# hrz2000/CustomNeRF

Hardware: AMD Instinct MI355X
Metric: training rays/s (higher is better)
Workload: dtype f16

## Files before the change

customnerf_amd/_lib.py:

```python
import ctypes as C
import os

import torch

_HERE = os.path.dirname(os.path.abspath(__file__))
LIB_PATH = os.path.join(_HERE, "libcustomnerf_hip.so")
ABI_VERSION = 7

vp, u32, u64, f32, i32 = C.c_void_p, C.c_uint32, C.c_uint64, C.c_float, C.c_int

SIGNATURES = {
    "cnerf_abi_version": [],
    "cnerf_profile_stage_events": [vp, u32],
    "cnerf_near_far_from_aabb": [vp, vp, vp, u32, f32, vp, vp, vp],
    "cnerf_sph_from_ray": [vp, vp, f32, u32, vp, vp],
    "cnerf_morton3D": [vp, u32, vp, vp],
    "cnerf_morton3D_invert": [vp, u32, vp, vp],
    "cnerf_packbits": [vp, u32, f32, vp, vp],
    "cnerf_march_rays_train": [vp, vp, vp, f32, f32, u32, u32, u32, u32, u32, vp, vp, vp, vp, vp, vp, vp, vp, vp],
    "cnerf_march_rays_train_count": [vp, vp, vp, f32, f32, u32, u32, u32, u32, vp, vp, vp, vp, vp, vp],
    "cnerf_march_rays_train_write": [vp, vp, vp, f32, f32, u32, u32, u32, u32, u32, vp, vp, vp, vp, vp, vp, vp, vp],
    "cnerf_march_rays_train_count_hits": [vp, vp, vp, f32, f32, u32, u32, u32, u32, vp, vp, vp, vp, vp, vp, vp],
    "cnerf_march_rays_train_write_hits": [vp, vp, f32, f32, u32, u32, u32, u32, u32, vp, vp, vp, vp, vp, vp, vp, vp],
    "cnerf_composite_rays_train_forward": [vp, vp, vp, vp, u32, u32, f32, vp, vp, vp, u32, vp],
    "cnerf_composite_rays_train_backward": [vp, vp, vp, vp, vp, vp, vp, vp, u32, u32, f32, vp, vp, u32, vp],
    "cnerf_march_rays": [u32, u32, vp, vp, vp, vp, f32, f32, u32, u32, u32, vp, vp, vp, vp, vp, vp, vp, vp],
    "cnerf_composite_rays": [u32, u32, f32, vp, vp, vp, vp, vp, vp, vp, vp, u32, vp],
    "cnerf_compact_rays_alive": [vp, u32, vp, vp, vp],
    "cnerf_grid_encode_forward": [vp, vp, vp, vp, u32, u32, u32, u32, u32, f32, u32, vp, u32, i32, u32, i32, vp],
    "cnerf_grid_encode_forward_strided": [vp, vp, vp, vp, u32, u32, u32, u32, u32, f32, u32, vp, u32, i32, u32, i32, u32, vp],
    "cnerf_grid_encode_forward_ordered": [vp, vp, vp, vp, u32, u32, u32, u32, u32, f32, u32, vp, u32, i32, u32, i32, u32, u32, vp],
    "cnerf_grid_encode_backward": [vp, vp, vp, vp, u32, u32, u32, u32, u32, f32, u32, vp, vp, u32, i32, u32, i32, vp, u64, vp],
    "cnerf_grid_encode_backward_prepare": [vp, vp, u32, u32, u32, u32, u32, f32, u32, u32, i32, u32, i32, vp, u64, vp, vp],
    "cnerf_grid_encode_backward_prepared": [vp, vp, vp, vp, u32, u32, u32, u32, u32, f32, u32, u32, i32, u32, i32, vp, u64, vp],
    "cnerf_grid_encode_backward_workspace_bytes": [vp, u32, u32, u32, u32, u32, f32, u32, i32, vp],
    "cnerf_grid_encode_backward_needs_plan": [vp, u32, u32, u32, u32, u32, f32, u32, u32, i32, vp],
    "cnerf_grad_total_variation": [vp, vp, vp, vp, f32, u32, u32, u32, u32, f32, u32, u32, i32, vp],
    "cnerf_cast_f32_to_f16": [vp, vp, u64, vp],
    "cnerf_field_forward": [vp, vp, vp, u32, u32, u32, u32, u32, vp, vp, vp, vp, vp, i32, vp],
    "cnerf_field_forward_strided": [vp, vp, vp, u32, u32, u32, u32, u32, vp, vp, vp, vp, vp, i32, u32, vp],
    "cnerf_field_backward": [vp, vp, vp, u32, u32, u32, u32, u32, vp, vp, vp, vp, vp, vp, vp, vp, vp, vp, u64, i32, vp],
    "cnerf_field_backward_ex": [vp, vp, vp, u32, u32, u32, u32, u32, vp, vp, vp, vp, vp, vp, vp, vp, vp, vp, u64, i32, vp, vp],
    "cnerf_field_backward_workspace_bytes": [u32, u32, u32, u32, i32, vp],
    "cnerf_stream_capture_id": [vp, vp],
    "cnerf_field_weight_image_bytes": [u32, u32, u32, vp],
    "cnerf_field_pack_weights": [u32, u32, u32, vp, vp, vp, vp, u64, vp],
    "cnerf_field_forward_img": [vp, vp, vp, u32, u32, u32, u32, u32, vp, vp, vp, vp, vp, i32, u32, vp, vp],
    "cnerf_field_backward_img": [vp, vp, vp, u32, u32, u32, u32, u32, vp, vp, vp, vp, vp, vp, vp, vp, vp, vp, u64, i32, vp, vp, vp],
    "cnerf_mlp_forward": [vp, u32, vp, u32, u32, u32, u32, u32, i32, vp, u32, i32, vp],
    "cnerf_mlp_backward": [vp, u32, vp, vp, u32, u32, u32, u32, u32, u32, i32, vp, u32, vp, vp, u64, i32, vp],
    "cnerf_mlp_backward_workspace_bytes": [u32, u32, u32, u32, u32, i32, vp],
    "cnerf_generate_rays": [vp, u32, u32, u32, f32, f32, f32, f32, f32, i32, vp, vp, vp],
    "cnerf_generate_rays_fisheye": [vp, u32, u32, u32, f32, f32, f32, f32, f32, vp, vp, vp, vp],
    "cnerf_occupancy_points": [vp, u32, f32, f32, vp, vp],
    "cnerf_occupancy_update": [vp, u32, f32, vp, vp, vp],
    "cnerf_occupancy_finalize_pack": [vp, u32, f32, vp, u32, vp, vp, vp],
    "cnerf_sample_pdf": [vp, vp, vp, u32, u32, u32, vp, vp],
    "cnerf_sample_coarse": [vp, vp, vp, vp, vp, vp, u32, u32, vp, vp, vp],
    "cnerf_sample_fine_merge": [vp, vp, vp, vp, vp, vp, vp, vp, u32, u32, u32, vp, vp, vp],
    "cnerf_sample_fine_merge_split": [vp, vp, vp, vp, vp, vp, vp, vp, u32, u32, u32, vp, vp, vp, vp, vp],
    "cnerf_sample_coarse_unit": [vp, vp, vp, vp, vp, vp, u32, u32, vp, vp, vp, f32, vp],
    "cnerf_sample_fine_merge_split_unit": [vp, vp, vp, vp, vp, vp, vp, vp, u32, u32, u32, vp, vp, vp, vp, f32, vp],
    "cnerf_composite_run": [vp, vp, vp, vp, vp, u32, u32, u32, i32, f32, vp, vp, vp],
    "cnerf_composite_run_backward": [vp, vp, vp, vp, vp, vp, u32, u32, u32, i32, f32, i32, i32, vp, vp, vp],
    "cnerf_recon_loss": [vp, vp, vp, u32, f32, f32, vp, vp, vp],
    "cnerf_recon_loss_scaled": [vp, vp, vp, u32, f32, f32, vp, vp, vp, vp],
    "cnerf_sample_coarse_unit_aabb": [vp, vp, vp, f32, vp, u32, u32, vp, vp, vp, vp, vp, f32, vp],
    "cnerf_composite_run_indexed": [vp, vp, vp, vp, vp, u32, u32, u32, i32, f32, vp, vp, vp, vp, vp, vp],
    "cnerf_composite_run_indexed_variants": [vp, vp, vp, vp, vp, u32, u32, u32, i32, f32, vp, vp, vp, vp, vp, u32, vp],
    "cnerf_composite_run_backward_indexed": [vp, vp, vp, vp, vp, vp, u32, u32, u32, i32, f32, i32, i32, vp, vp, vp, vp],
    "cnerf_composite_run_backward_indexed_flush": [vp, vp, vp, vp, vp, vp, u32, u32, u32, i32, f32, i32, i32, vp, vp, vp, i32, vp, vp],
    "cnerf_adam_step": [vp, vp, vp, vp, vp, u64, f32, f32, f32, f32, u32, f32, i32, vp],
    "cnerf_scaler_check": [vp, u64, vp, vp],
    "cnerf_scaler_watch": [vp],
    "cnerf_grid_backward_adam": [vp],
    "cnerf_grid_backward_adam_consumed": [vp],
    "cnerf_adam_step_scaled": [vp, vp, vp, vp, vp, u64, f32, f32, f32, f32, vp, f32, i32, vp],
    "cnerf_dp_pack": [vp, vp, u64, f32, vp],
    "cnerf_dp_reduce": [vp, u32, u64, vp, vp, vp],
    "cnerf_scaler_update": [vp, f32, f32, u32, vp],
    "cnerf_adam_step_scaled_multi": [vp, f32, f32, f32, vp, f32, i32, i32, f32, f32, u32, vp],
    "cnerf_marching_cubes_workspace_bytes": [u32, u32, u32, vp],
    "cnerf_marching_cubes_count": [vp, u32, u32, u32, f32, vp, u64, vp, vp],
    "cnerf_marching_cubes_emit": [vp, u32, u32, u32, f32, vp, vp, vp, u64, vp, vp, vp, u32, u32, vp],
    "cnerf_mesh_components_workspace_bytes": [u32, u32, vp],
    "cnerf_mesh_components_count": [vp, u32, u32, u32, i32, vp, u64, vp, vp],
    "cnerf_mesh_components_emit": [vp, vp, u32, vp, u32, u32, i32, vp, u64, vp, vp, vp, vp, u32, u32, vp],
    "cnerf_mesh_cluster_workspace_bytes": [u32, u32, vp, vp],
    "cnerf_mesh_cluster_count": [vp, u32, vp, u32, vp, vp, vp, vp, u64, vp, vp],
    "cnerf_mesh_cluster_emit": [vp, vp, u32, vp, u32, vp, vp, vp, vp, u64, vp, vp, vp, u32, u32, vp],
    "cnerf_mesh_decimate_workspace_bytes": [u32, u32, vp],
    "cnerf_mesh_decimate_init": [vp, u32, vp, u32, vp, u64, vp, vp],
    "cnerf_mesh_decimate_round": [u32, u32, u32, vp, u64, vp, vp],
    "cnerf_mesh_decimate_emit": [vp, u32, u32, vp, u64, vp, vp, vp, vp, u32, u32, vp],
    "cnerf_mesh_smooth_workspace_bytes": [u32, u32, vp],
    "cnerf_mesh_smooth_init": [vp, u32, u32, vp, u64, vp, vp],
    "cnerf_mesh_smooth_steps": [vp, u32, u32, u32, f32, f32, i32, vp, u64, vp, vp],
    "cnerf_mesh_smooth_normals": [vp, vp, u32, vp, u32, vp, u64, vp, vp],
    "cnerf_mesh_atlas_layout": [u32, u32, vp, vp],
    "cnerf_mesh_atlas_uvs": [vp, u32, u32, u32, vp, u32, vp, vp],
    "cnerf_mesh_atlas_points": [vp, vp, u32, vp, u32, u32, u32, u32, vp, vp, vp, u32, vp],
    "cnerf_mesh_atlas_store": [u32, u32, u32, u32, vp, u32, vp, vp, vp, vp],
    "cnerf_mesh_atlas_fill": [u32, u32, vp, vp, vp],
    "cnerf_mesh_raster_workspace_bytes": [u32, u32, u32, u32, vp],
    "cnerf_mesh_raster_visibility": [vp, u32, vp, u32, vp, f32, f32, f32, f32, u32, u32, i32, f32, i32, vp, u64, vp, vp, vp, vp, vp],
    "cnerf_mesh_raster_shade": [vp, vp, vp, u32, u32, vp, u32, u32, i32, vp, vp, vp, u32, vp, vp, f32, f32, vp, vp, vp, vp],
    "cnerf_mesh_bvh_workspace_bytes": [u32, u32, vp],
    "cnerf_mesh_bvh_build": [vp, u32, vp, u32, vp, u64, vp, vp],
    "cnerf_mesh_bvh_closest": [vp, u64, u32, u32, vp, u32, vp, vp, vp, vp, vp, vp],
    "cnerf_mesh_sample_workspace_bytes": [u32, vp],
    "cnerf_mesh_sample_count": [vp, u32, vp, u32, f32, vp, u64, vp, vp],
    "cnerf_mesh_sample_emit": [vp, u32, vp, u32, f32, vp, u64, vp, vp, vp, vp, u64, vp],
    "cnerf_sd_gemm": [vp, vp, u64, vp],
    "cnerf_sd_gemm_workspace_bytes": [vp, vp],
    "cnerf_sd_gemm_serves_ln": [vp, vp],
    "cnerf_sd_groupnorm_forward": [vp, vp, vp, u32, u32, u32, u32, f32, i32, vp, i32, vp, vp],
    "cnerf_sd_groupnorm_backward": [vp, vp, vp, vp, u32, u32, u32, u32, f32, i32, vp, vp, vp, vp],
    "cnerf_sd_groupnorm_backward_ex": [vp, vp, vp, vp, u32, u32, u32, u32, f32, i32, vp, vp, i32, vp, vp, vp],
    "cnerf_sd_layernorm_forward": [vp, vp, vp, u32, u32, f32, vp, vp],
    "cnerf_sd_softmax_forward": [vp, u64, u32, u32, vp],
    "cnerf_sd_softmax_backward": [vp, vp, u64, u32, u32, vp],
    "cnerf_sd_attention": [vp, vp, vp, vp, u32, u32, u32, u32, u32, u32, u64, u32, u64, u32, u64, u32, u64, i32, vp],
    "cnerf_sd_attention_v": [vp, vp, vp, vp, u32, u32, u32, u32, u32, u32, u64, u32, u64, u32, u64, u32, u64, i32, vp],
    "cnerf_sd_geglu": [vp, u64, u32, vp, vp],
    "cnerf_sd_transpose": [vp, vp, u32, u32, u32, u32, u32, u64, u64, vp],
    "cnerf_sd_image_to_vae_input": [vp, u32, u32, u32, u32, u32, vp, vp],
    "cnerf_sd_image_to_vae_input_backward": [vp, u32, u32, u32, u32, u32, vp, vp],
    "cnerf_sd_clip_preprocess": [vp, u32, u32, u32, u32, vp, vp, vp, vp],
    "cnerf_sd_patchify": [vp, u32, u32, u32, vp, vp],
    "cnerf_sd_timestep_embedding": [vp, u32, u32, vp, vp],
    "cnerf_sd_add_noise": [vp, vp, f32, u32, vp, vp],
    "cnerf_sd_sds_grad": [vp, u32, vp, f32, f32, f32, u32, vp, vp],
    "cnerf_edit_ray_images": [vp, u32, u32, vp, vp, vp, vp],
    "cnerf_edit_ray_images_backward": [vp, vp, vp, u32, u32, vp, vp],
    "cnerf_edit_l1_loss": [vp, vp, u32, f32, vp, vp, vp],
    "cnerf_edit_sds_loss": [vp, vp, u32, vp, vp, vp],
    "cnerf_edit_scale_by_scalar": [vp, vp, f32, u32, vp, vp],
    "cnerf_sd_sample_latents": [vp, vp, u32, u32, f32, vp, vp],
    "cnerf_sd_sample_latents_backward": [vp, vp, vp, u32, u32, f32, vp, vp],
    "cnerf_set_floats": [vp, vp, u32, vp],
    "cnerf_sd_add": [vp, vp, u64, vp, vp],
    "cnerf_sd_silu": [vp, u64, vp, vp],
    "cnerf_sd_concat": [vp, vp, u64, u32, u32, vp, vp],
    "cnerf_sd_concat_gn": [vp, vp, u64, u32, u32, vp, vp, u32, u32, vp],
}


class SdGemmDesc(C.Structure):
    _fields_ = [("A", vp), ("B", vp), ("C", vp), ("C32", vp), ("bias", vp), ("bias_rows", vp), ("residual", vp),
                ("M", u32), ("N", u32), ("K", u32), ("lda", u32), ("ldb", u32), ("ldc", u32), ("ldr", u32),
                ("rows_per_bias_row", u32), ("ld_bias_rows", u32), ("alpha", f32), ("act", C.c_int32), ("batch_outer", u32), ("batch_inner", u32),
                ("sa_o", u64), ("sa_i", u64), ("sb_o", u64), ("sb_i", u64), ("sc_o", u64), ("sc_i", u64),
                ("mode", C.c_int32), ("Cin", u32), ("H_in", u32), ("W_in", u32), ("H_out", u32), ("W_out", u32),
                ("KH", u32), ("KW", u32), ("stride", u32), ("pad_t", u32), ("pad_l", u32), ("ups", u32), ("tstride", u32),
                ("gn_sums", vp), ("gn_groups", u32), ("gn_rows", u32),
                ("ln_out", vp), ("ln_gamma", vp), ("ln_beta", vp), ("ln_eps", f32)]

ADAM_MAX_JOBS = 8


class AdamJobs(C.Structure):
    _fields_ = [("p", vp * ADAM_MAX_JOBS), ("g", vp * ADAM_MAX_JOBS), ("m", vp * ADAM_MAX_JOBS), ("v", vp * ADAM_MAX_JOBS), ("p_half", vp * ADAM_MAX_JOBS),
                ("n", u64 * ADAM_MAX_JOBS), ("lr", f32 * ADAM_MAX_JOBS), ("n_jobs", u32)]


class GridAdam(C.Structure):
    _fields_ = [("p", vp), ("g", vp), ("m", vp), ("v", vp), ("p_half", vp), ("n", u64), ("lr", f32), ("beta1", f32), ("beta2", f32), ("eps", f32),
                ("scaler_state", vp), ("extra_inv", f32), ("zero_grad", C.c_int)]


F32, F16 = 0, 1


def _load():
    if not os.path.exists(LIB_PATH):
        raise ImportError(
            f"{LIB_PATH} not found: the HIP extension is the product and has no fallback. "
            "Build it with `python -c 'import __graft_entry__ as g; g.build()'` or `make -C customnerf_amd/csrc`.")
    lib = C.CDLL(LIB_PATH)
    for name, argtypes in SIGNATURES.items():
        fn = getattr(lib, name)
        fn.argtypes = argtypes
        fn.restype = C.c_int
    lib.cnerf_target_arch.restype = C.c_char_p
    if lib.cnerf_abi_version() != ABI_VERSION:
        raise ImportError(f"ABI mismatch: library {lib.cnerf_abi_version()} vs binding {ABI_VERSION}")
    return lib


lib = _load()


def check(rc, what=""):
    if rc == 0:
        return
    if rc < 0:
        raise ValueError(f"customnerf_hip: {what} rejected its arguments (code {rc})")
    raise RuntimeError(f"customnerf_hip: {what} failed with hipError {rc}")


def ptr(t):
    return None if t is None else t.data_ptr()


def stream():
    return torch.cuda.current_stream().cuda_stream


def require_cuda(*tensors):
    for t in tensors:
        if t is not None and not t.is_cuda:
            raise RuntimeError("customnerf_amd: tensors must live on the GPU (HIP device memory); there is no CPU path")


def dtype_id(t):
    if t.dtype == torch.float32:
        return F32
    if t.dtype == torch.float16:
        return F16
    raise ValueError(f"unsupported dtype {t.dtype}")


def scratch_key(device):
    import torch
    return (device, torch.cuda.current_stream(device).cuda_stream)


_SCRATCH_GENERATION = [0]


def scratch_reallocated():
    _SCRATCH_GENERATION[0] += 1


def scratch_generation():
    return _SCRATCH_GENERATION[0]


_GRAD_CHAIN = {}


def grad_chain_wait(device):
    import torch
    cur = torch.cuda.current_stream(device)
    last = _GRAD_CHAIN.get(device)
    if last is not None and last.cuda_stream != cur.cuda_stream:
        cur.wait_stream(last)


def grad_chain_record(device):
    import torch
    _GRAD_CHAIN[device] = torch.cuda.current_stream(device)
```

customnerf_amd/csrc/gridencoder_binned.hip:

```cpp
#include "grid_common.h"
#include <vector>
#include <algorithm>
#include <cstdio>

#define BN_CHUNK_LOG2 12
#define BN_CHUNK (1u << BN_CHUNK_LOG2)
#define BN_THREADS 256
#define BN_PPT 4
#define BN_PTS (BN_THREADS * BN_PPT)
#define BN_MAX_CHUNKS 512
#define BN_SEG (1u << 18)

struct BinPlan {
    uint32_t bin_first[GE_MAX_LEVELS + 1];
    uint32_t nb;
    uint32_t total_bins;
};

struct BinWs {
    uint32_t *hist;
    uint32_t *bin_base;
    uint32_t *seg_first;
    void *records;
};
// ... 611 lines not shown
                    res_a = (uint32_t)old & 0x7FFFFFFFu;
                    res_b = (uint32_t)(old >> 32) & 0x7FFFFFFFu;
                }
            } else {
                if (sa) res_a = atomicAdd(&cursor[bin0 + 2 * lane], sa) & 0x7FFFFFFFu;
                if (sb) res_b = atomicAdd(&cursor[bin0 + 2 * lane + 1], sb) & 0x7FFFFFFFu;
            }
        }
    }
    asm volatile("s_waitcnt lgkmcnt(0)" ::: "memory");
    __builtin_amdgcn_s_barrier();
    asm volatile("" ::: "memory");
    uint2 *__restrict__ region = dslab + ((size_t)slot * nb + pb) * B3_REGION;
#pragma unroll
    for (int i = 0; i < PPT; i++) {
        if (!ok[i] || (abl & 4)) continue;
        const uint32_t fxq = min((uint32_t)(fx[i] * 65536.0f), 65535u);
        union { __half2 h; uint32_t u; } v;
        auto put = [&](uint32_t c, uint32_t ticket, uint32_t word, uint32_t val) {
            const uint32_t sl = start[c] + ticket;
            if (sl < B3_CAP) { s_rec[sl] = make_uint2(word, val); if (!wide) s_bin[sl] = (uint8_t)c; }
            else region[sl] = make_uint2(word, val);
        };
#pragma unroll
        for (int q = 0; q < 4; q++) {
            const uint32_t a0 = i0[i][q], a1 = i1[i][q];
            const uint32_t c0 = bin_of(a0);
            if (paired(a0, a1)) {
                const uint32_t t = 31u - (uint32_t)__clz((int)(a0 ^ a1));
                v.h = __floats2half2_rn(wyz[i][q] * g0[i], wyz[i][q] * g1[i]);
                put(c0, tk[i][q], local_of(a0) | (t << 12) | (fxq << 16), v.u);
            } else {
                const float w0 = (1 - fx[i]) * wyz[i][q], w1 = fx[i] * wyz[i][q];
                v.h = __floats2half2_rn(w0 * g0[i], w0 * g1[i]);
                put(c0, tk[i][q] & 0xFFFFu, local_of(a0) | (B3_SINGLE << 12), v.u);
                v.h = __floats2half2_rn(w1 * g0[i], w1 * g1[i]);
                put(bin_of(a1), tk[i][q] >> 16, local_of(a1) | (B3_SINGLE << 12), v.u);
            }
        }
    }
    if (!dense_lvl && wide) {
        if (threadIdx.x <= NBN / 2) {
            const uint32_t capb = plan.capb, b_lo = ((bin0 >> 1) + threadIdx.x) * 2u;
#pragma unroll
            for (int h = 0; h < 2; h++) {
                const uint32_t c = b_lo + h - bin0;
                if (c >= nch) continue;
                const uint32_t n = cnt[c], st0 = start[c], res = h ? res_b : res_a;
                const uint32_t staged = st0 >= B3_CAP ? 0u : min(n, (uint32_t)B3_CAP - st0);
                const uint32_t room = res >= capb ? 0u : capb - res;
                const uint32_t fit = min(min(n, room), staged);
                gdst[c] = res - st0;
                cnt[c] = fit;
                if (!(abl & 8)) runs[(size_t)(bin0 + c) * nb + pb] = (n - fit) | ((st0 + fit) << 16);
                if (n > fit) atomicOr(&cursor[bin0 + c], 0x80000000u);
            }
        }
    } else if (!dense_lvl && threadIdx.x < 64) {
        const uint32_t capb = plan.capb;
#pragma unroll
        for (int h = 0; h < 2; h++) {
            const uint32_t c = 2 * threadIdx.x + h;
            const uint32_t n = cnt[c], st0 = start[c], res = h ? res_b : res_a;
            const uint32_t staged = st0 >= B3_CAP ? 0u : min(n, (uint32_t)B3_CAP - st0);
            const uint32_t room = res >= capb ? 0u : capb - res;
            const uint32_t fit = min(min(n, room), staged);
            gdst[c] = res - st0;
            cnt[c] = fit;
            if (c < nch && !(abl & 8)) runs[(size_t)(bin0 + c) * nb + pb] = (n - fit) | ((st0 + fit) << 16);
            if (c < nch && n > fit) atomicOr(&cursor[bin0 + c], 0x80000000u);
        }
    }
    __syncthreads();
    const uint32_t total = (abl & 2) ? 0u : min(*s_total, (uint32_t)B3_CAP);
    if (dense_lvl) {
        for (uint32_t sl = threadIdx.x; sl < total; sl += B3_THREADS) region[sl] = s_rec[sl];
    } else if (wide) {
        const uint32_t capb = plan.capb, l16 = threadIdx.x & 15, grp = threadIdx.x >> 4;
        for (uint32_t c = grp; c < nch; c += B3_THREADS / 16) {
            const uint32_t st0 = start[c], en = min(c + 1 < NBN ? start[c + 1] : *s_total, total), fit = cnt[c], gd = gdst[c];
            for (uint32_t sl = st0 + l16; sl < en; sl += 16) {
                if (sl - st0 < fit) hslab[(size_t)(bin0 + c) * capb + (gd + sl)] = s_rec[sl];
                else region[sl] = s_rec[sl];
            }
        }
    } else {
        const uint32_t capb = plan.capb;
        for (uint32_t sl = threadIdx.x; sl < total; sl += B3_THREADS) {
            const uint32_t c = s_bin[sl];
            const uint32_t pos = gdst[c] + sl;
            if (sl - start[c] < cnt[c]) hslab[(size_t)(bin0 + c) * capb + pos] = s_rec[sl];
            else region[sl] = s_rec[sl];
        }
    }
}

__global__ void __launch_bounds__(BN_SCAN_THREADS) k_bin3_totals(const uint32_t *__restrict__ runs, uint32_t *__restrict__ pre, const uint32_t *__restrict__ cursor,
                                                                 uint32_t *__restrict__ bin_total, const Bin3Plan plan, uint32_t n_slots) {
    constexpr uint32_t NW = BN_SCAN_THREADS / 64;
    __shared__ uint32_t wave_tot[NW];
    __shared__ uint32_t carry;
    const uint32_t bin = blockIdx.x, nb = plan.p.nb;
    uint32_t slot = 0;
    while (slot + 1 < n_slots && plan.p.bin_first[slot + 1] <= bin) slot++;
    const bool hashed = plan.dense_slot[slot] == 0xFFFFFFFFu;
    if (hashed) {
        const uint32_t cw = cursor[bin], c = cw & 0x7FFFFFFFu;
        if (!(cw >> 31)) {
            if (threadIdx.x == 0) bin_total[bin] = min(c, plan.capb);
            return;
        }
    }
    const uint32_t *h = runs + (size_t)bin * nb;
    uint32_t *o = pre + (size_t)bin * nb;
    const uint32_t tid = threadIdx.x, lane = tid & 63, wave = tid >> 6;
    if (tid == 0) carry = 0;
    __syncthreads();
    for (uint32_t s0 = 0; s0 < nb; s0 += BN_SCAN_THREADS * 4) {
        const uint32_t i = s0 + tid * 4;
        uint32_t v[4];
#pragma unroll
        for (int k = 0; k < 4; k++) v[k] = i + k < nb ? (h[i + k] & 0xFFFFu) : 0;
        const uint32_t mine = v[0] + v[1] + v[2] + v[3];
        const uint32_t incl = cn_wave_incl_scan(mine);
        if (lane == 63) wave_tot[wave] = incl;
        __syncthreads();
        uint32_t wbase = 0, tot = 0;
#pragma unroll
        for (uint32_t w = 0; w < NW; w++) {
            const uint32_t t = wave_tot[w];
            if (w < wave) wbase += t;
            tot += t;
        }
        const uint32_t base = carry;
        uint32_t run = base + wbase + incl - mine;
#pragma unroll
        for (int k = 0; k < 4; k++) {
            if (i + k < nb) o[i + k] = run;
            run += v[k];
        }
        __syncthreads();
        if (tid == 0) carry = base + tot;
        __syncthreads();
    }
    if (tid == 0) bin_total[bin] = hashed ? min(cursor[bin] & 0x7FFFFFFFu, plan.capb) + carry : carry;
}

struct B3Adam {
    float *p, *m, *v;
    __half *ph;
    const float *state;
    float lr, beta1, beta2, eps, extra_inv;
    int zero_grad, on;
    const float *cst;
};
struct B3AdamConst { float gscale, step_size, rsqrt_bc2; int skip; };
__device__ __forceinline__ B3AdamConst b3_adam_const(const B3Adam &ad) {
    B3AdamConst c;
    c.gscale = ad.cst[0]; c.step_size = ad.cst[1]; c.rsqrt_bc2 = ad.cst[2]; c.skip = ad.cst[3] != 0.0f;
    return c;
}
__device__ __forceinline__ void b3_adam_update(const B3Adam &ad, const B3AdamConst &c, size_t idx, float4 gg, float4 pp, float4 mm, float4 vv, float4 *d4) {
    float *pa = &pp.x, *ga = &gg.x, *ma = &mm.x, *va = &vv.x;
#pragma unroll
    for (int k = 0; k < 4; k++) {
        const float gk = ga[k] * c.gscale;
        ma[k] = ad.beta1 * ma[k] + (1.0f - ad.beta1) * gk;
        va[k] = ad.beta2 * va[k] + (1.0f - ad.beta2) * gk * gk;
        pa[k] -= c.step_size * ma[k] / (sqrtf(va[k]) * c.rsqrt_bc2 + ad.eps);
    }
    *reinterpret_cast<float4 *>(ad.p + idx) = pp;
    *reinterpret_cast<float4 *>(ad.m + idx) = mm;
    *reinterpret_cast<float4 *>(ad.v + idx) = vv;
    *d4 = ad.zero_grad ? make_float4(0, 0, 0, 0) : gg;
    if (ad.ph) {
        union { __half2 h[2]; uint2 u; } o;
        o.h[0] = __floats2half2_rn(pp.x, pp.y);
        o.h[1] = __floats2half2_rn(pp.z, pp.w);
        *reinterpret_cast<uint2 *>(ad.ph + idx) = o.u;
    }
}
__device__ __forceinline__ void b3_adam_apply(const B3Adam &ad, const B3AdamConst &c, size_t idx, float4 gg, float4 *d4) {
    if (c.skip) {
        *d4 = ad.zero_grad ? make_float4(0, 0, 0, 0) : gg;
        return;
    }
    b3_adam_update(ad, c, idx, gg, *reinterpret_cast<const float4 *>(ad.p + idx), *reinterpret_cast<const float4 *>(ad.m + idx),
                   *reinterpret_cast<const float4 *>(ad.v + idx), d4);
}

__device__ __forceinline__ void b3_flush(const long long *acc, const GridLevels &lv, const Bin3Slots &plan, uint32_t slot, uint32_t bin, uint32_t nseg, uint32_t gseg,
                                         float *__restrict__ grad_grid, long long *__restrict__ partial, uint32_t hbits, const B3Adam &ad,
                                         const B3AdamConst &adc) {
    const uint32_t level = lv.order[slot];
    const uint32_t cb = bin - plan.bin_first[slot];
    const uint32_t e0 = hbits == 0xFFu ? cb << BN_CHUNK_LOG2 : 0u;
    const uint32_t n_entries = hbits == 0xFFu ? min(BN_CHUNK, lv.size[level] - e0) : min(BN_CHUNK, lv.size[level] >> hbits);
    float *__restrict__ dst = grad_grid + (size_t)lv.offset[level] * 2;
    if (nseg == 1 && ad.on && !adc.skip) {
        constexpr int NIT = BN_CHUNK / 2 / 1024;
        float4 gg[NIT], pp[NIT], mm[NIT], vv[NIT];
        auto index_of = [&](uint32_t j) {
            const uint32_t e = hbits == 0xFFu ? e0 + 2 * j : b3_entry_of(2 * j, cb, hbits);
            return ((size_t)lv.offset[level] + e) * 2;
        };
#pragma unroll
        for (int it = 0; it < NIT; it++) {
            const uint32_t j = it * 1024 + threadIdx.x;
            if (j < n_entries / 2) {
                const size_t idx = index_of(j);
                gg[it] = *reinterpret_cast<const float4 *>(grad_grid + idx);
                pp[it] = *reinterpret_cast<const float4 *>(ad.p + idx);
                mm[it] = *reinterpret_cast<const float4 *>(ad.m + idx);
                vv[it] = *reinterpret_cast<const float4 *>(ad.v + idx);
            }
        }
#pragma unroll
        for (int it = 0; it < NIT; it++) {
            const uint32_t j = it * 1024 + threadIdx.x;
            if (j >= n_entries / 2) continue;
            const size_t idx = index_of(j);
            float4 g = gg[it];
            g.x += bn_acc_to_float<__half>(acc[j * 2]); g.y += bn_acc_to_float<__half>(acc[BN_CHUNK + j * 2]);
            g.z += bn_acc_to_float<__half>(acc[j * 2 + 1]); g.w += bn_acc_to_float<__half>(acc[BN_CHUNK + j * 2 + 1]);
            b3_adam_update(ad, adc, idx, g, pp[it], mm[it], vv[it], reinterpret_cast<float4 *>(grad_grid + idx));
        }
    } else if (nseg == 1) {
        for (uint32_t j = threadIdx.x; j < n_entries / 2; j += 1024) {
            const uint32_t e = hbits == 0xFFu ? e0 + 2 * j : b3_entry_of(2 * j, cb, hbits);
            float4 *d4 = reinterpret_cast<float4 *>(dst + (size_t)e * 2);
            float4 g = *d4;
            g.x += bn_acc_to_float<__half>(acc[j * 2]); g.y += bn_acc_to_float<__half>(acc[BN_CHUNK + j * 2]);
            g.z += bn_acc_to_float<__half>(acc[j * 2 + 1]); g.w += bn_acc_to_float<__half>(acc[BN_CHUNK + j * 2 + 1]);
            if (ad.on) b3_adam_apply(ad, adc, ((size_t)lv.offset[level] + e) * 2, g, d4);
            else *d4 = g;
        }
    } else {
        long long *__restrict__ img = partial + (size_t)gseg * (BN_CHUNK * 2);
        for (uint32_t j = threadIdx.x; j < n_entries * 2; j += 1024) img[j] = acc[(j & 1) * BN_CHUNK + (j >> 1)];
    }
}

#define B3_RS_GROUPS 64
#ifndef B3_RS_BINS
#define B3_RS_BINS 256
#endif
__global__ void __launch_bounds__(256) k_bin3_reduce_split(const long long *__restrict__ partial, const uint32_t *__restrict__ seg_first,
                                                           const GridLevels lv, const Bin3Plan plan, float *__restrict__ grad_grid, uint32_t n_slots,
                                                           const uint32_t *__restrict__ split_list, const B3Adam ad) {
    __shared__ long long s_sum[3][B3_RS_GROUPS][4];
    const uint32_t n_split = split_list ? split_list[0] : gridDim.x;
    if (blockIdx.x >= n_split) return;
    B3AdamConst adc = {0.0f, 0.0f, 0.0f, 0};
    if (ad.on) adc = b3_adam_const(ad);
    for (uint32_t b = blockIdx.x; b < n_split; b += gridDim.x) {
    const uint32_t bin = split_list ? split_list[1 + b] : b;
    const uint32_t s0 = seg_first[bin], nseg = seg_first[bin + 1] - s0;
    if (nseg <= 1) continue;
    uint32_t slot = 0;
    while (slot + 1 < n_slots && plan.p.bin_first[slot + 1] <= bin) slot++;
    const uint32_t level = lv.order[slot];
    const bool dense_lvl = plan.dense_slot[slot] != 0xFFFFFFFFu;
    const uint32_t hb = plan.hbits[slot], cb = bin - plan.p.bin_first[slot];
    const uint32_t e0 = dense_lvl ? cb << BN_CHUNK_LOG2 : 0u;
    const uint32_t n_entries = dense_lvl ? min(BN_CHUNK, lv.size[level] - e0) : min(BN_CHUNK, lv.size[level] >> hb);
    if (blockIdx.y * B3_RS_GROUPS >= n_entries / 2) continue;
    const uint32_t lane = threadIdx.x & 63, sl = threadIdx.x >> 6;
    const uint32_t j = blockIdx.y * B3_RS_GROUPS + lane;
    const bool ok = j < n_entries / 2;
    long long sum[4] = {0, 0, 0, 0};
    const uint32_t e_dst = dense_lvl ? e0 + 2 * j : b3_entry_of(2 * j, cb, hb);
    const size_t idx = ((size_t)lv.offset[level] + e_dst) * 2;
    const bool fin = !sl && ok, upd = fin && ad.on && !adc.skip;
    float4 g_old = make_float4(0, 0, 0, 0), pp = g_old, mm = g_old, vv = g_old;
    if (fin) g_old = *reinterpret_cast<const float4 *>(grad_grid + idx);
    if (upd) {
        pp = *reinterpret_cast<const float4 *>(ad.p + idx);
        mm = *reinterpret_cast<const float4 *>(ad.m + idx);
        vv = *reinterpret_cast<const float4 *>(ad.v + idx);
    }
    if (ok) {
        const long long *__restrict__ src = partial + (size_t)s0 * (BN_CHUNK * 2) + (size_t)j * 4;
#pragma unroll 8
        for (uint32_t s = sl; s < nseg; s += 4) {
            const longlong2 v0 = reinterpret_cast<const longlong2 *>(src + (size_t)s * (BN_CHUNK * 2))[0];
            const longlong2 v1 = reinterpret_cast<const longlong2 *>(src + (size_t)s * (BN_CHUNK * 2))[1];
            sum[0] += v0.x; sum[1] += v0.y; sum[2] += v1.x; sum[3] += v1.y;
        }
    }
    if (sl) {
#pragma unroll
        for (int k = 0; k < 4; k++) s_sum[sl - 1][lane][k] = sum[k];
    }
    __syncthreads();
    if (!sl && ok) {
#pragma unroll
        for (int w = 0; w < 3; w++)
#pragma unroll
            for (int k = 0; k < 4; k++) sum[k] += s_sum[w][lane][k];
        float4 *dst = reinterpret_cast<float4 *>(grad_grid + idx);
        float4 g = g_old;
        g.x += bn_acc_to_float<__half>(sum[0]); g.y += bn_acc_to_float<__half>(sum[1]);
        g.z += bn_acc_to_float<__half>(sum[2]); g.w += bn_acc_to_float<__half>(sum[3]);
        if (upd) b3_adam_update(ad, adc, idx, g, pp, mm, vv, dst);
        else if (ad.on) *dst = ad.zero_grad ? make_float4(0, 0, 0, 0) : g;
        else *dst = g;
    }
    __syncthreads();
    }
}

template <int W>
__device__ __forceinline__ void b3_walk_runs(long long *acc, uint32_t *s_c, uint32_t *tiles, const uint32_t *__restrict__ rt, const uint32_t *__restrict__ pt,
                                             const uint2 *__restrict__ lvl_slab, uint32_t nb, uint32_t pb_first, uint32_t begin, uint32_t end) {
    const uint32_t lane = threadIdx.x & 63;
    constexpr uint32_t CB = B3_WALK_BLOCKS, KPL = CB / 64;
    uint32_t *s_pre = tiles, *s_base = tiles + CB + 1;
    for (uint32_t pb0 = pb_first; pb0 < nb; pb0 += CB) {
        if (threadIdx.x < 64) {
            uint32_t len[KPL], base[KPL], loc = 0, p_last = 0xFFFFFFFFu;
#pragma unroll
            for (uint32_t k = 0; k < KPL; k++) {
                const uint32_t pbl = pb0 + lane * KPL + k;
                uint32_t p_j = 0xFFFFFFFFu, r_j = 0;
                if (pbl < nb) { p_j = pt[pbl]; r_j = rt[pbl]; }
                uint32_t lo = 0, hi = 0;
                if (p_j < end) {
                    const uint32_t c_j = r_j & 0xFFFFu;
                    lo = max(p_j, begin) - p_j;
                    hi = max(min(p_j + c_j, end), p_j) - p_j;
                    if (hi < lo) hi = lo;
                }
                len[k] = hi - lo;
                base[k] = pbl * B3_REGION + (r_j >> 16) + lo;
                loc += len[k];
                p_last = p_j;
            }
            const uint32_t incl = cn_wave_incl_scan(loc);
            uint32_t run = incl - loc;
#pragma unroll
            for (uint32_t k = 0; k < KPL; k++) {
                s_pre[lane * KPL + k] = run;
                s_base[lane * KPL + k] = base[k];
                run += len[k];
            }
            if (lane == 63) { s_pre[CB] = incl; s_c[1] = p_last >= end ? 1u : 0u; }
        }
        __syncthreads();
        const uint32_t total = s_pre[CB], last = s_c[1];
        for (uint32_t f0 = threadIdx.x * W; f0 < total; f0 += 1024 * W) {
            uint32_t j = 0;
#pragma unroll
            for (uint32_t step = CB / 2; step; step >>= 1)
                if (s_pre[j + step] <= f0) j += step;
            uint32_t idx[W];
            bool ok4[W];
#pragma unroll
            for (int u = 0; u < W; u++) {
                const uint32_t f = f0 + u;
                ok4[u] = f < total;
                while (ok4[u] && f >= s_pre[j + 1]) j++;
                idx[u] = ok4[u] ? s_base[j] + (f - s_pre[j]) : s_base[0];
            }
            uint2 v[W];
#pragma unroll
            for (int u = 0; u < W; u++) v[u] = lvl_slab[idx[u]];
            B3Pending c;
            c.key = 0xFFFFFFFFu;
#pragma unroll
            for (int u = 0; u < W; u++)
                if (ok4[u]) b3_push_record(acc, c, v[u]);
            b3_flush_pending(acc, c);
        }
        __syncthreads();
        if (last) break;
    }
}

__global__ void __launch_bounds__(1024, 8) k_bin3_accum(const uint2 *__restrict__ hslab, const uint2 *__restrict__ dslab, const uint32_t *__restrict__ runs,
                                                     const uint32_t *__restrict__ pre, const uint32_t *__restrict__ cursor, const uint32_t *__restrict__ bin_base,
                                                     const uint32_t *__restrict__ seg_first, const GridLevels lv, const Bin3Plan plan,
                                                     float *__restrict__ grad_grid, long long *__restrict__ partial, const uint32_t *__restrict__ seg_bin,
                                                     uint32_t n_slots, uint32_t seg_records, uint32_t only, const B3Adam ad) {
    extern __shared__ __attribute__((aligned(16))) unsigned char bn_lds[];
    long long *acc = reinterpret_cast<long long *>(bn_lds);
    uint32_t *s_w = reinterpret_cast<uint32_t *>(bn_lds + sizeof(long long) * BN_CHUNK * 2);
    const uint32_t gseg = blockIdx.x;
    if (gseg >= seg_first[plan.p.total_bins]) return;
#ifdef CNERF_TUNING
    if (only) {
        uint32_t sl_ = 0;
        const uint32_t b_ = seg_bin[gseg];
        while (sl_ + 1 < n_slots && plan.p.bin_first[sl_ + 1] <= b_) sl_++;
        if ((plan.dense_slot[sl_] == 0xFFFFFFFFu) != (only == 1)) return;
    }
#else
    (void)only;
#endif
    const uint32_t nb = plan.p.nb;
    if (threadIdx.x == 0) {
        const uint32_t bin = seg_bin[gseg];
        uint32_t slot = 0;
        while (slot + 1 < n_slots && plan.p.bin_first[slot + 1] <= bin) slot++;
        uint32_t lo = 0;
        const bool hashed = plan.dense_slot[slot] == 0xFFFFFFFFu;
        const uint32_t cw = hashed ? cursor[bin] : 0u;
        const uint32_t treg = hashed ? min(cw & 0x7FFFFFFFu, plan.capb) : 0u;
        uint32_t begin = (gseg - seg_first[bin]) * seg_records;
        if (!hashed || ((cw >> 31) && begin > treg)) {
            begin -= treg;
            const uint32_t *p = pre + (size_t)bin * nb;
            uint32_t hi = nb;
            while (hi - lo > 1) {
                const uint32_t mid = (lo + hi) >> 1;
                if (p[mid] <= begin) lo = mid; else hi = mid;
            }
        }
        s_w[0] = bin; s_w[1] = lo; s_w[2] = slot; s_w[3] = treg;
    }
    for (uint32_t i = threadIdx.x; i < sizeof(long long) * BN_CHUNK * 2 / 16; i += 1024) reinterpret_cast<uint4 *>(bn_lds)[i] = make_uint4(0, 0, 0, 0);
    __syncthreads();
    const uint32_t bin = s_w[0], pb_first = s_w[1], slot = s_w[2], treg = s_w[3];
    const uint32_t seg = gseg - seg_first[bin], nseg = seg_first[bin + 1] - seg_first[bin];
    const uint32_t total = bin_base[bin + 1] - bin_base[bin];
    const uint32_t begin = seg * seg_records, end = min(begin + seg_records, total);
    uint32_t *s_c = s_w + 4, *tiles = s_w + 8;
    const uint32_t *__restrict__ rt = runs + (size_t)bin * nb, *__restrict__ pt = pre + (size_t)bin * nb;
    const uint2 *__restrict__ lvl_slab = dslab + (size_t)slot * nb * B3_REGION;
// ... 48 lines not shown
    plan.total_bins = acc;
}

static uint64_t bn_layout(const BinPlan &plan, uint32_t B, uint32_t nl, int dtype, BinWs *ws, void *base) {
    const uint64_t rec = dtype == CNERF_F16 ? 8 : 12;
    uint64_t off = 0;
    const uint64_t o_hist = off; off = bn_align(off + (uint64_t)plan.total_bins * plan.nb * 4);
    const uint64_t o_base = off; off = bn_align(off + (uint64_t)(plan.total_bins + 1) * 4);
    const uint64_t o_seg = off; off = bn_align(off + (uint64_t)(plan.total_bins + 1) * 4);
    const uint64_t o_rec = off; off = bn_align(off + (uint64_t)B * nl * 8 * rec);
    if (ws) {
        char *p = (char *)base;
        ws->hist = (uint32_t *)(p + o_hist);
        ws->bin_base = (uint32_t *)(p + o_base);
        ws->seg_first = (uint32_t *)(p + o_seg);
        ws->records = p + o_rec;
    }
    return off;
}

#define B3_SEG_MIN ((1u << 16) + (1u << 13))
static uint32_t b3_seg(uint32_t B, uint32_t max_chunks) {
    const uint64_t hashed_bin = (uint64_t)B * 4 / (max_chunks ? max_chunks : 1);
    const uint64_t s = hashed_bin + hashed_bin / 8;
    static const uint64_t cap = (uint64_t)cn_tune_env("CNERF_B3_SEG_CAP", 1 << 18);
    if (s < B3_SEG_MIN) return B3_SEG_MIN;
    const uint64_t k = (s + cap - 1) / cap;
    return (uint32_t)((s + k - 1) / k);
}

static uint32_t b3_max_bins(const Bin3Slots &plan, uint32_t nl) {
    uint32_t m = 1;
    for (uint32_t s = 0; s < nl; s++) m = m > plan.bin_first[s + 1] - plan.bin_first[s] ? m : plan.bin_first[s + 1] - plan.bin_first[s];
    return m;
}

struct Bin3Ws {
    uint32_t *runs, *pre, *cursor, *bin_base, *seg_first, *seg_bin, *split_list;
    float *adam_const;
    uint2 *hslab, *dslab;
    long long *partial;
    uint64_t max_seg, cursor_bytes;
};

static bool b3_is_dense(const GridLevels &lv, uint32_t level, int ac) {
    const uint64_t r1 = (uint64_t)lv.resolution[level] + (ac ? 0 : 1);
    return r1 * r1 * r1 <= lv.size[level];
}

static bool b3_plan(const GridLevels &lv, uint32_t nl, uint32_t B, Bin3Plan &plan, uint32_t &n_dense, int ac) {
    Bin3Slots &ps = plan.p;
    ps.nb = cn_div_up(B, B3_PTS);
    uint32_t acc = 0;
    for (uint32_t s = 0; s < nl; s++) {
        ps.bin_first[s] = acc;
        acc += cn_div_up(lv.size[lv.order[s]], BN_CHUNK);
    }
    for (uint32_t s = nl; s <= GE_MAX_LEVELS; s++) ps.bin_first[s] = acc;
    ps.total_bins = acc;
    n_dense = 0;
    uint64_t cap = 0;
    bool ok = true;
    for (uint32_t s = 0; s < GE_MAX_LEVELS; s++) { plan.dense_slot[s] = 0xFFFFFFFFu; plan.hbits[s] = 0; }
    for (uint32_t s = 0; s < nl; s++) {
        const uint32_t level = lv.order[s], size = lv.size[level];
        if (b3_is_dense(lv, level, ac)) { plan.dense_slot[s] = n_dense++; continue; }
        const uint32_t nch = ps.bin_first[s + 1] - ps.bin_first[s];
        if ((size & (size - 1)) != 0 || (nch & (nch - 1)) != 0 || !(size == nch * BN_CHUNK || (nch == 1 && size >= 32))) ok = false;
        uint32_t hb = 0;
        while ((1u << hb) < nch) hb++;
        plan.hbits[s] = (uint8_t)hb;
        const uint64_t mean = (uint64_t)B * 17 / 4 / nch;
        const uint64_t c = mean + mean / 2 + 8192;
        cap = cap > c ? cap : c;
    }
    plan.capb = (uint32_t)((cap + 1) & ~(uint64_t)1);
    return ok;
}

static bool b3_enabled(const GridLevels &lv, uint32_t nl, uint32_t B, int dtype, uint32_t gridtype, int ac) {
    static const int on = cn_tune_env("CNERF_B3", 1);
    static const int wide_on = cn_tune_env("CNERF_B3_WIDE", 1);
    (void)gridtype;
    if (!on || dtype != CNERF_F16) return false;
    Bin3Plan plan;
    uint32_t nd;
    if (!b3_plan(lv, nl, B, plan, nd, ac)) return false;
    const uint32_t mc = b3_max_bins(plan.p, nl);
    if (mc > (wide_on ? (uint32_t)B3_WIDE_CHUNKS : (uint32_t)B3_NARROW_CHUNKS)) return false;
    if ((uint64_t)plan.p.total_bins * plan.capb >= 0xF0000000ull) return false;
    return (uint64_t)nl * plan.p.nb * B3_REGION < 0xF0000000ull && (uint64_t)B * 8 < 0x7FFFFFFFull;
}

static uint64_t b3_layout(const Bin3Plan &plan, uint32_t n_dense, uint32_t B, uint32_t nl, Bin3Ws *ws, void *base) {
    const Bin3Slots &ps = plan.p;
    uint64_t off = 0;
    const uint64_t o_runs = off; off = bn_align(off + (uint64_t)ps.total_bins * ps.nb * 4);
    const uint64_t o_pre = off; off = bn_align(off + (uint64_t)ps.total_bins * ps.nb * 4);
    const uint64_t o_cur = off; off = bn_align(off + ((uint64_t)ps.total_bins + 2) * 4);
    const uint64_t o_base = off; off = bn_align(off + (uint64_t)(ps.total_bins + 1) * 4);
    const uint64_t o_seg = off; off = bn_align(off + (uint64_t)(ps.total_bins + 1) * 4);
    const uint64_t o_split = off; off = bn_align(off + (uint64_t)(ps.total_bins + 1) * 4);
    const uint64_t o_adamc = off; off = bn_align(off + 16);
    const uint64_t h_records = (uint64_t)ps.total_bins * plan.capb;
    const uint64_t d_records = (uint64_t)nl * ps.nb * B3_REGION;
    (void)n_dense;
    const uint64_t o_h = off; off = bn_align(off + h_records * 8);
    const uint64_t o_d = off; off = bn_align(off + d_records * 8);
    const uint64_t max_seg = (uint64_t)ps.total_bins + cn_div_up64((uint64_t)B * nl * 8, b3_seg(B, b3_max_bins(ps, nl)));
    const uint64_t o_segbin = off; off = bn_align(off + max_seg * 4);
    const uint64_t o_part = off; off = bn_align(off + max_seg * BN_CHUNK * 2 * 8);
    if (ws) {
        char *p = (char *)base;
        ws->runs = (uint32_t *)(p + o_runs);
        ws->pre = (uint32_t *)(p + o_pre);
        ws->cursor = (uint32_t *)(p + o_cur);
        ws->cursor_bytes = (uint64_t)ps.total_bins * 4;
        ws->bin_base = (uint32_t *)(p + o_base);
        ws->seg_first = (uint32_t *)(p + o_seg);
        ws->split_list = (uint32_t *)(p + o_split);
        ws->adam_const = (float *)(p + o_adamc);
        ws->hslab = (uint2 *)(p + o_h);
        ws->dslab = (uint2 *)(p + o_d);
        ws->seg_bin = (uint32_t *)(p + o_segbin);
        ws->partial = (long long *)(p + o_part);
        ws->max_seg = max_seg;
    }
    return off;
}

__global__ void __launch_bounds__(256) k_bin3_zero(uint32_t *__restrict__ p, uint32_t n) {
    const uint32_t i = blockIdx.x * 256 + threadIdx.x;
    if (i < n) p[i] = 0;
}

static CnerfGridAdam g_grid_adam;
static bool g_grid_adam_armed = false;
static int g_grid_adam_consumed = 0;
void bn_grid_adam_arm(const CnerfGridAdam *cfg) {
    g_grid_adam_armed = cfg != nullptr;
    if (cfg) { g_grid_adam = *cfg; g_grid_adam_consumed = 0; }
}
int bn_grid_adam_consumed() { const int c = g_grid_adam_consumed; g_grid_adam_consumed = 0; return c; }
static B3Adam b3_take_adam(float *gemb, const GridLevels &lv, uint32_t nl, bool third_form) {
    B3Adam ad = {};
    if (!g_grid_adam_armed || g_grid_adam.g != gemb) return ad;
    g_grid_adam_armed = false;
    const uint64_t covered = ((uint64_t)lv.offset[nl - 1] + lv.size[nl - 1]) * 2;
    if (!third_form || covered != g_grid_adam.n) return ad;
    ad.p = g_grid_adam.p; ad.m = g_grid_adam.m; ad.v = g_grid_adam.v; ad.ph = reinterpret_cast<__half *>(g_grid_adam.p_half);
    ad.state = g_grid_adam.scaler_state;
    ad.lr = g_grid_adam.lr; ad.beta1 = g_grid_adam.beta1; ad.beta2 = g_grid_adam.beta2; ad.eps = g_grid_adam.eps; ad.extra_inv = g_grid_adam.extra_inv;
    ad.zero_grad = g_grid_adam.zero_grad; ad.on = 1;
    g_grid_adam_consumed = 1;
    return ad;
}

static int b3_backward(const __half *grad, const float *inputs, const GridLevels &lv, float *gemb, uint32_t B, uint32_t nl, uint32_t gridtype, int ac,
                       uint32_t interp, void *workspace, hipStream_t st) {
    if (nl == 0) return CNERF_OK;
    Bin3Plan plan;
    uint32_t n_dense;
    if (!b3_plan(lv, nl, B, plan, n_dense, ac)) return CNERF_EINVAL;
    Bin3Ws ws;
    b3_layout(plan, n_dense, B, nl, &ws, workspace);
    static const int emit_pad = cn_tune_env("CNERF_B3_EMIT_LDS_PAD", 0);
    const uint32_t lds_n = B3_CAP * 9 + B3_NARROW_CHUNKS * 12 + 16, lds_w = B3_CAP * 8 + B3_WIDE_CHUNKS * 12 + 16;
    const uint32_t emit_lds = (lds_n > lds_w ? lds_n : lds_w) + (uint32_t)emit_pad, acc_lds = BN_CHUNK * 2 * sizeof(long long) + 32 + B3_MAXT * 8;
    static bool attr_set = false;
    if (!attr_set) {
        (void)hipFuncSetAttribute(reinterpret_cast<const void *>(&k_bin3_emit), hipFuncAttributeMaxDynamicSharedMemorySize, emit_lds);
        (void)hipFuncSetAttribute(reinterpret_cast<const void *>(&k_bin3_accum), hipFuncAttributeMaxDynamicSharedMemorySize, acc_lds);
        attr_set = true;
    }
    const Bin3Slots &ps = plan.p;
    const uint32_t seg = b3_seg(B, b3_max_bins(ps, nl));
    B3Adam ad = b3_take_adam(gemb, lv, nl, true);
    ad.cst = ws.adam_const;
    hipLaunchKernelGGL(k_bin3_zero, dim3(cn_div_up(ps.total_bins, 256)), dim3(256), 0, st, ws.cursor, ps.total_bins);
    cn_stage(0, st);
    hipLaunchKernelGGL(k_bin3_emit, dim3(ps.nb * nl), dim3(B3_THREADS), emit_lds, st, grad, inputs, lv, plan, ws.runs, ws.cursor, ws.hslab, ws.dslab, B, gridtype, ac,
                       interp, gemb, nl, (uint32_t)cn_tune_env("CNERF_B3_EMIT_ABL", 0), g_cn_found_inf);
    cn_stage(1, st);
    hipLaunchKernelGGL(k_bin3_totals, dim3(ps.total_bins), dim3(BN_SCAN_THREADS), 0, st, (const uint32_t *)ws.runs, ws.pre, (const uint32_t *)ws.cursor, ws.bin_base,
                       plan, nl);
    static const uint32_t rs_bins = (uint32_t)cn_tune_env("CNERF_B3_RS_BINS", B3_RS_BINS);
    static const int rs_list = cn_tune_env("CNERF_B3_RSLIST", 1);
    hipLaunchKernelGGL(k_bin_scan_bins, dim3(1), dim3(1024), 0, st, ws.bin_base, ws.bin_base, ws.seg_first, ps.total_bins, seg, ws.seg_bin, ws.split_list, ad.on,
                       ad.state, ad.lr, ad.beta1, ad.beta2, ad.extra_inv, ad.on ? ws.adam_const : (float *)nullptr);
    hipLaunchKernelGGL(k_bin3_accum, dim3((uint32_t)ws.max_seg), dim3(1024), acc_lds, st, (const uint2 *)ws.hslab, (const uint2 *)ws.dslab, (const uint32_t *)ws.runs,
                       (const uint32_t *)ws.pre, (const uint32_t *)ws.cursor, (const uint32_t *)ws.bin_base, (const uint32_t *)ws.seg_first, lv, plan, gemb, ws.partial,
                       (const uint32_t *)ws.seg_bin, nl, seg, (uint32_t)cn_tune_env("CNERF_B3_ONLY", 0), ad);
    cn_stage(2, st);
    hipLaunchKernelGGL(k_bin3_reduce_split, dim3(!rs_list || ps.total_bins < rs_bins ? ps.total_bins : rs_bins, BN_CHUNK * 2 / 4 / B3_RS_GROUPS), dim3(256), 0, st,
                       (const long long *)ws.partial, ws.seg_first, lv, plan, gemb, nl, rs_list ? (const uint32_t *)ws.split_list : (const uint32_t *)nullptr, ad);
    cn_stage(3, st);
#ifdef CNERF_TUNING
    static const int dbg = cn_tune_env("CNERF_B3_DEBUG", 0);
    static int dbg_calls = 0;
    if (dbg && (++dbg_calls % dbg) == 0) {
        uint32_t n_split = 0, n_seg = 0;
        (void)hipStreamSynchronize(st);
        (void)hipMemcpy(&n_split, ws.split_list, 4, hipMemcpyDeviceToHost);
        (void)hipMemcpy(&n_seg, ws.seg_first + ps.total_bins, 4, hipMemcpyDeviceToHost);
        std::vector<uint32_t> sf(ps.total_bins + 1), bb(ps.total_bins + 1);
        (void)hipMemcpy(sf.data(), ws.seg_first, sf.size() * 4, hipMemcpyDeviceToHost);
        (void)hipMemcpy(bb.data(), ws.bin_base, bb.size() * 4, hipMemcpyDeviceToHost);
        fprintf(stderr, "[b3] call %d: bins %u segments %u split bins %u seg %u | per slot (bins, segments, records, max bin):", dbg_calls, ps.total_bins, n_seg, n_split, seg);
        for (uint32_t sl = 0; sl < nl; sl++) {
            uint32_t mx = 0;
            for (uint32_t b_ = ps.bin_first[sl]; b_ < ps.bin_first[sl + 1]; b_++) mx = std::max(mx, bb[b_ + 1] - bb[b_]);
            fprintf(stderr, " L%u(%u,%u,%u,%u)", lv.order[sl], ps.bin_first[sl + 1] - ps.bin_first[sl], sf[ps.bin_first[sl + 1]] - sf[ps.bin_first[sl]],
                    bb[ps.bin_first[sl + 1]] - bb[ps.bin_first[sl]], mx);
        }
        fprintf(stderr, "\n");
    }
#endif
    return cn_launch_status();
}

bool bn_needs_plan(uint32_t B, uint32_t nl, const GridLevels &lv, int dtype, uint32_t gridtype) {
    return !(b3_enabled(lv, nl, B, dtype, gridtype, 0) && b3_enabled(lv, nl, B, dtype, gridtype, 1));
}

bool bn_eligible(uint32_t B, uint32_t D, uint32_t C, uint32_t nl, const GridLevels &lv) {
    if (D != 3 || C != 2 || nl == 0) return false;
    for (uint32_t l = 0; l < nl; l++)
        if (cn_div_up(lv.size[l], BN_CHUNK) > BN_MAX_CHUNKS || (lv.size[l] & 7)) return false;
    return (uint64_t)B * nl * 8 < 0xF0000000ull;
}

uint64_t bn_workspace_bytes(uint32_t B, uint32_t nl, const GridLevels &lv, int dtype) {
    uint64_t b3 = 0;
    for (int ac = 0; ac < 2; ac++) {
        if (!b3_enabled(lv, nl, B, dtype, 0u, ac)) continue;
        Bin3Plan p3;
        uint32_t nd;
        b3_plan(lv, nl, B, p3, nd, ac);
        const uint64_t b = b3_layout(p3, nd, B, nl, nullptr, nullptr);
        b3 = b > b3 ? b : b3;
    }
    BinPlan plan;
    bn_plan(lv, nl, B, plan);
    const uint64_t b1 = bn_layout(plan, B, nl, dtype, nullptr, nullptr);
    return b1 > b3 ? b1 : b3;
}

int bn_prepare(const float *inputs, const GridLevels &lv, uint32_t B, uint32_t nl, uint32_t gridtype, int ac, uint32_t interp, int dtype,
               void *workspace, hipStream_t st) {
    BinPlan plan;
    bn_plan(lv, nl, B, plan);
    BinWs ws;
    bn_layout(plan, B, nl, dtype, &ws, workspace);
    const dim3 grid1(plan.nb * nl);
    hipLaunchKernelGGL(k_bin_hist, grid1, dim3(BN_THREADS), 0, st, inputs, lv, plan, ws.hist, B, gridtype, ac, interp);
    hipLaunchKernelGGL(k_bin_scan_blocks, dim3(plan.total_bins), dim3(BN_SCAN_THREADS), 0, st, ws.hist, ws.bin_base, plan.nb);
    hipLaunchKernelGGL(k_bin_scan_bins, dim3(1), dim3(1024), 0, st, ws.bin_base, ws.bin_base, ws.seg_first, plan.total_bins, BN_SEG, (uint32_t *)nullptr);
    return cn_launch_status();
}

template <typename T>
static int bn_phase2(const T *grad, const float *inputs, const GridLevels &lv, float *gemb, uint32_t B, uint32_t nl, uint32_t gridtype, int ac,
                     uint32_t interp, int dtype, void *workspace, hipStream_t st) {
    BinPlan plan;
    bn_plan(lv, nl, B, plan);
    BinWs ws;
    bn_layout(plan, B, nl, dtype, &ws, workspace);
    const dim3 grid1(plan.nb * nl);
    hipLaunchKernelGGL((k_bin_emit<T>), grid1, dim3(BN_THREADS), 0, st, grad, inputs, lv, plan, ws.hist, ws.bin_base, (BinRec<T> *)ws.records, B,
                       gridtype, ac, interp, gemb, g_cn_found_inf);
    const uint64_t max_seg = (uint64_t)plan.total_bins + cn_div_up64((uint64_t)B * nl * 8, BN_SEG);
    const uint32_t lds_bytes = BN_CHUNK * 2 * sizeof(typename BinAcc<T>::type) + 16;
    static bool attr_set = false;
    if (!attr_set) {
        (void)hipFuncSetAttribute(reinterpret_cast<const void *>(&k_bin_accum<T>), hipFuncAttributeMaxDynamicSharedMemorySize, lds_bytes);
        attr_set = true;
    }
    hipLaunchKernelGGL((k_bin_accum<T>), dim3((uint32_t)max_seg), dim3(1024), lds_bytes, st, (const BinRec<T> *)ws.records,
                       ws.bin_base, ws.seg_first, lv, plan, gemb);
    return cn_launch_status();
}

int bn_backward(const void *grad, const float *inputs, const GridLevels &lv, float *gemb, uint32_t B, uint32_t nl, uint32_t gridtype, int ac,
                uint32_t interp, int dtype, void *workspace, hipStream_t st, bool prepared) {
    if (b3_enabled(lv, nl, B, dtype, gridtype, ac)) return b3_backward((const __half *)grad, inputs, lv, gemb, B, nl, gridtype, ac, interp, workspace, st);
    if (nl) (void)b3_take_adam(gemb, lv, nl, false);
    if (!prepared) {
        const int rc = bn_prepare(inputs, lv, B, nl, gridtype, ac, interp, dtype, workspace, st);
        if (rc) return rc;
    }
    if (dtype == CNERF_F16) return bn_phase2<__half>((const __half *)grad, inputs, lv, gemb, B, nl, gridtype, ac, interp, dtype, workspace, st);
    return bn_phase2<float>((const float *)grad, inputs, lv, gemb, B, nl, gridtype, ac, interp, dtype, workspace, st);
}
```

customnerf_amd/csrc/render.hip:

```cpp
#include "common.h"
#include <float.h>

#define RN_WAVES 4
#define RN_THREADS (RN_WAVES * 64)
#define RN_MAXS 128

__device__ __forceinline__ float rn_linspace01(uint32_t i, uint32_t n) {
    const float step = 1.0f / (float)(n - 1);
    return (i < n / 2) ? step * (float)i : 1.0f - step * (float)(n - 1 - i);
}

__device__ __forceinline__ float rn_norm_depth(float z, float near, float far) {
    const float x = (z - near) / (far - near);
    return (x != x) ? x : fminf(fmaxf(x, 0.0f), 1.0f);
}

__device__ __forceinline__ void rn_point(const float *o, const float *d, float z, const float *aabb, float *out) {
#pragma unroll
    for (int c = 0; c < 3; c++) out[c] = fminf(fmaxf(o[c] + d[c] * z, aabb[c]), aabb[3 + c]);
}

__global__ void __launch_bounds__(256) k_sample_coarse(const float *__restrict__ rays_o, const float *__restrict__ rays_d, const float *__restrict__ nears,
                                                       const float *__restrict__ fars, const float *__restrict__ aabb, const float *__restrict__ noise,
                                                       uint32_t N, uint32_t T, float *__restrict__ z_vals, float *__restrict__ xyzs,
// ... 338 lines not shown
        for (int k = 0; k < 6; k++) go[v][k] = g_out[((size_t)v * N + n) * 6 + k];
    bool use[3];
#pragma unroll
    for (int v = 0; v < 3; v++) {
        bool any = false;
#pragma unroll
        for (int k = 0; k < 6; k++) any = any || !(go[v][k] == 0.0f);
        use[v] = __builtin_amdgcn_readfirstlane(any ? 1 : 0) != 0;
    }

    float z_[NCH], delta_[NCH], sigma_[NCH], alpha_[3][NCH], tr_[3][NCH];
    float4 c_[NCH];
    uint32_t row_[NCH];
    float tot[3] = {0, 0, 0};
    {
        float carry[3] = {1.0f, 1.0f, 1.0f};
#pragma unroll
        for (int ch = 0; ch < NCH; ch++) {
            const uint32_t i = ch * 64 + lane;
            const bool ok = i < S;
            float z = 0, delta = 0, sigma = 0;
            float4 c = make_float4(0, 0, 0, 0);
            uint32_t row = 0;
            if (ok) {
                z = zr[i]; delta = (i + 1 < S) ? zr[i + 1] - z : sd;
                row = src_index ? src_index[(size_t)n * S + i] : n * S + i;
                sigma = sigmas[row]; c = c4[row];
            }
            z_[ch] = z; delta_[ch] = delta; sigma_[ch] = sigma; c_[ch] = c; row_[ch] = row;
            const float zn = rn_norm_depth(z, near, far);
            const float e = rn_edit(c.w, soft, thr);
#pragma unroll
            for (int v = 0; v < 3; v++) {
                if (!use[v]) continue;
                const float alpha = ok ? 1.0f - expf(-delta * (sigma * rn_variant_scale(v, e))) : 0.0f;
                const float tr = rn_excl_prod_scan(ok ? (1.0f - alpha + 1e-15f) : 1.0f, carry[v], lane);
                alpha_[v][ch] = alpha; tr_[v][ch] = tr;
                const float G = go[v][0] * c.x + go[v][1] * c.y + go[v][2] * c.z + go[v][3] * zn + go[v][4] + (detach_mask ? 0.0f : go[v][5] * c.w);
                if (ok) tot[v] += G * alpha * tr;
            }
        }
#pragma unroll
        for (int v = 0; v < 3; v++)
            if (use[v]) tot[v] = rn_wave_sum(tot[v]);
    }
    float pref[3] = {0, 0, 0};
#pragma unroll
    for (int ch = 0; ch < NCH; ch++) {
        const uint32_t i = ch * 64 + lane;
        const bool ok = i < S;
        const float z = z_[ch], delta = delta_[ch], sigma = sigma_[ch];
        const float4 c = c_[ch];
        const uint32_t row = row_[ch];
        const float zn = rn_norm_depth(z, near, far);
        const float e = rn_edit(c.w, soft, thr);
        float gs = 0.0f, ge = 0.0f;
        float4 gc = make_float4(0, 0, 0, 0);
#pragma unroll
        for (int v = 0; v < 3; v++) {
            if (!use[v]) continue;
            const float m = rn_variant_scale(v, e);
            const float alpha = alpha_[v][ch];
            const float q = 1.0f - alpha + 1e-15f;
            const float tr = tr_[v][ch];
            const float w = alpha * tr;
            const float G = go[v][0] * c.x + go[v][1] * c.y + go[v][2] * c.z + go[v][3] * zn + go[v][4] + (detach_mask ? 0.0f : go[v][5] * c.w);
            const float incl = rn_incl_sum_scan(ok ? G * w : 0.0f, pref[v], lane);
            const float suffix = tot[v] - incl;
            const float dalpha = G * tr - suffix / q;
            const float dsv = dalpha * delta * (1.0f - alpha);
            const bool detached = (v == 0) && detach_bg && !(c.w >= 0.5f);
            if (!detached) {
                gs += dsv * m;
                gc.x += go[v][0] * w; gc.y += go[v][1] * w; gc.z += go[v][2] * w;
            }
            gc.w += go[v][5] * w;
            if (v == 1) ge += dsv * sigma;
            if (v == 2) ge -= dsv * sigma;
        }
        if (soft) gc.w += ge * 100.0f * e * (1.0f - e);
        if (flush_thr > 0.0f) {
            const float sc = fminf(fmaxf(sigma, e_lo), e_hi);
            const bool dead = fabsf(gs) * sc < flush_thr && fabsf(gc.x) * (c.x * (1.0f - c.x)) < flush_thr && fabsf(gc.y) * (c.y * (1.0f - c.y)) < flush_thr &&
                              fabsf(gc.z) * (c.z * (1.0f - c.z)) < flush_thr && fabsf(gc.w) * (c.w * (1.0f - c.w)) < flush_thr;
            if (dead) { gs = 0.0f; gc = make_float4(0, 0, 0, 0); }
            else if (ok && tile_live) {
                const uint32_t Pc = N * T_coarse, t_f = S - T_coarse;
                const uint32_t lt = row < Pc ? (row - n * T_coarse) >> 5 : (T_coarse >> 5) + ((row - Pc - n * t_f) >> 5);
                live_bits |= 1u << lt;
            }
        }
        if (ok) {
            g_sigma[row] = gs;
            reinterpret_cast<float4 *>(g_rgbc)[row] = gc;
        }
    }
    if (tile_live) {
        const uint32_t Pc = N * T_coarse, t_f = S - T_coarse, ntc = T_coarse >> 5, ntf = t_f >> 5;
        for (uint32_t k = 0; k < ntc + ntf; k++) {
            const bool any = __ballot((live_bits >> k) & 1u) != 0;
            if (lane == 0) tile_live[k < ntc ? (n * T_coarse >> 5) + k : ((Pc + n * t_f) >> 5) + (k - ntc)] = any ? 1 : 0;
        }
    }
}

#define RL_BLOCKS 64
__device__ unsigned int g_recon_loss_ticket = 0;
__global__ void __launch_bounds__(256) k_recon_loss(const float *__restrict__ out_ray, const float *__restrict__ rgb_gt, const float *__restrict__ mask_gt,
                                                    uint32_t N, float k_rgb, float k_m, float *__restrict__ partial, float *__restrict__ g_out,
                                                    const float *__restrict__ grad_scale, float *__restrict__ loss) {
    __shared__ float red[2][4];
    __shared__ unsigned int s_last;
    float s_rgb = 0.0f, s_m = 0.0f;
    const float gsc = grad_scale ? grad_scale[0] : 1.0f;
    for (uint32_t n = blockIdx.x * 256 + threadIdx.x; n < N; n += gridDim.x * 256) {
        const float *r = out_ray + (size_t)n * 6;
        float g[6] = {0, 0, 0, 0, 0, 0};
#pragma unroll
        for (int c = 0; c < 3; c++) {
            const float d = r[c] - rgb_gt[(size_t)n * 3 + c];
            s_rgb += d * d;
            g[c] = (2.0f * k_rgb * d) * gsc;
        }
        if (mask_gt) {
            const float d = r[5] - mask_gt[n];
            s_m += d * d;
            g[5] = (2.0f * k_m * d) * gsc;
        }
#pragma unroll
        for (int c = 0; c < 6; c++) {
            g_out[(size_t)n * 6 + c] = g[c];
            g_out[((size_t)N + n) * 6 + c] = 0.0f;
            g_out[((size_t)2 * N + n) * 6 + c] = 0.0f;
        }
    }
    s_rgb = rn_wave_sum(s_rgb);
    s_m = rn_wave_sum(s_m);
    const uint32_t lane = threadIdx.x & 63, wave = threadIdx.x >> 6;
    if (lane == 0) { red[0][wave] = s_rgb; red[1][wave] = s_m; }
    __syncthreads();
    if (threadIdx.x == 0) {
        partial[blockIdx.x] = k_rgb * (red[0][0] + red[0][1] + red[0][2] + red[0][3]) + k_m * (red[1][0] + red[1][1] + red[1][2] + red[1][3]);
        __threadfence();
        s_last = atomicAdd(&g_recon_loss_ticket, 1u) == gridDim.x - 1 ? 1u : 0u;
    }
    __syncthreads();
    if (s_last && threadIdx.x < 64) {
        __threadfence();
        const float v = rn_wave_sum(threadIdx.x < gridDim.x ? __builtin_nontemporal_load(partial + threadIdx.x) : 0.0f);
        if (threadIdx.x == 0) { loss[0] = v; g_recon_loss_ticket = 0; }
    }
}


extern "C" {

int cnerf_sample_coarse(const float *rays_o, const float *rays_d, const float *nears, const float *fars, const float *aabb, const float *noise,
                        uint32_t N, uint32_t T, float *z_vals, float *xyzs, void *stream) {
    if (T < 2 || T > RN_MAXS) return CNERF_EINVAL;
    if (N == 0) return CNERF_OK;
    if (!rays_o || !rays_d || !nears || !fars || !aabb || !z_vals || !xyzs) return CNERF_ENULL;
    hipLaunchKernelGGL(k_sample_coarse, dim3(cn_div_up(N * T, 256)), dim3(256), 0, CN_STREAM(stream), rays_o, rays_d, nears, fars, aabb, noise, N, T,
                       z_vals, xyzs, (float *)nullptr, 0.0f, (float *)nullptr, (float *)nullptr, 0.0f);
    return cn_launch_status();
}

int cnerf_sample_coarse_unit(const float *rays_o, const float *rays_d, const float *nears, const float *fars, const float *aabb, const float *noise,
                             uint32_t N, uint32_t T, float *z_vals, float *xyzs, float *unit, float bound, void *stream) {
    if (T < 2 || T > RN_MAXS || !(bound > 0.0f)) return CNERF_EINVAL;
    if (N == 0) return CNERF_OK;
    if (!rays_o || !rays_d || !nears || !fars || !aabb || !z_vals || !xyzs || !unit) return CNERF_ENULL;
    hipLaunchKernelGGL(k_sample_coarse, dim3(cn_div_up(N * T, 256)), dim3(256), 0, CN_STREAM(stream), rays_o, rays_d, nears, fars, aabb, noise, N, T,
                       z_vals, xyzs, unit, bound, (float *)nullptr, (float *)nullptr, 0.0f);
    return cn_launch_status();
}

int cnerf_sample_coarse_unit_aabb(const float *rays_o, const float *rays_d, const float *aabb, float min_near, const float *noise, uint32_t N, uint32_t T,
                                  float *nears, float *fars, float *z_vals, float *xyzs, float *unit, float bound, void *stream) {
    if (T < 2 || T > RN_MAXS || !(bound > 0.0f)) return CNERF_EINVAL;
    if (N == 0) return CNERF_OK;
    if (!rays_o || !rays_d || !nears || !fars || !aabb || !z_vals || !xyzs || !unit) return CNERF_ENULL;
    hipLaunchKernelGGL(k_sample_coarse, dim3(cn_div_up(N * T, 256)), dim3(256), 0, CN_STREAM(stream), rays_o, rays_d, (const float *)nullptr,
                       (const float *)nullptr, aabb, noise, N, T, z_vals, xyzs, unit, bound, nears, fars, min_near);
    return cn_launch_status();
}

int cnerf_sample_fine_merge_split(const float *rays_o, const float *rays_d, const float *nears, const float *fars, const float *aabb, const float *z_vals,
                                  const float *sigmas, const float *u, uint32_t N, uint32_t T, uint32_t t, float *z_all, float *xyz_all, float *xyz_fine,
                                  uint32_t *src_index, void *stream) {
    if (T < 3 || T > RN_MAXS || t < 2 || t > RN_MAXS) return CNERF_EINVAL;
    if ((uint64_t)N * (T + t) >= 0xFFFFFFFFull) return CNERF_EINVAL;
    if (N == 0) return CNERF_OK;
    if (!rays_o || !rays_d || !nears || !fars || !aabb || !z_vals || !sigmas || !z_all) return CNERF_ENULL;
    if (!xyz_all && !(xyz_fine && src_index)) return CNERF_ENULL;
    hipLaunchKernelGGL(k_sample_fine_merge, dim3(cn_div_up(N, RN_WAVES)), dim3(RN_THREADS), 0, CN_STREAM(stream), rays_o, rays_d, nears, fars, aabb,
                       z_vals, sigmas, u, N, T, t, z_all, xyz_all, xyz_fine, src_index, (float *)nullptr, 0.0f);
    return cn_launch_status();
}

int cnerf_sample_fine_merge_split_unit(const float *rays_o, const float *rays_d, const float *nears, const float *fars, const float *aabb,
                                       const float *z_vals, const float *sigmas, const float *u, uint32_t N, uint32_t T, uint32_t t, float *z_all,
                                       float *xyz_fine, uint32_t *src_index, float *unit_fine, float bound, void *stream) {
    if (T < 3 || T > RN_MAXS || t < 2 || t > RN_MAXS || !(bound > 0.0f)) return CNERF_EINVAL;
    if ((uint64_t)N * (T + t) >= 0xFFFFFFFFull) return CNERF_EINVAL;
    if (N == 0) return CNERF_OK;
    if (!rays_o || !rays_d || !nears || !fars || !aabb || !z_vals || !sigmas || !z_all || !xyz_fine || !src_index || !unit_fine) return CNERF_ENULL;
    hipLaunchKernelGGL(k_sample_fine_merge, dim3(cn_div_up(N, RN_WAVES)), dim3(RN_THREADS), 0, CN_STREAM(stream), rays_o, rays_d, nears, fars, aabb,
                       z_vals, sigmas, u, N, T, t, z_all, (float *)nullptr, xyz_fine, src_index, unit_fine, bound);
    return cn_launch_status();
}

int cnerf_sample_fine_merge(const float *rays_o, const float *rays_d, const float *nears, const float *fars, const float *aabb, const float *z_vals,
                            const float *sigmas, const float *u, uint32_t N, uint32_t T, uint32_t t, float *z_all, float *xyz_all, void *stream) {
    if (!xyz_all) return CNERF_ENULL;
    return cnerf_sample_fine_merge_split(rays_o, rays_d, nears, fars, aabb, z_vals, sigmas, u, N, T, t, z_all, xyz_all, nullptr, nullptr, stream);
}

int cnerf_composite_run_indexed(const float *sigmas, const float *rgbc, const float *z_vals, const float *nears, const float *fars, uint32_t N, uint32_t S,
                                uint32_t num_steps, int soft_mask, float conf_thr, const uint32_t *src_index, float *out_ray, float *out_weights,
                                float *sigma_sorted, float *rgbc_sorted, void *stream) {
    return cnerf_composite_run_indexed_variants(sigmas, rgbc, z_vals, nears, fars, N, S, num_steps, soft_mask, conf_thr, src_index, out_ray, out_weights,
                                                sigma_sorted, rgbc_sorted, 7u, stream);
}

int cnerf_composite_run_indexed_variants(const float *sigmas, const float *rgbc, const float *z_vals, const float *nears, const float *fars, uint32_t N,
                                         uint32_t S, uint32_t num_steps, int soft_mask, float conf_thr, const uint32_t *src_index, float *out_ray,
                                         float *out_weights, float *sigma_sorted, float *rgbc_sorted, uint32_t variant_mask, void *stream) {
    if (S == 0 || S > 64 * RN_MAXCH || num_steps == 0 || variant_mask == 0 || variant_mask > 7u) return CNERF_EINVAL;
    if (N == 0) return CNERF_OK;
    if (!sigmas || !rgbc || !z_vals || !nears || !fars || !out_ray) return CNERF_ENULL;
    if ((((uintptr_t)rgbc) | ((uintptr_t)rgbc_sorted)) & 15) return CNERF_EINVAL;
    hipLaunchKernelGGL(k_composite_run_fwd, dim3(cn_div_up(N, RN_WAVES)), dim3(RN_THREADS), 0, CN_STREAM(stream), sigmas, rgbc, z_vals, nears, fars, N, S,
                       num_steps, soft_mask, conf_thr, out_ray, out_weights, src_index, sigma_sorted, rgbc_sorted, variant_mask);
    return cn_launch_status();
}

int cnerf_composite_run(const float *sigmas, const float *rgbc, const float *z_vals, const float *nears, const float *fars, uint32_t N, uint32_t S,
                        uint32_t num_steps, int soft_mask, float conf_thr, float *out_ray, float *out_weights, void *stream) {
    return cnerf_composite_run_indexed(sigmas, rgbc, z_vals, nears, fars, N, S, num_steps, soft_mask, conf_thr, nullptr, out_ray, out_weights, nullptr,
                                       nullptr, stream);
}

int cnerf_composite_run_backward_indexed_flush(const float *grad_out_ray, const float *sigmas, const float *rgbc, const float *z_vals, const float *nears,
                                               const float *fars, uint32_t N, uint32_t S, uint32_t num_steps, int soft_mask, float conf_thr, int detach_bg,
                                               int detach_mask_from_field, const uint32_t *src_index, float *grad_sigmas, float *grad_rgbc, int flush_half_zero,
                                               uint8_t *tile_live, void *stream) {
    if (S == 0 || S > 64 * RN_MAXCH || num_steps == 0) return CNERF_EINVAL;
    if (N == 0) return CNERF_OK;
    if (!grad_out_ray || !sigmas || !rgbc || !z_vals || !nears || !fars || !grad_sigmas || !grad_rgbc) return CNERF_ENULL;
    if ((((uintptr_t)rgbc) | ((uintptr_t)grad_rgbc)) & 15) return CNERF_EINVAL;
    if (tile_live && (!flush_half_zero || !src_index || num_steps >= S || (num_steps & 31u) || ((S - num_steps) & 31u) || S > 256)) return CNERF_EINVAL;
    if ((uint64_t)N * S > 0xFFFFFFFFull) return CNERF_EINVAL;
#define RN_CBWD(NCH)                                                                                                                                  \
    hipLaunchKernelGGL(k_composite_run_bwd<NCH>, dim3(cn_div_up(N, RN_WAVES)), dim3(RN_THREADS), 0, CN_STREAM(stream), grad_out_ray, sigmas, rgbc, z_vals, \
                       nears, fars, N, S, num_steps, soft_mask, conf_thr, detach_bg, detach_mask_from_field, grad_sigmas, grad_rgbc, src_index,     \
                       flush_half_zero ? 1.4901161193847656e-08f  : 0.0f, tile_live, num_steps)
    switch (cn_div_up(S, 64)) {
        case 1: RN_CBWD(1); break;
        case 2: RN_CBWD(2); break;
        case 3: RN_CBWD(3); break;
        default: RN_CBWD(4); break;
    }
#undef RN_CBWD
    return cn_launch_status();
}

int cnerf_composite_run_backward_indexed(const float *grad_out_ray, const float *sigmas, const float *rgbc, const float *z_vals, const float *nears,
                                         const float *fars, uint32_t N, uint32_t S, uint32_t num_steps, int soft_mask, float conf_thr, int detach_bg,
                                         int detach_mask_from_field, const uint32_t *src_index, float *grad_sigmas, float *grad_rgbc, void *stream) {
    return cnerf_composite_run_backward_indexed_flush(grad_out_ray, sigmas, rgbc, z_vals, nears, fars, N, S, num_steps, soft_mask, conf_thr, detach_bg,
                                                      detach_mask_from_field, src_index, grad_sigmas, grad_rgbc, 0, nullptr, stream);
}

int cnerf_composite_run_backward(const float *grad_out_ray, const float *sigmas, const float *rgbc, const float *z_vals, const float *nears,
                                 const float *fars, uint32_t N, uint32_t S, uint32_t num_steps, int soft_mask, float conf_thr, int detach_bg,
                                 int detach_mask_from_field, float *grad_sigmas, float *grad_rgbc, void *stream) {
    return cnerf_composite_run_backward_indexed(grad_out_ray, sigmas, rgbc, z_vals, nears, fars, N, S, num_steps, soft_mask, conf_thr, detach_bg,
                                                detach_mask_from_field, nullptr, grad_sigmas, grad_rgbc, stream);
}

int cnerf_recon_loss_scaled(const float *out_ray, const float *rgb_gt, const float *mask_gt, uint32_t N, float w_rgb, float w_conf,
                            const float *grad_scale, float *loss, float *grad_out_ray, void *stream) {
    if (N == 0) return CNERF_EINVAL;
    if (!out_ray || !rgb_gt || !loss || !grad_out_ray) return CNERF_ENULL;
    const uint32_t blocks = cn_div_up(N, 256) < RL_BLOCKS ? cn_div_up(N, 256) : RL_BLOCKS;
    hipLaunchKernelGGL(k_recon_loss, dim3(blocks), dim3(256), 0, CN_STREAM(stream), out_ray, rgb_gt, mask_gt, N, w_rgb / (3.0f * (float)N),
                       mask_gt ? w_conf / (float)N : 0.0f, loss + 1, grad_out_ray, grad_scale, loss);
    return cn_launch_status();
}

int cnerf_recon_loss(const float *out_ray, const float *rgb_gt, const float *mask_gt, uint32_t N, float w_rgb, float w_conf, float *loss,
                     float *grad_out_ray, void *stream) {
    return cnerf_recon_loss_scaled(out_ray, rgb_gt, mask_gt, N, w_rgb, w_conf, nullptr, loss, grad_out_ray, stream);
}

int cnerf_sample_pdf(const float *bins, const float *weights, const float *u, uint32_t B, uint32_t n_bins, uint32_t n_samples, float *samples, void *stream) {
    if (n_bins < 2 || n_bins > RN_PDF_MAXB) return CNERF_EINVAL;
    if (B == 0 || n_samples == 0) return CNERF_OK;
    if (!bins || !weights || !samples) return CNERF_ENULL;
    hipLaunchKernelGGL(k_sample_pdf, dim3(cn_div_up(B, RN_WAVES)), dim3(RN_THREADS), 0, CN_STREAM(stream), bins, weights, u, B, n_bins, n_samples, samples);
    return cn_launch_status();
}


}
```

customnerf_amd/gridencoder/grid.py:

```python
import os
import weakref

import numpy as np
import torch
import torch.nn as nn
from torch.autograd import Function

from .._lib import lib, check, ptr, stream, dtype_id, require_cuda, scratch_key, grad_chain_wait, grad_chain_record, scratch_reallocated

_PROFILE = None


def set_profile(sink):
    global _PROFILE
    _PROFILE = sink


def forward_kernel_name(half):
    return "k_grid_fwd_fast" if half else "k_grid_fwd"


LEVEL_MAJOR, SAMPLE_MAJOR = 0, 1


# ... 85 lines not shown
        C = table.shape[1]
        S = float(np.log2(per_level_scale))
        H = int(base_resolution)
        max_level = L if max_level is None else min(max_level, L)
        outputs = torch.empty(L, B, C, device=inputs.device, dtype=table.dtype)
        if max_level < L:
            outputs.zero_()
        if calc_grad_inputs:
            dy_dx = torch.empty(B, L * D * C, device=inputs.device, dtype=table.dtype)
            if max_level < L:
                dy_dx.zero_()
        else:
            dy_dx = None
        prof = _PROFILE
        if prof is not None:
            e0, e1 = torch.cuda.Event(enable_timing=True), torch.cuda.Event(enable_timing=True)
            e0.record()
        check(lib.cnerf_grid_encode_forward(ptr(inputs), ptr(table), offsets_host.ctypes.data, ptr(outputs), B, D, C, L, max_level, S, H,
                                            ptr(dy_dx), gridtype, int(align_corners), interpolation, dtype_id(table), stream()),
              "grid_encode_forward")
        if prof is not None:
            e1.record()
            prof.append((e0, e1, B, max_level, table.element_size()))
        ctx.save_for_backward(inputs, dy_dx)
        ctx.cfg = (offsets_host, B, D, C, L, S, H, gridtype, interpolation, max_level, align_corners, tuple(embeddings.shape))
        return outputs

    @staticmethod
    def backward(ctx, grad):
        inputs, dy_dx = ctx.saved_tensors
        offsets_host, B, D, C, L, S, H, gridtype, interpolation, max_level, align_corners, eshape = ctx.cfg
        grad = grad.contiguous()
        if dy_dx is not None and grad.dtype != dy_dx.dtype:
            grad = grad.to(dy_dx.dtype)
        grad_embeddings = torch.zeros(eshape, device=grad.device, dtype=torch.float32)
        grad_inputs = torch.empty(B, D, device=grad.device, dtype=torch.float32) if dy_dx is not None else None
        ws, ws_bytes = (None, 0) if dy_dx is not None else _bwd_workspace(offsets_host, B, D, C, L, max_level, S, H, dtype_id(grad), grad.device)
        check(lib.cnerf_grid_encode_backward(ptr(grad), ptr(inputs), offsets_host.ctypes.data, ptr(grad_embeddings), B, D, C, L, max_level,
                                             S, H, ptr(dy_dx), ptr(grad_inputs), gridtype, int(align_corners), interpolation,
                                             dtype_id(grad), ptr(ws), ws_bytes, stream()), "grid_encode_backward")
        return grad_inputs, grad_embeddings, None, None, None, None, None, None, None, None, None


_PRE_SCATTER_HOOK = None


def set_pre_scatter_hook(fn):
    global _PRE_SCATTER_HOOK
    _PRE_SCATTER_HOOK = fn


_SIDE = {}


class _Plan:
    __slots__ = ('ws', 'event', 'inputs_ptr', 'rows', '__weakref__')

    def __init__(self, ws, event, inputs_ptr, rows):
        self.ws, self.event, self.inputs_ptr, self.rows = ws, event, inputs_ptr, rows


def _side(device):
    key = scratch_key(device)
    st = _SIDE.get(key)
    if st is None:
        st = _SIDE[key] = {'stream': torch.cuda.Stream(device=device), 'ws': None, 'owner': None}
    return st


def _side_busy(side):
    return side['owner'] is not None and side['owner']() is not None


_NEEDS_PLAN = {}


def _needs_plan(offsets_host, B, D, C, L, S, H, dt, gridtype):
    import ctypes
    key = (offsets_host.ctypes.data, B, D, C, L, S, H, dt, gridtype)
    v = _NEEDS_PLAN.get(key)
    if v is None:
        n = ctypes.c_int(0)
        check(lib.cnerf_grid_encode_backward_needs_plan(offsets_host.ctypes.data, B, D, C, L, L, S, H, gridtype, dt, ctypes.addressof(n)),
              "grid_encode_backward_needs_plan")
        if len(_NEEDS_PLAN) > 256:
            _NEEDS_PLAN.clear()
        v = _NEEDS_PLAN[key] = (bool(n.value), offsets_host)
    return v[0]


def _prepare_plan(inputs, offsets_host, B, D, C, L, S, H, gridtype, align_corners, interpolation, dt, device):
    import ctypes
    if not _needs_plan(offsets_host, B, D, C, L, S, H, dt, gridtype):
        return None
    side = _side(device)
    if _side_busy(side):
        return None
    need = ctypes.c_uint64(0)
    check(lib.cnerf_grid_encode_backward_workspace_bytes(offsets_host.ctypes.data, B, D, C, L, L, S, H, dt, ctypes.addressof(need)),
          "grid_encode_backward_workspace_bytes")
    if not need.value:
        return None
    if side['ws'] is None or side['ws'].numel() < need.value:
        side['ws'] = torch.empty(int(need.value * 1.25) + 256, dtype=torch.uint8, device=device)
        scratch_reallocated()
    ws = side['ws']
    cur = torch.cuda.current_stream()
    side['stream'].wait_stream(cur)
    ok = ctypes.c_int(0)
    check(lib.cnerf_grid_encode_backward_prepare(ptr(inputs), offsets_host.ctypes.data, B, D, C, L, L, S, H, gridtype, int(align_corners),
                                                 interpolation, dt, ptr(ws), ws.numel(), ctypes.addressof(ok), side['stream'].cuda_stream),
          "grid_encode_backward_prepare")
    if not ok.value:
        return None
    ev = torch.cuda.Event()
    ev.record(side['stream'])
    plan = _Plan(ws, ev, inputs.data_ptr(), B)
    side['owner'] = weakref.ref(plan)
    return plan


class _grid_attach(Function):

    @staticmethod
    def forward(ctx, enc, inputs, embeddings, offsets_host, per_level_scale, base_resolution, gridtype, align_corners, interpolation, overlap,
                grad_in_place=False, plan=None):
        ctx.param = embeddings if grad_in_place else None
        L, B, C = enc.shape
        D = inputs.shape[1]
        S, H = float(np.log2(per_level_scale)), int(base_resolution)
        dt = dtype_id(enc)
        ctx.save_for_backward(inputs)
        ctx.cfg = (offsets_host, B, D, C, L, S, H, gridtype, interpolation, align_corners, tuple(embeddings.shape))
        if plan is not None and (plan.inputs_ptr != inputs.data_ptr() or plan.rows != B):
            plan = None
        if plan is None and overlap:
            plan = _prepare_plan(inputs, offsets_host, B, D, C, L, S, H, gridtype, align_corners, interpolation, dt, enc.device)
        ctx.plan = plan
        return enc.detach()

    @staticmethod
    def backward(ctx, grad):
        inputs, = ctx.saved_tensors
        offsets_host, B, D, C, L, S, H, gridtype, interpolation, align_corners, eshape = ctx.cfg
        grad = grad.contiguous()
        if _PRE_SCATTER_HOOK is not None:
            _PRE_SCATTER_HOOK()
        tgt = ctx.param.grad if ctx.param is not None else None
        in_place = (tgt is not None and tgt.dtype == torch.float32 and tgt.is_contiguous() and tuple(tgt.shape) == tuple(eshape)
                    and tgt.device == grad.device)
        grad_embeddings = tgt if in_place else torch.zeros(eshape, device=grad.device, dtype=torch.float32)
        if in_place:
            grad_chain_wait(grad.device)
        if ctx.plan is not None:
            ws, ev = ctx.plan.ws, ctx.plan.event
            torch.cuda.current_stream().wait_event(ev)
            try:
                check(lib.cnerf_grid_encode_backward_prepared(ptr(grad), ptr(inputs), offsets_host.ctypes.data, ptr(grad_embeddings), B, D, C, L, L, S, H,
                                                              gridtype, int(align_corners), interpolation, dtype_id(grad), ptr(ws), ws.numel(), stream()),
                      "grid_encode_backward_prepared")
            finally:
                ctx.plan = None
        else:
            ws, ws_bytes = _bwd_workspace(offsets_host, B, D, C, L, L, S, H, dtype_id(grad), grad.device)
            check(lib.cnerf_grid_encode_backward(ptr(grad), ptr(inputs), offsets_host.ctypes.data, ptr(grad_embeddings), B, D, C, L, L, S, H, None, None,
                                                 gridtype, int(align_corners), interpolation, dtype_id(grad), ptr(ws), ws_bytes, stream()), "grid_encode_backward")
        if in_place:
            grad_chain_record(grad.device)
        return None, None, (None if in_place else grad_embeddings), None, None, None, None, None, None, None, None, None


def grid_encode(inputs, embeddings, offsets, per_level_scale, base_resolution, calc_grad_inputs=False, gridtype=0,
                align_corners=False, interpolation=0, max_level=None):
    table = embeddings
    if torch.is_autocast_enabled() and embeddings.shape[1] % 2 == 0:
        table = embeddings.detach().to(torch.half)
    out = _grid_encode.apply(inputs, embeddings, table.detach(), _offsets_host(offsets), per_level_scale, base_resolution,
                             calc_grad_inputs, gridtype, align_corners, interpolation, max_level)
    L, B, C = out.shape
    return out.permute(1, 0, 2).reshape(B, L * C)


class GridEncoder(nn.Module):

    def __init__(self, input_dim=3, num_levels=16, level_dim=2, per_level_scale=2, base_resolution=16, log2_hashmap_size=19,
                 desired_resolution=None, gridtype='hash', align_corners=False, interpolation='linear'):
        super().__init__()
        if desired_resolution is not None:
            per_level_scale = np.exp2(np.log2(desired_resolution / base_resolution) / (num_levels - 1))
        if level_dim not in (1, 2, 4, 8):
            raise ValueError("GridEncoding: C must be 1, 2, 4, or 8.")
        if input_dim not in (2, 3, 4, 5):
            raise ValueError("GridEncoding: D must be 2, 3, 4, or 5.")
        self.input_dim = input_dim
        self.num_levels = num_levels
        self.level_dim = level_dim
        self.per_level_scale = per_level_scale
        self.log2_hashmap_size = log2_hashmap_size
        self.base_resolution = base_resolution
        self.output_dim = num_levels * level_dim
        self.gridtype = gridtype
        self.gridtype_id = _gridtype_to_id[gridtype]
        self.interpolation = interpolation
        self.interp_id = _interp_to_id[interpolation]
        self.align_corners = align_corners

        offsets, offset = [], 0
        self.max_params = 2 ** log2_hashmap_size
        for i in range(num_levels):
            resolution = int(np.ceil(base_resolution * per_level_scale ** i))
            params_in_level = min(self.max_params, (resolution if align_corners else resolution + 1) ** input_dim)
            params_in_level = int(np.ceil(params_in_level / 8) * 8)
            offsets.append(offset)
            offset += params_in_level
        offsets.append(offset)
        self._offsets_host = np.array(offsets, dtype=np.int32)
        self.register_buffer('offsets', torch.from_numpy(self._offsets_host.copy()))
        self.n_params = offsets[-1] * level_dim
        self.embeddings = nn.Parameter(torch.empty(offset, level_dim))
        self._half_table = None
        self._half_version = None
        self.reset_parameters()

    def reset_parameters(self):
        std = 1e-4
        self.embeddings.data.uniform_(-std, std)
        self.invalidate_half_table()

    def __repr__(self):
        return (f"GridEncoder: input_dim={self.input_dim} num_levels={self.num_levels} level_dim={self.level_dim} "
                f"resolution={self.base_resolution} -> {int(round(self.base_resolution * self.per_level_scale ** (self.num_levels - 1)))} "
                f"per_level_scale={self.per_level_scale:.4f} params={tuple(self.embeddings.shape)} gridtype={self.gridtype} "
                f"align_corners={self.align_corners} interpolation={self.interpolation}")

    def half_table(self):
        emb = self.embeddings
        key = (emb._version, emb.data_ptr(), getattr(emb, '_cnerf_epoch', 0))
        if self._half_table is None or self._half_version != key or self._half_table.device != emb.device:
            if self._half_table is None or self._half_table.shape != emb.shape or self._half_table.device != emb.device:
                self._half_table = torch.empty(emb.shape, dtype=torch.half, device=emb.device)
            check(lib.cnerf_cast_f32_to_f16(ptr(emb), ptr(self._half_table), emb.numel(), stream()), "cast_f32_to_f16")
            self._half_version = key
        return self._half_table

    def invalidate_half_table(self):
        self._half_version = None

    def set_half_table(self, table, version_key=None):
        self._half_table = table
        emb = self.embeddings
        self._half_version = version_key if version_key is not None else (emb._version, emb.data_ptr(), getattr(emb, '_cnerf_epoch', 0))

    def encode(self, inputs, bound=1, max_level=None, half=None):
        inputs = (inputs + bound) / (2 * bound)
        inputs = inputs.reshape(-1, self.input_dim)
        if half is None:
            half = torch.is_autocast_enabled() and self.level_dim % 2 == 0
        table = self.half_table() if half else self.embeddings.detach()
        return _grid_encode.apply(inputs, self.embeddings, table, self._offsets_host, self.per_level_scale, self.base_resolution,
                                  inputs.requires_grad, self.gridtype_id, self.align_corners, self.interp_id, max_level)

    @torch.no_grad()
    def encode_into(self, inputs_unit, out, row0, half=None, traversal=LEVEL_MAJOR):
        if half is None:
            half = torch.is_autocast_enabled() and self.level_dim % 2 == 0
        table = self.half_table() if half else self.embeddings.detach()
        require_cuda(inputs_unit, out, table)
        inputs_unit = inputs_unit.contiguous().float()
        B, D = inputs_unit.shape
        L, P, C = out.shape
        assert out.is_contiguous() and out.dtype == table.dtype and C == table.shape[1] and row0 + B <= P and L == self._offsets_host.shape[0] - 1
        prof = _PROFILE
        dst = out.data_ptr() + row0 * C * out.element_size()
        tuner = traversal if isinstance(traversal, TraversalTuner) else None
        todo = tuner.plan() if tuner is not None else [int(traversal)]
        for k, trav in enumerate(todo):
            timed = prof is not None or len(todo) > 1
            if timed:
                e0, e1 = torch.cuda.Event(enable_timing=True), torch.cuda.Event(enable_timing=True)
                e0.record()
            check(lib.cnerf_grid_encode_forward_ordered(ptr(inputs_unit), ptr(table), self._offsets_host.ctypes.data, dst, B, D, C, L, L,
                                                        float(np.log2(self.per_level_scale)), int(self.base_resolution), None, self.gridtype_id,
                                                        int(self.align_corners), self.interp_id, dtype_id(table), P, trav, stream()), "grid_encode_forward_ordered")
            if timed:
                e1.record()
                if len(todo) > 1:
                    tuner.record(trav, e0, e1)
                if prof is not None and k == len(todo) - 1:
                    prof.append((e0, e1, B, L, table.element_size()))

    def prepare_backward(self, inputs_unit, half):
        assert inputs_unit.is_contiguous() and inputs_unit.dtype == torch.float32
        P, D = inputs_unit.shape
        dt = dtype_id(torch.empty(0, dtype=torch.float16 if half else torch.float32))
        return _prepare_plan(inputs_unit, self._offsets_host, P, D, self.level_dim, self.num_levels, float(np.log2(self.per_level_scale)),
                             int(self.base_resolution), self.gridtype_id, self.align_corners, self.interp_id, dt, inputs_unit.device)

    def attach_backward(self, enc, inputs_unit, overlap=True, plan=None):
        return _grid_attach.apply(enc, inputs_unit.contiguous().float(), self.embeddings, self._offsets_host, self.per_level_scale, self.base_resolution,
                                  self.gridtype_id, self.align_corners, self.interp_id, bool(overlap), bool(getattr(self, 'grad_in_place', False)), plan)

    def forward(self, inputs, bound=1, max_level=None, return_kernel_layout=False):
        prefix_shape = list(inputs.shape[:-1])
        out = self.encode(inputs, bound, max_level)
        if return_kernel_layout:
            return out
        L, B, C = out.shape
        return out.permute(1, 0, 2).reshape(prefix_shape + [self.output_dim])

    @torch.no_grad()
    def grad_total_variation(self, weight=1e-7, inputs=None, bound=1, B=1000000):
        D, C = self.input_dim, self.embeddings.shape[1]
        L = self._offsets_host.shape[0] - 1
        S = float(np.log2(self.per_level_scale))
        H = self.base_resolution
        if inputs is None:
            inputs = torch.rand(B, self.input_dim, device=self.embeddings.device)
        else:
            inputs = ((inputs + bound) / (2 * bound)).view(-1, self.input_dim)
            B = inputs.shape[0]
        if self.embeddings.grad is None:
            raise ValueError('grad is None, should be called after loss.backward() and before optimizer.step()!')
        inputs = inputs.contiguous().float()
        require_cuda(inputs, self.embeddings)
        check(lib.cnerf_grad_total_variation(ptr(inputs), ptr(self.embeddings), ptr(self.embeddings.grad), self._offsets_host.ctypes.data,
                                             float(weight), B, D, C, L, S, H, self.gridtype_id, int(self.align_corners), stream()),
              "grad_total_variation")
```

customnerf_amd/nerf/render_ops.py:

```python
import torch
from torch.autograd import Function

from .._lib import lib, check, ptr, stream, require_cuda


def sample_coarse(rays_o, rays_d, nears, fars, aabb, T, noise=None, xyz_out=None, unit_out=None, bound=None):
    require_cuda(rays_o, rays_d, nears, fars, aabb, noise, xyz_out, unit_out)
    N = rays_o.shape[0]
    z = torch.empty(N, T, dtype=torch.float32, device=rays_o.device)
    xyz = xyz_out if xyz_out is not None else torch.empty(N, T, 3, dtype=torch.float32, device=rays_o.device)
    assert xyz.is_contiguous() and xyz.dtype == torch.float32 and xyz.numel() == N * T * 3
    if unit_out is not None:
        assert unit_out.is_contiguous() and unit_out.dtype == torch.float32 and unit_out.numel() == N * T * 3 and bound is not None
        check(lib.cnerf_sample_coarse_unit(ptr(rays_o), ptr(rays_d), ptr(nears), ptr(fars), ptr(aabb), ptr(noise), N, int(T), ptr(z), ptr(xyz),
                                           ptr(unit_out), float(bound), stream()), "sample_coarse_unit")
        return z, xyz
    check(lib.cnerf_sample_coarse(ptr(rays_o), ptr(rays_d), ptr(nears), ptr(fars), ptr(aabb), ptr(noise), N, int(T), ptr(z), ptr(xyz), stream()),
          "sample_coarse")
    return z, xyz


def sample_coarse_aabb(rays_o, rays_d, aabb, min_near, T, noise, xyz_out, unit_out, bound):
    require_cuda(rays_o, rays_d, aabb, noise, xyz_out, unit_out)
    N = rays_o.shape[0]
# ... 13 lines not shown
    z_all = torch.empty(N, T + t, dtype=torch.float32, device=z_vals.device)
    xyz_all = torch.empty(N, T + t, 3, dtype=torch.float32, device=z_vals.device)
    check(lib.cnerf_sample_fine_merge(ptr(rays_o), ptr(rays_d), ptr(nears), ptr(fars), ptr(aabb), ptr(z_vals), ptr(sigmas), ptr(u), N, int(T), int(t),
                                      ptr(z_all), ptr(xyz_all), stream()), "sample_fine_merge")
    return z_all, xyz_all


def sample_fine_merge_split(rays_o, rays_d, nears, fars, aabb, z_vals, sigmas, t, u=None, xyz_fine_out=None, unit_fine_out=None, bound=None):
    require_cuda(z_vals, sigmas, u, xyz_fine_out)
    N, T = z_vals.shape
    z_all = torch.empty(N, T + t, dtype=torch.float32, device=z_vals.device)
    xyz_fine = xyz_fine_out if xyz_fine_out is not None else torch.empty(N, t, 3, dtype=torch.float32, device=z_vals.device)
    assert xyz_fine.is_contiguous() and xyz_fine.dtype == torch.float32 and xyz_fine.numel() == N * t * 3
    src = torch.empty(N, T + t, dtype=torch.int32, device=z_vals.device)
    if unit_fine_out is not None:
        require_cuda(unit_fine_out)
        assert unit_fine_out.is_contiguous() and unit_fine_out.dtype == torch.float32 and unit_fine_out.numel() == N * t * 3 and bound is not None
        check(lib.cnerf_sample_fine_merge_split_unit(ptr(rays_o), ptr(rays_d), ptr(nears), ptr(fars), ptr(aabb), ptr(z_vals), ptr(sigmas), ptr(u), N, int(T),
                                                     int(t), ptr(z_all), ptr(xyz_fine), ptr(src), ptr(unit_fine_out), float(bound), stream()),
              "sample_fine_merge_split_unit")
        return z_all, xyz_fine, src
    check(lib.cnerf_sample_fine_merge_split(ptr(rays_o), ptr(rays_d), ptr(nears), ptr(fars), ptr(aabb), ptr(z_vals), ptr(sigmas), ptr(u), N, int(T), int(t),
                                            ptr(z_all), None, ptr(xyz_fine), ptr(src), stream()), "sample_fine_merge_split")
    return z_all, xyz_fine, src


class _CompositeRunIndexed(Function):

    @staticmethod
    def forward(ctx, sigmas, rgbc, z_vals, src_index, nears, fars, num_steps, soft_mask, conf_thr, detach_bg, detach_mask, flush_half_zero=False, variants=7):
        sigmas = sigmas.contiguous().float()
        rgbc = rgbc.contiguous().float()
        N, S = z_vals.shape
        ctx.flush = bool(flush_half_zero)
        out_ray = torch.empty(3, N, 6, dtype=torch.float32, device=z_vals.device)
        check(lib.cnerf_composite_run_indexed_variants(ptr(sigmas), ptr(rgbc), ptr(z_vals), ptr(nears), ptr(fars), N, S, int(num_steps), int(soft_mask),
                                                       float(conf_thr), ptr(src_index), ptr(out_ray), None, None, None, int(variants), stream()),
              "composite_run_indexed")
        ctx.save_for_backward(sigmas, rgbc, z_vals, src_index, nears, fars)
        ctx.cfg = (int(num_steps), int(soft_mask), float(conf_thr), int(detach_bg), int(detach_mask))
        return out_ray

    @staticmethod
    def backward(ctx, g_ray):
        if g_ray is None:
            return (None,) * 13
        sigmas, rgbc, z_vals, src_index, nears, fars = ctx.saved_tensors
        num_steps, soft, thr, dbg, dmask = ctx.cfg
        N, S = z_vals.shape
        g_ray = g_ray.contiguous().float()
        g_sigma = torch.empty_like(sigmas)
        g_rgbc = torch.empty_like(rgbc)
        if ctx.flush:
            tiles = (num_steps % 32 == 0 and (S - num_steps) % 32 == 0 and 0 < num_steps < S and S <= 256 and g_sigma.numel() == N * S)
            tile_live = torch.empty(N * S // 32, dtype=torch.uint8, device=g_sigma.device) if tiles else None
            check(lib.cnerf_composite_run_backward_indexed_flush(ptr(g_ray), ptr(sigmas), ptr(rgbc), ptr(z_vals), ptr(nears), ptr(fars), N, S, num_steps, soft,
                                                                 thr, dbg, dmask, ptr(src_index), ptr(g_sigma), ptr(g_rgbc), 1, ptr(tile_live), stream()),
                  "composite_run_backward_indexed_flush")
            if tile_live is not None:
                g_sigma._cnerf_tile_live = (tile_live, g_sigma.data_ptr(), g_sigma._version, g_rgbc.data_ptr(), g_rgbc._version)
        else:
            check(lib.cnerf_composite_run_backward_indexed(ptr(g_ray), ptr(sigmas), ptr(rgbc), ptr(z_vals), ptr(nears), ptr(fars), N, S, num_steps, soft, thr,
                                                           dbg, dmask, ptr(src_index), ptr(g_sigma), ptr(g_rgbc), stream()), "composite_run_backward_indexed")
        return g_sigma, g_rgbc, None, None, None, None, None, None, None, None, None, None, None


def composite_run_indexed(sigmas, rgbc, z_vals, src_index, nears, fars, num_steps, soft_mask, conf_thr, detach_bg=False, detach_mask=False,
                          flush_half_zero=False, variants=7):
    return _CompositeRunIndexed.apply(sigmas, rgbc, z_vals, src_index, nears, fars, num_steps, soft_mask, conf_thr, detach_bg, detach_mask, flush_half_zero,
                                      variants)


@torch.no_grad()
def composite_run_indexed_aux(sigmas, rgbc, z_vals, src_index, nears, fars, num_steps, soft_mask, conf_thr):
    sigmas = sigmas.detach().contiguous().float()
    rgbc = rgbc.detach().contiguous().float()
    N, S = z_vals.shape
    dev = z_vals.device
    out_ray = torch.empty(3, N, 6, dtype=torch.float32, device=dev)
    out_w = torch.empty(3, N, S, dtype=torch.float32, device=dev)
    sig_s = torch.empty(N, S, dtype=torch.float32, device=dev)
    rgbc_s = torch.empty(N, S, 4, dtype=torch.float32, device=dev)
    check(lib.cnerf_composite_run_indexed(ptr(sigmas), ptr(rgbc), ptr(z_vals), ptr(nears), ptr(fars), N, S, int(num_steps), int(soft_mask), float(conf_thr),
                                          ptr(src_index), ptr(out_ray), ptr(out_w), ptr(sig_s), ptr(rgbc_s), stream()), "composite_run_indexed")
    return out_w, sig_s, rgbc_s


class _CompositeRun(Function):

    @staticmethod
    def forward(ctx, sigmas, rgbc, z_vals, nears, fars, num_steps, soft_mask, conf_thr, detach_bg, detach_mask):
        sigmas = sigmas.contiguous().float()
        rgbc = rgbc.contiguous().float()
        N, S = z_vals.shape
        out_ray = torch.empty(3, N, 6, dtype=torch.float32, device=z_vals.device)
        out_w = torch.empty(3, N, S, dtype=torch.float32, device=z_vals.device)
        check(lib.cnerf_composite_run(ptr(sigmas), ptr(rgbc), ptr(z_vals), ptr(nears), ptr(fars), N, S, int(num_steps), int(soft_mask), float(conf_thr),
                                      ptr(out_ray), ptr(out_w), stream()), "composite_run")
        ctx.save_for_backward(sigmas, rgbc, z_vals, nears, fars)
        ctx.cfg = (int(num_steps), int(soft_mask), float(conf_thr), int(detach_bg), int(detach_mask))
        ctx.mark_non_differentiable(out_w)
        ctx.set_materialize_grads(False)
        return out_ray, out_w

    @staticmethod
    def backward(ctx, g_ray, g_w):
        if g_ray is None:
            return (None,) * 10
        sigmas, rgbc, z_vals, nears, fars = ctx.saved_tensors
        num_steps, soft, thr, dbg, dmask = ctx.cfg
        N, S = z_vals.shape
        g_ray = g_ray.contiguous().float()
        g_sigma = torch.empty_like(sigmas)
        g_rgbc = torch.empty_like(rgbc)
        check(lib.cnerf_composite_run_backward(ptr(g_ray), ptr(sigmas), ptr(rgbc), ptr(z_vals), ptr(nears), ptr(fars), N, S, num_steps, soft, thr, dbg,
                                               dmask, ptr(g_sigma), ptr(g_rgbc), stream()), "composite_run_backward")
        return g_sigma, g_rgbc, None, None, None, None, None, None, None, None


def composite_run(sigmas, rgbc, z_vals, nears, fars, num_steps, soft_mask, conf_thr, detach_bg=False, detach_mask=False):
    return _CompositeRun.apply(sigmas, rgbc, z_vals, nears, fars, num_steps, soft_mask, conf_thr, detach_bg, detach_mask)


class _ReconLoss(Function):

    @staticmethod
    def forward(ctx, out_ray, rgb_gt, mask_gt, w_rgb, w_conf, grad_scale=None):
        require_cuda(out_ray, rgb_gt, mask_gt, grad_scale)
        out_ray = out_ray.contiguous().float()
        N = out_ray.shape[1]
        rgb_gt = rgb_gt.reshape(N, 3).contiguous().float()
        mask_gt = mask_gt.reshape(N).contiguous().float() if mask_gt is not None else None
        loss = torch.empty(65, dtype=torch.float32, device=out_ray.device)
        g = torch.empty_like(out_ray)
        check(lib.cnerf_recon_loss_scaled(ptr(out_ray), ptr(rgb_gt), ptr(mask_gt), N, float(w_rgb), float(w_conf), ptr(grad_scale), ptr(loss), ptr(g),
                                          stream()), "recon_loss")
        ctx.save_for_backward(g)
        ctx.scale = grad_scale
        return loss[0]

    @staticmethod
    def backward(ctx, g_loss):
        g, = ctx.saved_tensors
        sc = ctx.scale
        if sc is None:
            return g * g_loss, None, None, None, None, None
        if g_loss.data_ptr() == sc.data_ptr() and g_loss.dtype == sc.dtype:
            return g, None, None, None, None, None
        return g * (g_loss / sc.reshape(())), None, None, None, None, None


def recon_loss(out_ray, rgb_gt, mask_gt, w_rgb, w_conf, grad_scale=None):
    return _ReconLoss.apply(out_ray, rgb_gt, mask_gt, w_rgb, w_conf, grad_scale)
```

customnerf_amd/nerf/renderer.py:

```python
import math

import numpy as np
import torch
import torch.nn as nn

from .. import raymarching, mesh as _mesh
from .._lib import lib, check, ptr, stream, require_cuda
from . import render_ops


def sample_pdf(bins, weights, n_samples, det=False, u=None):
    require_cuda(bins, weights, u)
    bins, weights = bins.contiguous().float(), weights.contiguous().float()
    B, T = bins.shape
    if weights.shape != (B, T - 1):
        raise ValueError(f"sample_pdf: weights must be [B, {T - 1}] for bins [B, {T}]")
    if not det and u is None:
        u = torch.rand(B, n_samples, device=bins.device)
    out = torch.empty(B, n_samples, dtype=torch.float32, device=bins.device)
    check(lib.cnerf_sample_pdf(ptr(bins), ptr(weights), None if det else ptr(u.contiguous().float()), B, T, int(n_samples), ptr(out), stream()), "sample_pdf")
    return out


def convert_sigma_samples_to_ply(input_3d_sigma_array, voxel_grid_origin, volume_size, ply_filename_out, level=5.0, offset=None, scale=None):
    vol = input_3d_sigma_array
    vol = (vol if torch.is_tensor(vol) else torch.from_numpy(np.ascontiguousarray(vol))).float()
    if not vol.is_cuda:
        vol = vol.cuda()
    verts, faces, normals = _mesh.marching_cubes(vol, level, spacing=tuple(volume_size), origin=(0.0, 0.0, 0.0))
    verts, faces, normals = verts.cpu().numpy(), faces.cpu().numpy(), normals.cpu().numpy()
    mesh_points = verts + np.asarray(voxel_grid_origin, dtype=np.float32)
    if scale is not None:
        mesh_points = mesh_points / scale
    if offset is not None:
        mesh_points = mesh_points - offset
    _mesh.write_ply(ply_filename_out, mesh_points, faces)
    return verts, faces, normals


class _Lazy:
    __slots__ = ('fn', 'value', 'done')

    def __init__(self, fn):
        self.fn, self.value, self.done = fn, None, False

    def get(self):
        if not self.done:
            self.value, self.done, self.fn = self.fn(), True, None
        return self.value


class _LazyResults(dict):

    def __getitem__(self, k):
        v = dict.__getitem__(self, k)
        if isinstance(v, _Lazy):
            v = v.get()
            dict.__setitem__(self, k, v)
        return v

    def get(self, k, default=None):
        return self[k] if k in self else default

    def items(self):
        return [(k, self[k]) for k in dict.keys(self)]

    def values(self):
        return [self[k] for k in dict.keys(self)]


class NeRFRenderer(nn.Module):
    def __init__(self, opt):
        super().__init__()
        self.opt = opt
        self.bound = opt.bound
        self.cascade = 1 + math.ceil(math.log2(opt.bound))
        self.grid_size = 128
        self.cuda_ray = opt.cuda_ray
        self.min_near = opt.min_near
        self.density_thresh = opt.density_thresh

        aabb_train = torch.FloatTensor([-opt.bound, -opt.bound, -opt.bound, opt.bound, opt.bound, opt.bound])
        self.register_buffer('aabb_train', aabb_train)
        self.register_buffer('aabb_infer', aabb_train.clone())
        self.register_buffer('aabb_train_bg', 2 * aabb_train.clone())
        self.register_buffer('aabb_infer_bg', 2 * aabb_train.clone())

        if self.cuda_ray:
            self.register_buffer('density_grid', torch.zeros([self.cascade, self.grid_size ** 3]))
            self.register_buffer('density_bitfield', torch.zeros(self.cascade * self.grid_size ** 3 // 8, dtype=torch.uint8))
            self.mean_density = 0
            self.iter_density = 0
            self.register_buffer('step_counter', torch.zeros(16, 2, dtype=torch.int32))
            self.mean_count = 0
            self.local_step = 0

    def forward(self, x, d):
        raise NotImplementedError()

    def density(self, x):
        raise NotImplementedError()

    def reset_extra_state(self):
        if not self.cuda_ray:
            return
        self.density_grid.zero_()
        self.mean_density = 0
        self.iter_density = 0
        self.step_counter.zero_()
        self.mean_count = 0
        self.local_step = 0

    def run(self, rays_o, rays_d, num_steps=128, upsample_steps=128, light_d=None, ambient_ratio=1.0, shading='albedo',
            bg_color=None, perturb=False, _draws=None, **kwargs):
        require_cuda(rays_o, rays_d)
        if not getattr(self.opt, 'train_conf', 0):
            return {}
        if not (3 <= num_steps <= 128 and 2 <= upsample_steps <= 128):
            raise ValueError(f"run(): the sampling kernels take 3..128 coarse and 2..128 importance samples per ray (got {num_steps} + {upsample_steps}; "
                             "the reference's recipe is 64 + 64)")
        return self._run_fused(rays_o, rays_d, num_steps, upsample_steps, perturb, _draws, fg_bg=bool(kwargs.get('fg_bg', True)))

    def _dirs_twice(self, rays_d):
        if torch.cuda.is_current_stream_capturing():
            return torch.cat([rays_d, rays_d], 0)
        cache = self.__dict__.setdefault('_dirs2_cache', {})
        key = (rays_d.data_ptr(), rays_d._version, tuple(rays_d.shape))
        ent = cache.get(key)
        if ent is None:
            if len(cache) >= 64:
                cache.pop(next(iter(cache)))
            ent = (rays_d, torch.cat([rays_d, rays_d], 0))
            cache[key] = ent
        return ent[1]

    def _field_all(self, xyz, rays_d, S):
        if getattr(self, 'supports_dir_group', False):
            sigmas, rgbc, _ = self(xyz, rays_d, dir_group=S)
        else:
            sigmas, rgbc, _ = self(xyz, rays_d.repeat_interleave(S, dim=0))
        if rgbc.shape[-1] != 4:
            raise ValueError("run() with opt.train_conf needs forward() to return rgb + 1 confidence channel (network_grid.py:126-129)")
        return sigmas.reshape(-1), rgbc.reshape(-1, 4)

    def _run_fused(self, rays_o, rays_d, num_steps, upsample_steps, perturb, _draws=None, fg_bg=True):
        prefix = rays_o.shape[:-1]
        rays_o = rays_o.contiguous().view(-1, 3).float()
        rays_d = rays_d.contiguous().view(-1, 3).float()
        N = rays_o.shape[0]
        device = rays_o.device
        draws = _draws or {}
        aabb = self.aabb_train if self.training else self.aabb_infer
        S = num_steps + upsample_steps
        soft, thr = bool(getattr(self.opt, 'soft_mask', False)), float(getattr(self.opt, 'conf_thr', 0.5))
        dbg, dmask = bool(getattr(self.opt, 'detach_bg', False)), bool(getattr(self.opt, 'detach_mask_from_field', False))
        split = (num_steps == upsample_steps and getattr(self.opt, 'split_eval', True) and getattr(self, 'supports_split_eval', False)
                 and not getattr(self.opt, 'eval_fine_density', False))
        grad_on = torch.is_grad_enabled()
        plan = None
        if not split:
            nears, fars = raymarching.near_far_from_aabb(rays_o, rays_d, aabb, self.min_near)
        with torch.no_grad():
            noise = None
            both = None
            blockwise = False
            if perturb and self.training and 'z' not in draws and 'u' not in draws:
                both = torch.rand(N * (num_steps + upsample_steps), device=device)
            if perturb:
                noise = (draws['z'].to(device).contiguous() if 'z' in draws else
                         (both[:N * num_steps].view(N, num_steps) if both is not None else torch.rand(N, num_steps, device=device)))
            if self.training:
                u_draw = lambda: (draws['u'].to(device).contiguous() if 'u' in draws else
                                  (both[N * num_steps:].view(N, upsample_steps) if both is not None else torch.rand(N, upsample_steps, device=device)))
            else:
                u_draw = lambda: None
            if split:
                Pc, P = N * num_steps, N * S
                xyz_list = torch.empty(P, 3, dtype=torch.float32, device=device)
                enc, unit = self.split_buffers(P, device)
                bnd = float(self.opt.bound)
                nears, fars, z_vals, xyz_c = render_ops.sample_coarse_aabb(rays_o, rays_d, aabb.contiguous().float(), self.min_near, num_steps, noise,
                                                                           xyz_list[:Pc].view(N, num_steps, 3), unit[:Pc].view(N, num_steps, 3), bnd)
                self.split_encode(enc, unit, xyz_list[:Pc], 0, unit_ready=True)
                blockwise = bool(getattr(self.opt, 'blockwise_field', True)) and self._fused_cfg()[2] == 4
                if blockwise:
                    sig_all, rgbc_all = self.split_outputs(P, device)
                    self.split_forward_rows(enc, 0, xyz_list[:Pc], rays_d, num_steps, sig_all, rgbc_all)
                    sig_c = sig_all[:Pc]
                else:
                    sig_c = self.split_density(enc, xyz_list[:Pc])
                z_all, xyz_f, src = render_ops.sample_fine_merge_split(rays_o, rays_d, nears, fars, aabb, z_vals, sig_c, upsample_steps, u_draw(),
                                                                        xyz_fine_out=xyz_list[Pc:].view(N, upsample_steps, 3),
                                                                        unit_fine_out=unit[Pc:].view(N, upsample_steps, 3), bound=bnd)
                plan = self.split_prepare(unit, grad_on)
                self.split_encode(enc, unit, xyz_list[Pc:], Pc, unit_ready=True, importance=True)
                if blockwise:
                    self.split_forward_rows(enc, Pc, xyz_list[Pc:], rays_d, upsample_steps, sig_all, rgbc_all)
            else:
                z_vals, xyzs = render_ops.sample_coarse(rays_o, rays_d, nears, fars, aabb, num_steps, noise)
                sig_c = self.density(xyzs.view(-1, 3))['sigma'].float().contiguous()
                z_all, xyz_all = render_ops.sample_fine_merge(rays_o, rays_d, nears, fars, aabb, z_vals, sig_c, upsample_steps, u_draw())
                if getattr(self.opt, 'eval_fine_density', False):
                    self.density(xyz_all.view(-1, 3))
        if split:
            dirs2 = self._dirs_twice(rays_d)
            if blockwise:
                sig_l, rgbc_l = self.split_attach(enc, unit, xyz_list, dirs2, num_steps, sig_all, rgbc_all, plan=plan)
            else:
                sig_l, rgbc_l = self.split_forward(enc, unit, xyz_list, dirs2, num_steps, plan=plan)
            flush = bool(grad_on and getattr(self.opt, 'early_termination', True) and self._fused_cfg() and self._half())
            out_ray = render_ops.composite_run_indexed(sig_l, rgbc_l, z_all, src, nears, fars, num_steps, soft, thr, dbg, dmask, flush_half_zero=flush,
                                                       variants=7 if fg_bg else 1)
            aux = _Lazy(lambda: render_ops.composite_run_indexed_aux(sig_l, rgbc_l, z_all, src, nears, fars, num_steps, soft, thr))
            weights_of = lambda v: _Lazy(lambda: aux.get()[0][v])
            sigma_e = _Lazy(lambda: aux.get()[1].view(N, S, 1))
            rgbs_e = _Lazy(lambda: aux.get()[2].view(N, S, 4)[..., :3])
            conf_of = lambda: aux.get()[2].view(N, S, 4)[..., 3:4]
        else:
            sigmas, rgbc = self._field_all(xyz_all.view(-1, 3), rays_d, S)
            out_ray, out_w = render_ops.composite_run(sigmas.view(N, S), rgbc.view(N, S, 4), z_all, nears, fars, num_steps, soft, thr, dbg, dmask)
            weights_of = lambda v: out_w[v]
            sigma_e, rgbs_e = sigmas.view(N, S, 1), rgbc.view(N, S, 4)[..., :3]
            conf_of = lambda: rgbc.view(N, S, 4)[..., 3:4]
        mask = _Lazy(lambda: (nears < fars).reshape(*prefix))

        def pack(v):
            r = out_ray[v]
            return _LazyResults({'image': r[:, 0:3].reshape(*prefix, 3), 'depth': r[:, 3].reshape(*prefix), 'weights_sum': r[:, 4],
                                 'render_mask': r[:, 5].reshape(*prefix, 1), 'weights': weights_of(v), 'mask': mask})
        results = pack(0)
        results['sigma'] = sigma_e
        results['rgbs'] = rgbs_e
        if getattr(self.opt, 'soft_mask', False):
            thr_ = self.opt.conf_thr
            results['edit_mask'] = _Lazy(lambda: torch.sigmoid((conf_of().detach() - thr_) * 100))
        else:
            results['edit_mask'] = _Lazy(lambda: conf_of().detach() > 0.5)
        results['z_vals'] = z_all
        results['_out_ray'] = out_ray
        if fg_bg or not split:
            results['fg'] = pack(1)
            results['bg'] = pack(2)
        return results

    def weights_sum_i(self, sample_dist, sigmas, normals, dirs, weights, z_vals, nears, fars, rgbs, prefix, masks=None,
                      bg_color=None, if_fg=False, is_all=False, num_steps=None):
        N, S = z_vals.shape
        nears, fars = nears.reshape(N).contiguous().float(), fars.reshape(N).contiguous().float()
        if num_steps is None:
            sd_ = sample_dist.reshape(-1).float().expand(N) if sample_dist.numel() in (1, N) else sample_dist.reshape(-1).float()[:N]
            ratio = torch.where((fars > nears) & (sd_ > 0), (fars - nears) / sd_.clamp_min(1e-30), torch.full_like(nears, -1.0))
            num_steps = int(torch.round(ratio.max()).item())
            if num_steps <= 0:
                raise ValueError("weights_sum_i: no ray intersects the box (near >= far everywhere); pass num_steps")
        conf = masks.reshape(N, S, 1).float() if masks is not None else torch.zeros(N, S, 1, device=z_vals.device)
        rgbc = torch.cat([rgbs.reshape(N, S, 3).float(), conf], dim=-1)
        detach_bg = bool(is_all and getattr(self.opt, 'detach_bg', False))
        out_ray, out_w = render_ops.composite_run(sigmas.reshape(N, S).float(), rgbc, z_vals.contiguous().float(), nears, fars, num_steps,
                                                  True, float(getattr(self.opt, 'conf_thr', 0.5)), detach_bg,
                                                  bool(getattr(self.opt, 'detach_mask_from_field', False)))
        r = out_ray[0]
        results = {}
        image = r[:, 0:3].reshape(*prefix, 3)
        if if_fg and bg_color is not None:
            results['black_image'] = image
            image = image + (1 - r[:, 4]).unsqueeze(-1).reshape(*prefix, 1) * bg_color
        results['image'] = image
        if getattr(self.opt, 'train_conf', 0) and masks is not None:
            results['render_mask'] = r[:, 5].reshape(*prefix, 1)
        results['depth'] = r[:, 3].reshape(*prefix)
        results['weights_sum'] = r[:, 4]
        results['weights'] = out_w[0]
        results['mask'] = (nears < fars).reshape(*prefix)
        return results

    def run_cuda(self, rays_o, rays_d, dt_gamma=0, light_d=None, ambient_ratio=1.0, shading='albedo', bg_color=None,
                 perturb=False, force_all_rays=False, max_steps=1024, T_thresh=1e-4, _noises=None, **kwargs):
        prefix = rays_o.shape[:-1]
        rays_o = rays_o.cuda().contiguous().view(-1, 3)
        rays_d = rays_d.cuda().contiguous().view(-1, 3)
        aabb = self.aabb_train if self.training else self.aabb_infer
        nears, fars = raymarching.near_far_from_aabb(rays_o, rays_d, aabb)
        results = {}
        if self.training:
            weights_sum, depth, image = self._march_train(rays_o, rays_d, nears, fars, dt_gamma, perturb, force_all_rays, max_steps, T_thresh, _noises, results)
        else:
            weights_sum, depth, image = self._march_infer(rays_o, rays_d, nears, fars, dt_gamma, perturb, max_steps, T_thresh, light_d, ambient_ratio, shading)
        bg = getattr(self.opt, 'bg_color', None)
        if bg:
            bg = torch.as_tensor(np.asarray(bg, dtype=np.float32), device=image.device).reshape(1, -1)
            image = image + (1 - weights_sum).unsqueeze(-1) * bg
        results.update(image=image.view(*prefix, 3), depth=depth.view(*prefix), weights_sum=weights_sum.reshape(*prefix),
                       mask=(nears < fars).reshape(*prefix))
        return results

    def _march_train(self, rays_o, rays_d, nears, fars, dt_gamma, perturb, force_all_rays, max_steps, T_thresh, noises, results):
        counter = self.step_counter[self.local_step % 16]
        counter.zero_()
        self.local_step += 1
        xyzs, dirs, deltas, rays = raymarching.march_rays_train(rays_o, rays_d, self.bound, self.density_bitfield, self.cascade, self.grid_size,
                                                                nears, fars, counter, self.mean_count, perturb, 128, force_all_rays, dt_gamma,
                                                                max_steps, noises=noises)
        sigmas, rgbs, _ = self(xyzs, dirs)
        results['rays'] = rays
        results['num_points'] = xyzs.shape[0]
        return raymarching.composite_rays_train(sigmas, rgbs.float(), deltas, rays, T_thresh)

    def _march_infer(self, rays_o, rays_d, nears, fars, dt_gamma, perturb, max_steps, T_thresh, light_d, ambient_ratio, shading):
        N, device = rays_o.shape[0], rays_o.device
        acc = torch.zeros(5 * N, dtype=torch.float32, device=device)
        weights_sum, depth, image = acc[:N], acc[N:2 * N], acc[2 * N:].view(N, 3)
        alive = torch.arange(N, dtype=torch.int32, device=device)
        alive_next = torch.empty_like(alive)
        count = torch.zeros(1, dtype=torch.int32, device=device)
        rays_t = nears.clone()
        n_alive, done = N, 0
        while done < max_steps and n_alive > 0:
            n_step = max(min(N // n_alive, 8), 1)
            xyzs, dirs, deltas = raymarching.march_rays(n_alive, n_step, alive, rays_t, rays_o, rays_d, self.bound, self.density_bitfield,
                                                        self.cascade, self.grid_size, nears, fars, 128, perturb and done == 0, dt_gamma, max_steps)
            sigmas, rgbs, _ = self(xyzs, dirs, light_d, ratio=ambient_ratio, shading=shading)
            raymarching.composite_rays(n_alive, n_step, alive, rays_t, sigmas, rgbs, deltas, weights_sum, depth, image, T_thresh)
            raymarching.compact_rays_alive(alive, n_alive, alive_next, count)
            alive, alive_next = alive_next, alive
            n_alive = int(count.item())
            done += n_step
        return weights_sum, depth, image

    @property
    def mean_density(self):
        md = self.__dict__.get('_mean_density', 0)
        return float(md[0]) if torch.is_tensor(md) else md

    @mean_density.setter
    def mean_density(self, v):
        self.__dict__['_mean_density'] = v

    @torch.no_grad()
    def update_extra_state(self, decay=0.95, S=128, _rand=None):
        if not self.cuda_ray:
            return
        H, dev = self.grid_size, self.density_bitfield.device
        n = H ** 3
        nblk = (n + 255) // 256
        partials = torch.empty(self.cascade * nblk, 2, dtype=torch.float64, device=dev)
        xyzs = torch.empty(n, 3, dtype=torch.float32, device=dev)
        for cas in range(self.cascade):
            bound = min(2 ** cas, self.bound)
            half = bound / H
            rnd = (_rand[cas].to(dev) if _rand is not None else torch.rand(n, 3, device=dev)).contiguous().float()
            check(lib.cnerf_occupancy_points(ptr(rnd), H, float(bound), float(half), ptr(xyzs), stream()), "occupancy_points")
            sigmas = self.density(xyzs)['sigma'].reshape(-1).float().contiguous()
            check(lib.cnerf_occupancy_update(ptr(sigmas), H, float(decay), ptr(self.density_grid[cas]), ptr(partials[cas * nblk:]), stream()), "occupancy_update")
        state = torch.empty(2, dtype=torch.float32, device=dev)
        check(lib.cnerf_occupancy_finalize_pack(ptr(partials), self.cascade * nblk, float(self.density_thresh), ptr(self.density_grid),
                                                self.density_bitfield.numel(), ptr(state), ptr(self.density_bitfield), stream()), "occupancy_finalize_pack")
        self.mean_density = state
        self.iter_density += 1
        total_step = min(16, self.local_step)
        if total_step > 0:
            self.mean_count = self._mean_sample_count(total_step)
        self.local_step = 0

    def _mean_sample_count(self, total_step):
        tot = self.step_counter[:total_step, 0].sum().float()
        import torch.distributed as dist
        if getattr(self.opt, 'sync_mean_count', True) and dist.is_available() and dist.is_initialized() and dist.get_world_size() > 1:
            from .. import _coll
            _coll.all_reduce(tot)
            tot = tot / dist.get_world_size()
        return int(tot.item() / total_step)

    def _mesh_lattice(self, resolution, aabb):
        aabb = (self.aabb_infer if aabb is None else torch.as_tensor(aabb, dtype=torch.float32)).detach().float().cpu().reshape(6)
        lo, hi = aabb[:3], aabb[3:]
        if resolution < 2 or not bool((hi > lo).all()):
            raise ValueError(f"extract_mesh: need resolution >= 2 and a non-empty box, got {resolution} and {aabb.tolist()}")
        return lo, (hi - lo) / (resolution - 1)

    @torch.no_grad()
    def density_volume(self, resolution=256, aabb=None, chunk=2 ** 21, part='all', view_dir=(0.0, 0.0, -1.0)):
        if part not in ('all', 'fg', 'bg'):
            raise ValueError(f"extract_mesh: part must be 'all', 'fg' or 'bg', got {part!r}")
        R = int(resolution)
        lo, step = self._mesh_lattice(R, aabb)
        dev = self.aabb_infer.device
        lo, step = lo.to(dev), step.to(dev)
        n = R ** 3
        vol = torch.empty(n, dtype=torch.float32, device=dev)
        d = torch.tensor(view_dir, dtype=torch.float32, device=dev).reshape(1, 3)
        soft, thr = bool(getattr(self.opt, 'soft_mask', False)), float(getattr(self.opt, 'conf_thr', 0.5))
        for s in range(0, n, chunk):
# ... 94 lines not shown
```

customnerf_amd/optim.py:

```python
import torch

import ctypes

from ._lib import lib, check, ptr, stream, require_cuda, AdamJobs, ADAM_MAX_JOBS, GridAdam

SMALL_PARAM_MAX = 1 << 16


def adam_step(p, g, m, v, lr, betas=(0.9, 0.99), eps=1e-15, step=1, grad_scale_inv=1.0, zero_grad=True, p_half=None):
    require_cuda(p, g, m, v, p_half)
    check(lib.cnerf_adam_step(ptr(p), ptr(g), ptr(m), ptr(v), ptr(p_half), p.numel(), float(lr), float(betas[0]), float(betas[1]),
                              float(eps), int(step), float(grad_scale_inv), int(zero_grad), stream()), "adam_step")


class DynamicLossScaler:

    def __init__(self, device, init_scale=65536.0, growth_factor=2.0, backoff_factor=0.5, growth_interval=2000):
        self.state = torch.tensor([init_scale, 0.0, 0.0, 0.0], dtype=torch.float32, device=device)
        self.growth_factor, self.backoff_factor, self.growth_interval = growth_factor, backoff_factor, growth_interval
        self._update_consumed = False

    def scale(self, loss):
        return loss * self.state[0]

    def backward(self, loss):
        loss.backward(gradient=self.state[0].to(loss.dtype).reshape(loss.shape))

    def check(self, flat_grads):
        require_cuda(flat_grads)
        check(lib.cnerf_scaler_check(ptr(flat_grads), flat_grads.numel(), ptr(self.state), stream()), "scaler_check")

    def watch(self, on=True):
        check(lib.cnerf_scaler_watch(ptr(self.state) if on else None), "scaler_watch")

    def update(self):
        if self._update_consumed:
            self._update_consumed = False
            return
        check(lib.cnerf_scaler_update(ptr(self.state), float(self.growth_factor), float(self.backoff_factor), int(self.growth_interval), stream()), "scaler_update")

    def get_scale(self):
        return float(self.state[0])

    def good_steps(self):
        return int(self.state[3])

    def state_dict(self):
        st = self.state.detach().cpu().tolist()
        return {"scale": st[0], "growth_factor": self.growth_factor, "backoff_factor": self.backoff_factor, "growth_interval": self.growth_interval,
                "_growth_tracker": int(st[1]), "_good_steps": int(st[3])}

    def load_state_dict(self, sd):
        good = sd.get("_good_steps", int(self.state[3]))
        self.state.copy_(torch.tensor([float(sd["scale"]), float(sd.get("_growth_tracker", 0)), 0.0, float(good)]))
        self.growth_factor, self.backoff_factor, self.growth_interval = sd["growth_factor"], sd["backoff_factor"], sd["growth_interval"]


class FusedAdam(torch.optim.Optimizer):

    def __init__(self, params, lr=5e-4, betas=(0.9, 0.99), eps=1e-15, zero_grad_in_step=True):
        super().__init__(params, dict(lr=lr, betas=betas, eps=eps))
        self.zero_grad_in_step = zero_grad_in_step
        self.half_shadows = {}
        self.grad_scale_inv = 1.0
        self.scaler = None
        self.skip_params = set()
        self.updates_scaler = False

    def arm_in_backward(self, p):
        self.disarm_in_backward()
        if self.scaler is None or p.grad is None or not (p.is_cuda and p.is_contiguous() and p.grad.is_contiguous() and p.dtype == torch.float32
                                                           and p.grad.dtype == torch.float32 and p.numel() % 4 == 0):
            return False
        group = next((g for g in self.param_groups if any(q is p for q in g['params'])), None)
        if group is None or id(p) in self.skip_params:
            return False
        st = self.state[p]
        if not st:
            st['step'] = 0
            st['exp_avg'] = torch.zeros_like(p)
            st['exp_avg_sq'] = torch.zeros_like(p)
        sh = self.half_shadows.get(p)
        require_cuda(p.data, p.grad, st['exp_avg'], st['exp_avg_sq'], sh, self.scaler.state)
        cfg = GridAdam()
        cfg.p, cfg.g, cfg.m, cfg.v = p.data.data_ptr(), p.grad.data_ptr(), st['exp_avg'].data_ptr(), st['exp_avg_sq'].data_ptr()
        cfg.p_half = sh.data_ptr() if sh is not None else None
        cfg.n = p.numel()
        cfg.lr, cfg.beta1, cfg.beta2, cfg.eps = float(group['lr']), float(group['betas'][0]), float(group['betas'][1]), float(group['eps'])
        cfg.scaler_state = self.scaler.state.data_ptr()
        cfg.extra_inv = float(self.grad_scale_inv)
        cfg.zero_grad = int(self.zero_grad_in_step)
        check(lib.cnerf_grid_backward_adam(ctypes.addressof(cfg)), "grid_backward_adam")
        self._armed = p
        return True

    def disarm_in_backward(self):
        p, self._armed = getattr(self, '_armed', None), None
        if p is None:
            return None
        done = ctypes.c_int(0)
        check(lib.cnerf_grid_backward_adam_consumed(ctypes.addressof(done)), "grid_backward_adam_consumed")
        check(lib.cnerf_grid_backward_adam(None), "grid_backward_adam")
        return p if done.value else None

    @torch.no_grad()
    def step(self, closure=None):
        self.updates_scaler = False
        if self.scaler is not None:
            self.scaler._update_consumed = False
        stepped = self.disarm_in_backward()
        if stepped is not None:
            self.state[stepped]['step'] += 1
            stepped._cnerf_epoch = getattr(stepped, '_cnerf_epoch', 0) + 1
        small = []
        betas0, eps0 = self.param_groups[0]['betas'], self.param_groups[0]['eps']
        for group in self.param_groups:
            for p in group['params']:
                if p.grad is None or id(p) in self.skip_params or p is stepped:
                    continue
                st = self.state[p]
                if not st:
                    st['step'] = 0
                    st['exp_avg'] = torch.zeros_like(p)
                    st['exp_avg_sq'] = torch.zeros_like(p)
                st['step'] += 1
                if (self.scaler is not None and p.numel() <= SMALL_PARAM_MAX and len(small) < ADAM_MAX_JOBS and group['betas'] == betas0
                        and group['eps'] == eps0 and p.grad.is_contiguous() and p.is_contiguous()):
                    small.append((p, st, group))
                    continue
                if self.scaler is not None:
                    require_cuda(p.data, p.grad, st['exp_avg'], st['exp_avg_sq'], self.half_shadows.get(p))
                    check(lib.cnerf_adam_step_scaled(ptr(p.data), ptr(p.grad), ptr(st['exp_avg']), ptr(st['exp_avg_sq']), ptr(self.half_shadows.get(p)),
                                                     p.numel(), float(group['lr']), float(group['betas'][0]), float(group['betas'][1]), float(group['eps']),
                                                     ptr(self.scaler.state), float(self.grad_scale_inv), int(self.zero_grad_in_step), stream()), "adam_step_scaled")
                else:
                    adam_step(p.data, p.grad, st['exp_avg'], st['exp_avg_sq'], group['lr'], group['betas'], group['eps'], st['step'],
                              self.grad_scale_inv, self.zero_grad_in_step, self.half_shadows.get(p))
                p._cnerf_epoch = getattr(p, '_cnerf_epoch', 0) + 1
        if small:
            jobs = AdamJobs()
            for j, (p, st, group) in enumerate(small):
                sh = self.half_shadows.get(p)
                require_cuda(p.data, p.grad, st['exp_avg'], st['exp_avg_sq'], sh)
                jobs.p[j], jobs.g[j], jobs.m[j], jobs.v[j] = p.data.data_ptr(), p.grad.data_ptr(), st['exp_avg'].data_ptr(), st['exp_avg_sq'].data_ptr()
                jobs.p_half[j] = sh.data_ptr() if sh is not None else None
                jobs.n[j], jobs.lr[j] = p.numel(), float(group['lr'])
                p._cnerf_epoch = getattr(p, '_cnerf_epoch', 0) + 1
            jobs.n_jobs = len(small)
            sc = self.scaler
            check(lib.cnerf_adam_step_scaled_multi(ctypes.addressof(jobs), float(betas0[0]), float(betas0[1]), float(eps0), ptr(sc.state),
                                                   float(self.grad_scale_inv), int(self.zero_grad_in_step), 1, float(sc.growth_factor),
                                                   float(sc.backoff_factor), int(sc.growth_interval), stream()), "adam_step_scaled_multi")
            self.updates_scaler = True
            sc._update_consumed = True

    def zero_grad(self, set_to_none=False):
        if self.zero_grad_in_step and not set_to_none:
            return
        super().zero_grad(set_to_none=set_to_none)
```

customnerf_amd/trainer.py:

```python
import torch
import torch.distributed as dist
import torch.nn.functional as F

from . import _coll
from .optim import DynamicLossScaler, FusedAdam


def flat_grad_buffer(parameters):
    ps = [p for p in parameters if p.requires_grad]
    if not ps:
        return None
    flat = torch.zeros(sum(_slot(p.numel()) for p in ps), dtype=torch.float32, device=ps[0].device)
    off = 0
    for p in ps:
        p.grad = flat[off:off + p.numel()].view_as(p)
        off += _slot(p.numel())
    return flat


def enable_grad_in_place(model):
    enc = getattr(model, 'pos_en', None)
    if enc is not None and hasattr(enc, 'attach_backward'):
        enc.grad_in_place = True
    model.grad_in_place = True


def _slot(n):
    return (n + 3) // 4 * 4


def _grads_alias_flat(grads, flat):
    off = flat.data_ptr()
    for g in grads:
        if g.dtype != flat.dtype or not g.is_contiguous() or g.data_ptr() != off:
            return False
        off += _slot(g.numel()) * flat.element_size()
    return off == flat.data_ptr() + flat.numel() * flat.element_size()


def allreduce_grads_flat(parameters, flat, world_size):
    if world_size <= 1:
        return flat
    grads = [p.grad for p in parameters if p.grad is not None]
    if flat is not None and _grads_alias_flat(grads, flat):
        _coll.all_reduce(flat, op=dist.ReduceOp.SUM)
        return flat
    n = sum(g.numel() for g in grads)
    if flat is None or flat.numel() != n:
        flat = torch.empty(n, dtype=torch.float32, device=grads[0].device)
    torch._foreach_copy_(list(flat.split([g.numel() for g in grads])), [g.reshape(-1) for g in grads])
    _coll.all_reduce(flat, op=dist.ReduceOp.SUM)
    torch._foreach_copy_([g.reshape(-1) for g in grads], list(flat.split([g.numel() for g in grads])))
    return flat


def register_half_shadow(optimizer, model, fp16):
    enc = getattr(model, 'pos_en', None)
    if fp16 and enc is not None and hasattr(enc, 'half_table') and enc.embeddings.is_cuda and enc.level_dim % 2 == 0:
        optimizer.half_shadows[enc.embeddings] = enc.half_table()


def refresh_half_shadow(optimizer, model):
    enc = getattr(model, 'pos_en', None)
    if enc is not None and enc.embeddings in optimizer.half_shadows:
        enc.set_half_table(optimizer.half_shadows[enc.embeddings])


class packed_weights_window:

    def __init__(self, model, opt=None):
        self.d = getattr(model, '__dict__', None) if getattr(opt, 'packed_field_weights', True) else None

    def __enter__(self):
        if self.d is not None:
            self.prev = self.d.get('packed_field_weights', False)
            self.d['packed_field_weights'] = True

    def __exit__(self, *exc):
        if self.d is not None:
            self.d['packed_field_weights'] = self.prev
        return False


def inf_check_is_folded(trainer):
    m = trainer.model
    if trainer.world_size != 1 or getattr(trainer, '_dp', None) is not None or trainer.scaler is None or not getattr(trainer, 'fused_adam', True):
        return False
    if not (hasattr(m, '_fused_cfg') and hasattr(m, '_half') and hasattr(m, 'pos_en') and getattr(m, 'grad_in_place', False)):
        return False
    try:
        if not (m._fused_cfg() and m._half()):
            return False
        known = {id(m.pos_en.embeddings), id(m.network.params), id(m.density_network.params), id(m.rgb_network.params)}
    except Exception:
        return False
    return all(id(p) in known for p in m.parameters() if p.requires_grad) and bool(getattr(trainer.opt, 'fold_inf_check', True))


def check_grads_finite(scaler, parameters, flat):
    grads = [p.grad for p in parameters if p.grad is not None]
    if flat is not None and _grads_alias_flat(grads, flat):
        scaler.check(flat)
    else:
        for g in grads:
            scaler.check(g.contiguous())


def setup_sharded_dp(trainer, model, fp16, rank=None, group=None):
    from .dp import ShardedExchange, BIG_PARAM_MIN
    opt_ = trainer.optimizer
    lr_by_id = {id(p): i for i, g in enumerate(opt_.param_groups) for p in g['params']}
    params = [p for p in model.parameters() if p.requires_grad]
    enc = getattr(model, 'pos_en', None)
    half = bool(fp16 and enc is not None and hasattr(enc, 'half_table') and enc.level_dim % 2 == 0)
    rank = dist.get_rank(group) if rank is None else rank
    dp = ShardedExchange(params, trainer._flat, lambda p: trainer.base_lrs[lr_by_id[id(p)]], trainer.world_size, rank, betas=(0.9, 0.99), eps=1e-15,
                         scaler=trainer.scaler, half_shadow=half, group=group)
    opt_.skip_params = {id(st['p']) for st in dp.state}
    if half and enc is not None:
        sh = dp.shadow_table(enc.embeddings)
        if sh is not None:
            opt_.half_shadows[enc.embeddings] = sh
            enc.set_half_table(sh)
    if dp.async_ops and enc is not None and hasattr(enc, 'attach_backward'):
        from .gridencoder import grid as ge
        ge.set_pre_scatter_hook(dp.start_small)
    return dp


def apply_optimizer_step(trainer):
    f = trainer.lr_factor()
    for g, base in zip(trainer.optimizer.param_groups, trainer.base_lrs):
        g['lr'] = base * f
    dp = getattr(trainer, '_dp', None)
    trainer.optimizer.grad_scale_inv = 1.0 / (trainer.loss_scale * trainer.world_size)
    if dp is not None:
        ev = getattr(trainer, '_exchange_events', None)
        if ev is not None:
            e0, e1 = torch.cuda.Event(enable_timing=True), torch.cuda.Event(enable_timing=True)
            e0.record()
        dp.exchange()
        dp.check()
        dp.step(f, trainer.loss_scale)
        if ev is not None:
            e1.record()
            ev.append((e0, e1))
        trainer.optimizer.step()
        if trainer.scaler is not None:
            trainer.scaler.update()
    else:
        trainer.allreduce_grads()
        if trainer.scaler is not None:
            if not getattr(trainer, '_inf_folded', False):
                check_grads_finite(trainer.scaler, list(trainer.model.parameters()), trainer._flat)
            trainer.optimizer.step()
            trainer.scaler.update()
        else:
            trainer.optimizer.step()
    refresh_half_shadow(trainer.optimizer, trainer.model)


class CheckpointMixin:

    def state_dict(self):
        if getattr(self, '_dp', None) is not None:
            self._dp.consolidate()
        return self.model.state_dict()

    def save_checkpoint(self, path, epoch=0, stats=None, full=False, rank=None):
        from . import checkpoint
        dp = getattr(self, '_dp', None)
        if dp is not None:
            if full:
                dp.export_optimizer_state(self.optimizer)
            else:
                dp.consolidate()
        if rank is None:
            rank = dist.get_rank() if (dist.is_available() and dist.is_initialized()) else 0
        if rank != 0:
            return None
        return checkpoint.save_checkpoint(path, self.model, epoch=epoch, global_step=self.global_step, stats=stats, optimizer=self.optimizer, full=full,
                                          scaler=self.scaler)


class EvalMixin:

    def _render_eval(self, model, rays_o, rays_d, perturb=False):
        opt = self.opt
        kw = dict(num_steps=opt.num_steps, upsample_steps=opt.upsample_steps, dt_gamma=getattr(opt, 'dt_gamma', 0), max_steps=opt.max_steps)
        with torch.no_grad(), torch.autocast('cuda', dtype=torch.float16, enabled=self.fp16):
            return model.render(rays_o, rays_d, staged=True, perturb=perturb, force_all_rays=True, **kw)

    def eval_step(self, data):
        rgbs, mask, rays_o, rays_d, H, W, _ = data
        dev = next(self.model.parameters()).device
        rgbs, mask, rays_o, rays_d = rgbs.to(dev), mask.to(dev), rays_o.to(dev), rays_d.to(dev)
        B = rays_o.shape[0]
        outputs = self._render_eval(self.model, rays_o, rays_d)
        ims = [rgbs.reshape(B, H, W, 3).float(), outputs['image'].reshape(B, H, W, 3).float(), outputs['depth'].reshape(B, H, W, 1).float().repeat(1, 1, 1, 3)]
        if getattr(self.opt, 'train_conf', 0):
            ims += [mask.reshape(B, H, W, 1).float().repeat(1, 1, 1, 3),
                    outputs['render_mask'].reshape(B, H, W, -1).float().mean(-1, keepdim=True).repeat(1, 1, 1, 3),
                    outputs['fg']['image'].reshape(B, H, W, 3).float(), outputs['bg']['image'].reshape(B, H, W, 3).float()]
        return torch.cat(ims, dim=2), None, None, torch.tensor([0])

    def test_step(self, data, bg_color=None, perturb=False, if_gui=False):
        direction = torch.tensor(0)
        if if_gui:
            rays_o, rays_d, H, W, direction = data['rays_o'], data['rays_d'], data['H'], data['W'], data['dir']
        else:
            _, _, rays_o, rays_d, H, W, _ = data
        dev = next(self.model.parameters()).device
        rays_o, rays_d = rays_o.to(dev), rays_d.to(dev)
        B = rays_o.shape[0]
        outputs = self._render_eval(self.model, rays_o, rays_d, perturb=perturb)
        pred_rgb = outputs['image'].reshape(B, H, W, 3).float()
        pred_depth = outputs['depth'].reshape(B, H, W).float()
        if getattr(self.opt, 'train_conf', 0) and getattr(self.opt, 'render_all', False):
            pred_rgb = torch.cat([pred_rgb, outputs['render_mask'].reshape(B, H, W, 1).float().repeat(1, 1, 1, 3),
                                  outputs['fg']['image'].reshape(B, H, W, 3).float(), outputs['bg']['image'].reshape(B, H, W, 3).float()], dim=2)
        return pred_rgb, pred_depth, direction


class ReconTrainer(CheckpointMixin, EvalMixin):
    def __init__(self, model, opt, lr=None, fp16=False, world_size=1, fused_adam=True, loss_scale='dynamic', dp_mode='allreduce'):
        self.model, self.opt = model, opt
        self.fp16 = fp16
        self.world_size = world_size
        self.dp_mode = dp_mode if world_size > 1 else 'none'
        if loss_scale == 'dynamic' and not (fp16 and fused_adam):
            loss_scale = 128.0
        self.scaler = DynamicLossScaler(next(model.parameters()).device) if loss_scale == 'dynamic' else None
        self.loss_scale = 1.0 if (not fp16 or self.scaler is not None) else float(loss_scale)
        lr = opt.lr if lr is None else lr
        groups = model.get_params(lr)
        self.base_lrs = [g['lr'] for g in groups]
        if fused_adam:
            self.optimizer = FusedAdam(groups, betas=(0.9, 0.99), eps=1e-15)
            self.optimizer.scaler = self.scaler
            register_half_shadow(self.optimizer, model, fp16)
        else:
            self.optimizer = torch.optim.Adam(groups, betas=(0.9, 0.99), eps=1e-15)
        self.fused_adam = fused_adam
        self.global_step = 0
        self._flat = flat_grad_buffer(self.model.parameters())
        if fused_adam:
            enable_grad_in_place(model)
        self._dp = setup_sharded_dp(self, model, fp16) if (self.dp_mode == 'sharded' and fused_adam) else None

    def lr_factor(self):
        return 0.1 ** min(self.global_step / self.opt.iters, 1)

    def dp_describe(self):
        if self.dp_mode == 'sharded' and getattr(self, '_dp', None) is not None:
            return self._dp.describe()
        return "fp32 grad all-reduce, in place on the flat buffer"

    def loss(self, outputs, rgbs, mask):
        if '_out_ray' in outputs and outputs['_out_ray'].is_cuda and getattr(self.opt, 'fused_loss', True):
            from .nerf.render_ops import recon_loss
            with_mask = bool(getattr(self.opt, 'train_conf', 0)) and 'render_mask' in outputs
            sc = getattr(self, 'scaler', None)
            return recon_loss(outputs['_out_ray'], rgbs, mask if with_mask else None, getattr(self.opt, 'train_rgb', 1.0),
                              getattr(self.opt, 'train_conf', 0) if with_mask else 0.0, sc.state[0:1] if sc is not None else None)
        pred_rgb = outputs['image']
        loss = getattr(self.opt, 'train_rgb', 1.0) * F.mse_loss(pred_rgb.reshape(-1, 3).float(), rgbs.reshape(-1, 3))
        if getattr(self.opt, 'train_conf', 0) and 'render_mask' in outputs:
            loss = loss + self.opt.train_conf * F.mse_loss(outputs['render_mask'].reshape(-1).float(), mask.reshape(-1))
        return loss

    def allreduce_grads(self):
        self._flat = allreduce_grads_flat(list(self.model.parameters()), self._flat, self.world_size)

    def select_rays(self, rays_o, rays_d, rgbs, mask, select_inds=None):
        n = int(getattr(self.opt, 'batch_rays', 0) or 0)
        if not n and select_inds is None:
            return rays_o, rays_d, rgbs, mask
        N = rays_o.reshape(-1, 3).shape[0]
        if select_inds is None:
            import numpy as np
            select_inds = np.random.choice(N, size=[n], replace=False)
        idx = torch.as_tensor(select_inds, dtype=torch.long).to(rays_o.device)
        pick = lambda t, c: t.reshape(1, N, c).index_select(1, idx) if t is not None else None
        return pick(rays_o, 3), pick(rays_d, 3), pick(rgbs, 3), pick(mask, 1)

    def _watch_scaler(self):
        self._inf_folded = inf_check_is_folded(self)
        if self.scaler is not None:
            self.scaler.watch(self._inf_folded)

    def train_step(self, rays_o, rays_d, rgbs, mask, select_inds=None, **render_kw):
        self._watch_scaler()
        try:
            with packed_weights_window(self.model, self.opt):
                return self._train_step(rays_o, rays_d, rgbs, mask, select_inds, **render_kw)
        finally:
            if self.scaler is not None:
                self.scaler.watch(False)

    def _arm_table_step(self):
        if not (self.fused_adam and getattr(self, '_inf_folded', False) and self.world_size == 1 and getattr(self, '_dp', None) is None
                and getattr(self.opt, 'fuse_table_adam', True) and not torch.cuda.is_current_stream_capturing()):
            return False
        f = self.lr_factor()
        for g, base in zip(self.optimizer.param_groups, self.base_lrs):
            g['lr'] = base * f
        self.optimizer.grad_scale_inv = 1.0 / (self.loss_scale * self.world_size)
        return self.optimizer.arm_in_backward(self.model.pos_en.embeddings)

    def _train_step(self, rays_o, rays_d, rgbs, mask, select_inds=None, **render_kw):
        self.model.train()
        rays_o, rays_d, rgbs, mask = self.select_rays(rays_o, rays_d, rgbs, mask, select_inds)
        render_kw.setdefault('fg_bg', getattr(self, 'needs_fg_bg', False))
        with torch.autocast('cuda', dtype=torch.float16, enabled=self.fp16):
            outputs = self.model.render(rays_o, rays_d, staged=False, perturb=True, force_all_rays=True, **render_kw)
            loss = self.loss(outputs, rgbs, mask)
        if self.scaler is not None:
            self._arm_table_step()
            try:
                self.scaler.backward(loss)
            except BaseException:
                self.optimizer.disarm_in_backward()
                raise
        else:
            (loss * self.loss_scale).backward()
        if self.fused_adam:
            apply_optimizer_step(self)
        else:
            self.allreduce_grads()
            f = self.lr_factor()
            for g, base in zip(self.optimizer.param_groups, self.base_lrs):
                g['lr'] = base * f
            inv = 1.0 / (self.loss_scale * self.world_size)
            if inv != 1.0:
                torch._foreach_mul_([p.grad for p in self.model.parameters() if p.grad is not None], inv)
            self.optimizer.step()
            self.optimizer.zero_grad(set_to_none=False)
        self.global_step += 1
        return loss.detach(), outputs

    def train_step_graphed(self, rays_o, rays_d, rgbs, mask, **render_kw):
        if not (self.fused_adam and self.scaler is not None) or int(getattr(self.opt, 'batch_rays', -1) or -1) > 0:
            raise ValueError("train_step_graphed: fused Adam with the dynamic loss scaler, no batch_rays")
        from ._lib import scratch_generation
        tensors = (rays_o, rays_d, rgbs, mask)
        key = tuple((t.data_ptr(), tuple(t.shape), t.dtype) for t in tensors) + (tuple(sorted(render_kw.items())),)
        cache = self.__dict__.setdefault('_graphs', {})
        if cache and any(e[3] != scratch_generation() for e in cache.values()):
            cache.clear()
            self.__dict__.pop('_graph_pool', None)
        ent = cache.get(key)
        if ent is None:
            gen0 = scratch_generation()
            for _ in range(2):
                self.train_step(rays_o, rays_d, rgbs, mask, **render_kw)
            torch.cuda.synchronize()
            self.model.train()
            graph = torch.cuda.CUDAGraph()
            self._watch_scaler()
            try:
                with torch.cuda.graph(graph, pool=self.__dict__.get('_graph_pool')), packed_weights_window(self.model, self.opt):
                    with torch.autocast('cuda', dtype=torch.float16, enabled=self.fp16):
                        outputs = self.model.render(rays_o, rays_d, staged=False, perturb=True, force_all_rays=True,
                                                    **dict(render_kw, fg_bg=render_kw.get('fg_bg', getattr(self, 'needs_fg_bg', False))))
                        loss = self.loss(outputs, rgbs, mask)
                    self.scaler.backward(loss)
                    loss = loss.detach()
            finally:
                self.scaler.watch(False)
            gen1 = scratch_generation()
            if gen1 != gen0 and cache:
                cache.clear()
            self._graph_pool = graph.pool()
            ent = cache[key] = (graph, loss, tensors, gen1)
            for k_ in list(cache):
                cache[k_] = cache[k_][:3] + (gen1,)
        self.model.train()
        self._inf_folded = inf_check_is_folded(self)
        ent[0].replay()
        apply_optimizer_step(self)
        self.global_step += 1
        return ent[1], None


def train_one_epoch(trainer, views, shard=None, log=None):
    model, opt = trainer.model, trainer.opt
    rank, world = shard if shard is not None else (0, 1)
    model.train()
    total, n = 0.0, 0
    for i in range(rank, len(views), world):
        if getattr(model, 'cuda_ray', False) and trainer.global_step % getattr(opt, 'update_extra_interval', 16) == 0:
            with torch.autocast('cuda', dtype=torch.float16, enabled=trainer.fp16):
                model.update_extra_state()
        data = views[i]
        if hasattr(trainer, 'train_step_editing'):
            loss, loss_dict = trainer.train_step(data)
        else:
            rgbs, mask, rays_o, rays_d, H, W, _ = data
            loss, _ = trainer.train_step(rays_o, rays_d, rgbs, mask, num_steps=opt.num_steps, upsample_steps=opt.upsample_steps,
                                         dt_gamma=getattr(opt, 'dt_gamma', 0), max_steps=opt.max_steps)
        total = total + loss
        n += 1
    avg = float(total) / max(n, 1)
    if log is not None:
        log(f"==> Finished epoch: average_loss {avg:.6f} over {n} views, lr x{trainer.lr_factor():.4f}")
    return avg
```

include/customnerf_hip.h:

```cpp
#ifndef CUSTOMNERF_HIP_H
#define CUSTOMNERF_HIP_H

#include <stdint.h>

#ifdef __cplusplus
extern "C" {
#endif

#define CNERF_OK 0
#define CNERF_EINVAL (-1)
#define CNERF_ENULL (-2)

#define CNERF_F32 0
#define CNERF_F16 1

#define CNERF_ABI_VERSION 7
int cnerf_abi_version(void);
const char *cnerf_target_arch(void);
#define CNERF_STAGE_EVENTS 8
int cnerf_profile_stage_events(void *const *events, uint32_t n);


int cnerf_near_far_from_aabb(const float *rays_o, const float *rays_d, const float *aabb, uint32_t N,
                             float min_near, float *nears, float *fars, void *stream);

int cnerf_sph_from_ray(const float *rays_o, const float *rays_d, float radius, uint32_t N, float *coords, void *stream);

int cnerf_morton3D(const int32_t *coords, uint32_t N, int32_t *indices, void *stream);
int cnerf_morton3D_invert(const int32_t *indices, uint32_t N, int32_t *coords, void *stream);

int cnerf_packbits(const float *grid, uint32_t N, float density_thresh, uint8_t *bitfield, void *stream);

int cnerf_occupancy_points(const float *rand, uint32_t H, float cas_bound, float half_grid, float *xyzs, void *stream);
int cnerf_occupancy_update(const float *sigmas, uint32_t H, float decay, float *density_grid_cascade, double *partials, void *stream);
int cnerf_occupancy_finalize_pack(const double *partials, uint32_t n_partials, float density_thresh, const float *density_grid,
                                  uint32_t n_bytes, float *state, uint8_t *bitfield, void *stream);

int cnerf_march_rays_train(const float *rays_o, const float *rays_d, const uint8_t *grid, float bound, float dt_gamma,
                           uint32_t max_steps, uint32_t N, uint32_t C, uint32_t H, uint32_t M, const float *nears,
                           const float *fars, float *xyzs, float *dirs, float *deltas, int32_t *rays, int32_t *counter,
                           const float *noises, void *stream);
int cnerf_march_rays_train_count(const float *rays_o, const float *rays_d, const uint8_t *grid, float bound, float dt_gamma,
                                 uint32_t max_steps, uint32_t N, uint32_t C, uint32_t H, const float *nears,
                                 const float *fars, int32_t *rays, int32_t *counter, const float *noises, void *stream);
int cnerf_march_rays_train_write(const float *rays_o, const float *rays_d, const uint8_t *grid, float bound, float dt_gamma,
                                 uint32_t max_steps, uint32_t N, uint32_t C, uint32_t H, uint32_t M, const float *nears,
                                 const float *fars, float *xyzs, float *dirs, float *deltas, const int32_t *rays,
                                 const float *noises, void *stream);
int cnerf_march_rays_train_count_hits(const float *rays_o, const float *rays_d, const uint8_t *grid, float bound, float dt_gamma,
                                      uint32_t max_steps, uint32_t N, uint32_t C, uint32_t H, const float *nears,
                                      const float *fars, int32_t *rays, int32_t *counter, const float *noises, float *hits,
                                      void *stream);
int cnerf_march_rays_train_write_hits(const float *rays_o, const float *rays_d, float bound, float dt_gamma, uint32_t max_steps,
                                      uint32_t N, uint32_t C, uint32_t H, uint32_t M, const float *nears, const float *noises,
                                      const float *hits, const int32_t *rays, float *xyzs, float *dirs, float *deltas,
                                      void *stream);

int cnerf_composite_rays_train_forward(const float *sigmas, const float *rgbs, const float *deltas, const int32_t *rays,
                                       uint32_t M, uint32_t N, float T_thresh, float *weights_sum, float *depth,
                                       float *image, uint32_t rgb_stride, void *stream);
int cnerf_composite_rays_train_backward(const float *grad_weights_sum, const float *grad_image, const float *sigmas,
                                        const float *rgbs, const float *deltas, const int32_t *rays,
                                        const float *weights_sum, const float *image, uint32_t M, uint32_t N,
                                        float T_thresh, float *grad_sigmas, float *grad_rgbs, uint32_t rgb_stride,
                                        void *stream);

int cnerf_march_rays(uint32_t n_alive, uint32_t n_step, const int32_t *rays_alive, const float *rays_t,
                     const float *rays_o, const float *rays_d, float bound, float dt_gamma, uint32_t max_steps,
                     uint32_t C, uint32_t H, const uint8_t *grid, const float *nears, const float *fars, float *xyzs,
                     float *dirs, float *deltas, const float *noises, void *stream);
int cnerf_composite_rays(uint32_t n_alive, uint32_t n_step, float T_thresh, int32_t *rays_alive, float *rays_t,
                         const float *sigmas, const float *rgbs, const float *deltas, float *weights_sum, float *depth,
                         float *image, uint32_t rgb_stride, void *stream);
int cnerf_compact_rays_alive(const int32_t *rays_alive_in, uint32_t n, int32_t *rays_alive_out, int32_t *count, void *stream);


int cnerf_grid_encode_forward(const float *inputs, const void *embeddings, const int32_t *offsets_host, void *outputs,
                              uint32_t B, uint32_t D, uint32_t C, uint32_t L, uint32_t max_level, float S, uint32_t H,
                              void *dy_dx, uint32_t gridtype, int align_corners, uint32_t interp, int dtype, void *stream);
int cnerf_grid_encode_forward_strided(const float *inputs, const void *embeddings, const int32_t *offsets_host, void *outputs,
                                      uint32_t B, uint32_t D, uint32_t C, uint32_t L, uint32_t max_level, float S, uint32_t H,
                                      void *dy_dx, uint32_t gridtype, int align_corners, uint32_t interp, int dtype,
                                      uint32_t out_level_stride, void *stream);
#define CNERF_GRID_LEVEL_MAJOR 0
#define CNERF_GRID_SAMPLE_MAJOR 1
int cnerf_grid_encode_forward_ordered(const float *inputs, const void *embeddings, const int32_t *offsets_host, void *outputs,
                                      uint32_t B, uint32_t D, uint32_t C, uint32_t L, uint32_t max_level, float S, uint32_t H,
                                      void *dy_dx, uint32_t gridtype, int align_corners, uint32_t interp, int dtype,
                                      uint32_t out_level_stride, uint32_t traversal, void *stream);

int cnerf_grid_encode_backward(const void *grad, const float *inputs, const int32_t *offsets_host, float *grad_embeddings,
                               uint32_t B, uint32_t D, uint32_t C, uint32_t L, uint32_t max_level, float S, uint32_t H,
                               const void *dy_dx, float *grad_inputs, uint32_t gridtype, int align_corners,
                               uint32_t interp, int dtype, void *workspace, uint64_t workspace_bytes, void *stream);
int cnerf_grid_encode_backward_prepare(const float *inputs, const int32_t *offsets_host, uint32_t B, uint32_t D, uint32_t C, uint32_t L,
                                       uint32_t max_level, float S, uint32_t H, uint32_t gridtype, int align_corners, uint32_t interp,
                                       int dtype, void *workspace, uint64_t workspace_bytes, int *prepared, void *stream);
int cnerf_grid_encode_backward_needs_plan(const int32_t *offsets_host, uint32_t B, uint32_t D, uint32_t C, uint32_t L, uint32_t max_level, float S,
                                          uint32_t H, uint32_t gridtype, int dtype, int *needs_plan);
int cnerf_grid_encode_backward_prepared(const void *grad, const float *inputs, const int32_t *offsets_host, float *grad_embeddings,
                                        uint32_t B, uint32_t D, uint32_t C, uint32_t L, uint32_t max_level, float S, uint32_t H,
                                        uint32_t gridtype, int align_corners, uint32_t interp, int dtype, void *workspace,
                                        uint64_t workspace_bytes, void *stream);
int cnerf_grid_encode_backward_workspace_bytes(const int32_t *offsets_host, uint32_t B, uint32_t D, uint32_t C, uint32_t L,
                                               uint32_t max_level, float S, uint32_t H, int dtype, uint64_t *bytes);

int cnerf_grad_total_variation(const float *inputs, const float *embeddings, float *grad, const int32_t *offsets_host,
                               float weight, uint32_t B, uint32_t D, uint32_t C, uint32_t L, float S, uint32_t H,
                               uint32_t gridtype, int align_corners, void *stream);

int cnerf_cast_f32_to_f16(const float *src, void *dst, uint64_t n, void *stream);

int cnerf_field_forward(const void *enc, const float *xyz, const float *dirs, uint32_t dir_group, uint32_t P, uint32_t enc_dim,
                        uint32_t n_hidden_geo, uint32_t n_rgb_out, const float *params_net, const float *params_den,
                        const float *params_rgb, float *sigma, float *rgbc, int dtype, void *stream);
int cnerf_field_forward_strided(const void *enc, const float *xyz, const float *dirs, uint32_t dir_group, uint32_t P, uint32_t enc_dim,
                                uint32_t n_hidden_geo, uint32_t n_rgb_out, const float *params_net, const float *params_den,
                                const float *params_rgb, float *sigma, float *rgbc, int dtype, uint32_t enc_level_stride,
                                void *stream);

int cnerf_field_backward(const void *enc, const float *xyz, const float *dirs, uint32_t dir_group, uint32_t P, uint32_t enc_dim,
                         uint32_t n_hidden_geo, uint32_t n_rgb_out, const float *params_net, const float *params_den,
                         const float *params_rgb, const float *grad_sigma, const float *grad_rgbc, void *grad_enc,
                         float *grad_params_net, float *grad_params_den, float *grad_params_rgb, void *workspace,
                         uint64_t workspace_bytes, int dtype, void *stream);
int cnerf_field_backward_ex(const void *enc, const float *xyz, const float *dirs, uint32_t dir_group, uint32_t P, uint32_t enc_dim,
                            uint32_t n_hidden_geo, uint32_t n_rgb_out, const float *params_net, const float *params_den,
                            const float *params_rgb, const float *grad_sigma, const float *grad_rgbc, void *grad_enc,
                            float *grad_params_net, float *grad_params_den, float *grad_params_rgb, void *workspace,
                            uint64_t workspace_bytes, int dtype, const uint8_t *tile_live, void *stream);
int cnerf_field_backward_workspace_bytes(uint32_t P, uint32_t enc_dim, uint32_t n_hidden_geo, uint32_t n_rgb_out, int dtype,
                                         uint64_t *bytes);
typedef struct CnerfGridAdam {
    float *p, *g, *m, *v;
    void *p_half;
    uint64_t n;
    float lr, beta1, beta2, eps;
    const float *scaler_state;
    float extra_inv;
    int zero_grad;
} CnerfGridAdam;
int cnerf_grid_backward_adam(const CnerfGridAdam *cfg);
int cnerf_grid_backward_adam_consumed(int *yes);

int cnerf_stream_capture_id(void *stream, uint64_t *id);
int cnerf_field_weight_image_bytes(uint32_t enc_dim, uint32_t n_hidden_geo, uint32_t n_rgb_out, uint64_t *bytes);
int cnerf_field_pack_weights(uint32_t enc_dim, uint32_t n_hidden_geo, uint32_t n_rgb_out, const float *params_net, const float *params_den,
                             const float *params_rgb, void *image, uint64_t image_bytes, void *stream);
int cnerf_field_forward_img(const void *enc, const float *xyz, const float *dirs, uint32_t dir_group, uint32_t P, uint32_t enc_dim,
                            uint32_t n_hidden_geo, uint32_t n_rgb_out, const float *params_net, const float *params_den,
                            const float *params_rgb, float *sigma, float *rgbc, int dtype, uint32_t enc_level_stride,
                            const void *weight_image, void *stream);
int cnerf_field_backward_img(const void *enc, const float *xyz, const float *dirs, uint32_t dir_group, uint32_t P, uint32_t enc_dim,
                             uint32_t n_hidden_geo, uint32_t n_rgb_out, const float *params_net, const float *params_den,
                             const float *params_rgb, const float *grad_sigma, const float *grad_rgbc, void *grad_enc,
                             float *grad_params_net, float *grad_params_den, float *grad_params_rgb, void *workspace,
                             uint64_t workspace_bytes, int dtype, const uint8_t *tile_live, const void *weight_image, void *stream);

int cnerf_mlp_forward(const void *x, uint32_t ldx, const float *params, uint32_t P, uint32_t n_in, uint32_t n_out,
                      uint32_t n_neurons, uint32_t n_hidden_layers, int output_activation, void *y, uint32_t ldy, int dtype,
                      void *stream);
int cnerf_mlp_backward(const void *x, uint32_t ldx, const float *params, const void *grad_y, uint32_t ldgy, uint32_t P,
                       uint32_t n_in, uint32_t n_out, uint32_t n_neurons, uint32_t n_hidden_layers, int output_activation,
                       void *grad_x, uint32_t ldgx, float *grad_params, void *workspace, uint64_t workspace_bytes, int dtype,
                       void *stream);
int cnerf_mlp_backward_workspace_bytes(uint32_t P, uint32_t n_in, uint32_t n_out, uint32_t n_neurons,
                                       uint32_t n_hidden_layers, int dtype, uint64_t *bytes);

int cnerf_generate_rays(const float *c2w, uint32_t V, uint32_t H, uint32_t W, float fx, float fy, float cx, float cy,
                        float level, int convention, float *origins, float *directions, void *stream);
int cnerf_generate_rays_fisheye(const float *c2w, uint32_t V, uint32_t H, uint32_t W, float fx, float fy, float cx, float cy,
                                float level, const float *distortion_host, float *origins, float *directions, void *stream);

int cnerf_sample_pdf(const float *bins, const float *weights, const float *u, uint32_t B, uint32_t n_bins, uint32_t n_samples,
                     float *samples, void *stream);
int cnerf_sample_coarse(const float *rays_o, const float *rays_d, const float *nears, const float *fars, const float *aabb,
                        const float *noise, uint32_t N, uint32_t T, float *z_vals, float *xyzs, void *stream);
int cnerf_sample_fine_merge(const float *rays_o, const float *rays_d, const float *nears, const float *fars,
                            const float *aabb, const float *z_vals, const float *sigmas, const float *u, uint32_t N,
                            uint32_t T, uint32_t t, float *z_all, float *xyz_all, void *stream);
int cnerf_sample_fine_merge_split(const float *rays_o, const float *rays_d, const float *nears, const float *fars,
                                  const float *aabb, const float *z_vals, const float *sigmas, const float *u, uint32_t N,
                                  uint32_t T, uint32_t t, float *z_all, float *xyz_all, float *xyz_fine, uint32_t *src_index,
                                  void *stream);
int cnerf_sample_coarse_unit(const float *rays_o, const float *rays_d, const float *nears, const float *fars, const float *aabb,
                             const float *noise, uint32_t N, uint32_t T, float *z_vals, float *xyzs, float *unit, float bound,
                             void *stream);
int cnerf_sample_coarse_unit_aabb(const float *rays_o, const float *rays_d, const float *aabb, float min_near, const float *noise, uint32_t N,
                                  uint32_t T, float *nears, float *fars, float *z_vals, float *xyzs, float *unit, float bound, void *stream);
int cnerf_sample_fine_merge_split_unit(const float *rays_o, const float *rays_d, const float *nears, const float *fars,
                                       const float *aabb, const float *z_vals, const float *sigmas, const float *u, uint32_t N,
                                       uint32_t T, uint32_t t, float *z_all, float *xyz_fine, uint32_t *src_index,
                                       float *unit_fine, float bound, void *stream);
int cnerf_composite_run(const float *sigmas, const float *rgbc, const float *z_vals, const float *nears, const float *fars,
                        uint32_t N, uint32_t S, uint32_t num_steps, int soft_mask, float conf_thr, float *out_ray,
                        float *out_weights, void *stream);
int cnerf_composite_run_backward(const float *grad_out_ray, const float *sigmas, const float *rgbc, const float *z_vals,
                                 const float *nears, const float *fars, uint32_t N, uint32_t S, uint32_t num_steps,
                                 int soft_mask, float conf_thr, int detach_bg, int detach_mask_from_field,
                                 float *grad_sigmas, float *grad_rgbc, void *stream);
int cnerf_composite_run_indexed(const float *sigmas, const float *rgbc, const float *z_vals, const float *nears, const float *fars,
                                uint32_t N, uint32_t S, uint32_t num_steps, int soft_mask, float conf_thr,
                                const uint32_t *src_index, float *out_ray, float *out_weights, float *sigma_sorted,
                                float *rgbc_sorted, void *stream);
int cnerf_composite_run_indexed_variants(const float *sigmas, const float *rgbc, const float *z_vals, const float *nears, const float *fars,
                                         uint32_t N, uint32_t S, uint32_t num_steps, int soft_mask, float conf_thr, const uint32_t *src_index,
                                         float *out_ray, float *out_weights, float *sigma_sorted, float *rgbc_sorted, uint32_t variant_mask,
                                         void *stream);
int cnerf_composite_run_backward_indexed(const float *grad_out_ray, const float *sigmas, const float *rgbc, const float *z_vals,
                                         const float *nears, const float *fars, uint32_t N, uint32_t S, uint32_t num_steps,
                                         int soft_mask, float conf_thr, int detach_bg, int detach_mask_from_field,
                                         const uint32_t *src_index, float *grad_sigmas, float *grad_rgbc, void *stream);
int cnerf_composite_run_backward_indexed_flush(const float *grad_out_ray, const float *sigmas, const float *rgbc, const float *z_vals,
                                               const float *nears, const float *fars, uint32_t N, uint32_t S, uint32_t num_steps,
                                               int soft_mask, float conf_thr, int detach_bg, int detach_mask_from_field,
                                               const uint32_t *src_index, float *grad_sigmas, float *grad_rgbc, int flush_half_zero,
                                               uint8_t *tile_live, void *stream);

int cnerf_recon_loss(const float *out_ray, const float *rgb_gt, const float *mask_gt, uint32_t N, float w_rgb, float w_conf,
                     float *loss, float *grad_out_ray, void *stream);
int cnerf_recon_loss_scaled(const float *out_ray, const float *rgb_gt, const float *mask_gt, uint32_t N, float w_rgb, float w_conf,
                            const float *grad_scale, float *loss, float *grad_out_ray, void *stream);

int cnerf_adam_step(float *p, float *g, float *m, float *v, void *p_half, uint64_t n, float lr, float beta1, float beta2,
                    float eps, uint32_t step, float grad_scale_inv, int zero_grad, void *stream);

int cnerf_scaler_check(const float *g, uint64_t n, float *state, void *stream);
int cnerf_scaler_watch(float *state);
int cnerf_adam_step_scaled(float *p, float *g, float *m, float *v, void *p_half, uint64_t n, float lr, float beta1, float beta2,
                           float eps, const float *state, float extra_inv, int zero_grad, void *stream);
int cnerf_scaler_update(float *state, float growth_factor, float backoff_factor, uint32_t growth_interval, void *stream);
#define CNERF_ADAM_MAX_JOBS 8
typedef struct CnerfAdamJobs {
    float *p[CNERF_ADAM_MAX_JOBS], *g[CNERF_ADAM_MAX_JOBS], *m[CNERF_ADAM_MAX_JOBS], *v[CNERF_ADAM_MAX_JOBS];
    void *p_half[CNERF_ADAM_MAX_JOBS];
    uint64_t n[CNERF_ADAM_MAX_JOBS];
    float lr[CNERF_ADAM_MAX_JOBS];
    uint32_t n_jobs;
} CnerfAdamJobs;
int cnerf_adam_step_scaled_multi(const CnerfAdamJobs *jobs, float beta1, float beta2, float eps, float *state, float extra_inv, int zero_grad,
                                 int update_scaler, float growth_factor, float backoff_factor, uint32_t growth_interval, void *stream);

int cnerf_dp_pack(float *grad, void *payload_half, uint64_t n, float scale, void *stream);
int cnerf_dp_reduce(const void *recv_half, uint32_t world, uint64_t shard, float *out, float *scaler_state, void *stream);

int cnerf_marching_cubes_workspace_bytes(uint32_t nx, uint32_t ny, uint32_t nz, uint64_t *bytes_host);
int cnerf_marching_cubes_count(const float *vol, uint32_t nx, uint32_t ny, uint32_t nz, float level, void *ws, uint64_t ws_bytes,
                               uint32_t *counts, void *stream);
int cnerf_marching_cubes_emit(const float *vol, uint32_t nx, uint32_t ny, uint32_t nz, float level, const float *origin_host,
                              const float *spacing_host, void *ws, uint64_t ws_bytes, float *verts, float *normals, int32_t *faces,
                              uint32_t max_verts, uint32_t max_faces, void *stream);

int cnerf_mesh_components_workspace_bytes(uint32_t V, uint32_t F, uint64_t *bytes_host);
int cnerf_mesh_components_count(const int32_t *faces, uint32_t V, uint32_t F, uint32_t min_faces, int largest, void *ws, uint64_t ws_bytes,
                                uint32_t *counts, void *stream);
int cnerf_mesh_components_emit(const float *verts, const float *normals, uint32_t V, const int32_t *faces, uint32_t F, uint32_t min_faces,
                               int largest, void *ws, uint64_t ws_bytes, float *verts_out, float *normals_out, int32_t *faces_out,
                               int32_t *old_index, uint32_t max_verts, uint32_t max_faces, void *stream);
int cnerf_mesh_cluster_workspace_bytes(uint32_t V, uint32_t F, const uint32_t *grid_host, uint64_t *bytes_host);
int cnerf_mesh_cluster_count(const float *verts, uint32_t V, const int32_t *faces, uint32_t F, const float *origin_host, const float *cell_host,
                             const uint32_t *grid_host, void *ws, uint64_t ws_bytes, uint32_t *counts, void *stream);
int cnerf_mesh_cluster_emit(const float *verts, const float *normals, uint32_t V, const int32_t *faces, uint32_t F, const float *origin_host,
                            const float *cell_host, const uint32_t *grid_host, void *ws, uint64_t ws_bytes, float *verts_out, float *normals_out,
                            int32_t *faces_out, uint32_t max_verts, uint32_t max_faces, void *stream);

int cnerf_mesh_decimate_workspace_bytes(uint32_t V, uint32_t F, uint64_t *bytes_host);
int cnerf_mesh_decimate_init(const float *verts, uint32_t V, const int32_t *faces, uint32_t F, void *ws, uint64_t ws_bytes,
                             uint32_t *counts, void *stream);
int cnerf_mesh_decimate_round(uint32_t V, uint32_t F, uint32_t target_faces, void *ws, uint64_t ws_bytes, uint32_t *counts, void *stream);
int cnerf_mesh_decimate_emit(const float *normals, uint32_t V, uint32_t F, void *ws, uint64_t ws_bytes, float *verts_out,
                             float *normals_out, int32_t *faces_out, int32_t *old_index, uint32_t max_verts, uint32_t max_faces,
                             void *stream);

int cnerf_mesh_atlas_layout(uint32_t F, uint32_t R, uint32_t *n_host, uint32_t *s_host);
int cnerf_mesh_atlas_uvs(const int32_t *faces, uint32_t V, uint32_t F, uint32_t R, float *uvs, uint32_t max_faces, uint32_t *flags,
                         void *stream);
int cnerf_mesh_atlas_points(const float *verts, const float *normals, uint32_t V, const int32_t *faces, uint32_t F, uint32_t R, uint32_t t0,
                            uint32_t t1, const uint32_t *flags, float *x, float *d, uint32_t max_points, void *stream);
int cnerf_mesh_atlas_store(uint32_t F, uint32_t R, uint32_t t0, uint32_t t1, const float *rgb, uint32_t rgb_stride, const uint8_t *fill_host,
                           const uint32_t *flags, uint8_t *image, void *stream);
int cnerf_mesh_atlas_fill(uint32_t F, uint32_t R, const uint8_t *fill_host, uint8_t *image, void *stream);

int cnerf_mesh_smooth_workspace_bytes(uint32_t V, uint32_t F, uint64_t *bytes_host);
int cnerf_mesh_smooth_init(const int32_t *faces, uint32_t V, uint32_t F, void *ws, uint64_t ws_bytes, uint32_t *flags, void *stream);
int cnerf_mesh_smooth_steps(const float *verts_in, uint32_t V, uint32_t F, uint32_t iterations, float lambda, float mu, int pin_boundary,
                            void *ws, uint64_t ws_bytes, float *verts_out, void *stream);
int cnerf_mesh_smooth_normals(const float *verts, const float *normals_in, uint32_t V, const int32_t *faces, uint32_t F, void *ws,
                              uint64_t ws_bytes, float *normals_out, void *stream);

int cnerf_mesh_raster_workspace_bytes(uint32_t V, uint32_t F, uint32_t H, uint32_t W, uint64_t *bytes_host);
int cnerf_mesh_raster_visibility(const float *verts, uint32_t V, const int32_t *faces, uint32_t F, const float *c2w_host, float fx, float fy,
                                 float cx, float cy, uint32_t H, uint32_t W, int convention, float near, int cull, void *ws, uint64_t ws_bytes,
                                 int32_t *face_out, float *depth_out, float *bary_out, uint32_t *counts, void *stream);
int cnerf_mesh_raster_shade(const int32_t *face, const float *depth, const float *bary, uint32_t H, uint32_t W, const int32_t *faces, uint32_t V,
                            uint32_t F, int mode, const uint8_t *colors, const float *uvs, const uint8_t *texture, uint32_t R,
                            const float *verts, const float *normals, float d0, float d1, const uint8_t *bg_host, uint8_t *image, uint8_t *mask,
                            void *stream);

int cnerf_mesh_bvh_workspace_bytes(uint32_t V, uint32_t F, uint64_t *bytes_host);
int cnerf_mesh_bvh_build(const float *verts, uint32_t V, const int32_t *faces, uint32_t F, void *ws, uint64_t ws_bytes, uint32_t *counts,
                         void *stream);
int cnerf_mesh_bvh_closest(const void *ws, uint64_t ws_bytes, uint32_t V, uint32_t F, const float *points, uint32_t Q, float *dist2,
                           int32_t *face, float *point, float *bary, uint64_t *stats, void *stream);
int cnerf_mesh_sample_workspace_bytes(uint32_t F, uint64_t *bytes_host);
int cnerf_mesh_sample_count(const float *verts, uint32_t V, const int32_t *faces, uint32_t F, float spacing, void *ws, uint64_t ws_bytes,
                            uint64_t *counts, void *stream);
int cnerf_mesh_sample_emit(const float *verts, uint32_t V, const int32_t *faces, uint32_t F, float spacing, void *ws, uint64_t ws_bytes,
                           float *points, int32_t *face, float *bary, float *weight, uint64_t max_samples, void *stream);

#ifdef __cplusplus
}
#endif
#endif
```

Measured before the change: 8.397 million.

## Fuse compositing, recon loss and its backward into one kernel; skip zero grad reads

Adds a kernel that composites rays, computes the reconstruction loss and its gradient, and runs the compositing backward in a single pass. The last block uses a ticket to reduce the loss. This removes separate forward-composite, loss and backward launches and their intermediate memory traffic. The grid Adam path also gets a flag, set when a version token shows the table gradient was already zeroed, that lets it skip reading and rewriting the gradient buffer. In exchange the backward is computed eagerly during the forward and depends on fragile token bookkeeping to prove the gradient is zero.

```diff
diff --git a/customnerf_amd/_lib.py b/customnerf_amd/_lib.py
--- a/customnerf_amd/_lib.py
+++ b/customnerf_amd/_lib.py
@@ -65,6 +65,8 @@
     "cnerf_composite_run_backward": [vp, vp, vp, vp, vp, vp, u32, u32, u32, i32, f32, i32, i32, vp, vp, vp],
     "cnerf_recon_loss": [vp, vp, vp, u32, f32, f32, vp, vp, vp],
     "cnerf_recon_loss_scaled": [vp, vp, vp, u32, f32, f32, vp, vp, vp, vp],
+    "cnerf_composite_run_loss_backward_indexed": [vp, vp, vp, vp, vp, u32, u32, u32, i32, f32, i32, i32, vp, vp, vp, f32, f32, vp, vp, vp, vp, vp, vp, i32,
+                                                  vp, vp],
     "cnerf_sample_coarse_unit_aabb": [vp, vp, vp, f32, vp, u32, u32, vp, vp, vp, vp, vp, f32, vp],
     "cnerf_composite_run_indexed": [vp, vp, vp, vp, vp, u32, u32, u32, i32, f32, vp, vp, vp, vp, vp, vp],
     "cnerf_composite_run_indexed_variants": [vp, vp, vp, vp, vp, u32, u32, u32, i32, f32, vp, vp, vp, vp, vp, u32, vp],
@@ -166,7 +168,7 @@
 
 class GridAdam(C.Structure):
     _fields_ = [("p", vp), ("g", vp), ("m", vp), ("v", vp), ("p_half", vp), ("n", u64), ("lr", f32), ("beta1", f32), ("beta2", f32), ("eps", f32),
-                ("scaler_state", vp), ("extra_inv", f32), ("zero_grad", C.c_int)]
+                ("scaler_state", vp), ("extra_inv", f32), ("zero_grad", C.c_int), ("grad_is_zero", C.c_int)]
 
 
 F32, F16 = 0, 1
diff --git a/customnerf_amd/csrc/gridencoder_binned.hip b/customnerf_amd/csrc/gridencoder_binned.hip
--- a/customnerf_amd/csrc/gridencoder_binned.hip
+++ b/customnerf_amd/csrc/gridencoder_binned.hip
@@ -787,6 +787,7 @@
     const float *state;
     float lr, beta1, beta2, eps, extra_inv;
     int zero_grad, on;
+    int gzero;
     const float *cst;
 };
 struct B3AdamConst { float gscale, step_size, rsqrt_bc2; int skip; };
@@ -807,7 +808,7 @@
     *reinterpret_cast<float4 *>(ad.p + idx) = pp;
     *reinterpret_cast<float4 *>(ad.m + idx) = mm;
     *reinterpret_cast<float4 *>(ad.v + idx) = vv;
-    *d4 = ad.zero_grad ? make_float4(0, 0, 0, 0) : gg;
+    if (!ad.gzero) *d4 = ad.zero_grad ? make_float4(0, 0, 0, 0) : gg;
     if (ad.ph) {
         union { __half2 h[2]; uint2 u; } o;
         o.h[0] = __floats2half2_rn(pp.x, pp.y);
@@ -844,7 +845,7 @@
             const uint32_t j = it * 1024 + threadIdx.x;
             if (j < n_entries / 2) {
                 const size_t idx = index_of(j);
-                gg[it] = *reinterpret_cast<const float4 *>(grad_grid + idx);
+                gg[it] = ad.gzero ? make_float4(0, 0, 0, 0) : *reinterpret_cast<const float4 *>(grad_grid + idx);
                 pp[it] = *reinterpret_cast<const float4 *>(ad.p + idx);
                 mm[it] = *reinterpret_cast<const float4 *>(ad.m + idx);
                 vv[it] = *reinterpret_cast<const float4 *>(ad.v + idx);
@@ -908,7 +909,7 @@
     const size_t idx = ((size_t)lv.offset[level] + e_dst) * 2;
     const bool fin = !sl && ok, upd = fin && ad.on && !adc.skip;
     float4 g_old = make_float4(0, 0, 0, 0), pp = g_old, mm = g_old, vv = g_old;
-    if (fin) g_old = *reinterpret_cast<const float4 *>(grad_grid + idx);
+    if (fin && !(upd && ad.gzero)) g_old = *reinterpret_cast<const float4 *>(grad_grid + idx);
     if (upd) {
         pp = *reinterpret_cast<const float4 *>(ad.p + idx);
         mm = *reinterpret_cast<const float4 *>(ad.m + idx);
@@ -1263,6 +1264,7 @@
     ad.state = g_grid_adam.scaler_state;
     ad.lr = g_grid_adam.lr; ad.beta1 = g_grid_adam.beta1; ad.beta2 = g_grid_adam.beta2; ad.eps = g_grid_adam.eps; ad.extra_inv = g_grid_adam.extra_inv;
     ad.zero_grad = g_grid_adam.zero_grad; ad.on = 1;
+    ad.gzero = g_grid_adam.grad_is_zero && g_grid_adam.zero_grad && g_cn_found_inf != nullptr && g_cn_found_inf == g_grid_adam.scaler_state + 2;
     g_grid_adam_consumed = 1;
     return ad;
 }
diff --git a/customnerf_amd/csrc/render.hip b/customnerf_amd/csrc/render.hip
--- a/customnerf_amd/csrc/render.hip
+++ b/customnerf_amd/csrc/render.hip
@@ -514,6 +514,204 @@
     }
 }
 
+typedef float rn_f4 __attribute__((ext_vector_type(4)));
+
+template <int NCH>
+__global__ void __launch_bounds__(RN_THREADS) k_composite_run_loss_bwd(const float *__restrict__ sigmas, const float *__restrict__ rgbc,
+                                                                       const float *__restrict__ z_vals, const float *__restrict__ nears,
+                                                                       const float *__restrict__ fars, uint32_t N, uint32_t S, uint32_t num_steps,
+                                                                       int soft, float thr, int detach_bg, int detach_mask,
+                                                                       const uint32_t *__restrict__ src_index, const float *__restrict__ rgb_gt,
+                                                                       const float *__restrict__ mask_gt, float k_rgb, float k_m,
+                                                                       const float *__restrict__ grad_scale, float *__restrict__ out_ray,
+                                                                       float *__restrict__ g_sigma, float *__restrict__ g_rgbc, float flush_thr,
+                                                                       uint8_t *__restrict__ tile_live, rn_f4 *terms, float *loss, uint32_t vblocks) {
+    __shared__ float red[2][RL_BLOCKS][RN_WAVES];
+    __shared__ unsigned int s_last;
+    const uint32_t lane = threadIdx.x & 63, wave = threadIdx.x >> 6;
+    const uint32_t n = blockIdx.x * RN_WAVES + wave;
+    const uint32_t T_coarse = num_steps;
+    if (n < N) {
+        const float near = nears[n], far = fars[n];
+        const float sd = (far - near) / (float)num_steps;
+        const float *zr = z_vals + (size_t)n * S;
+        const float4 *c4 = reinterpret_cast<const float4 *>(rgbc);
+        float z_[NCH], delta_[NCH], sigma_[NCH], alpha_[NCH], tr_[NCH];
+        float4 c_[NCH];
+        uint32_t row_[NCH];
+        float acc[6] = {0, 0, 0, 0, 0, 0};
+        {
+            float carry = 1.0f;
+#pragma unroll
+            for (int ch = 0; ch < NCH; ch++) {
+                const uint32_t i = ch * 64 + lane;
+                const bool ok = i < S;
+                float z = 0, delta = 0, sigma = 0;
+                float4 c = make_float4(0, 0, 0, 0);
+                uint32_t row = 0;
+                if (ok) {
+                    z = zr[i];
+                    delta = (i + 1 < S) ? zr[i + 1] - z : sd;
+                    row = src_index ? src_index[(size_t)n * S + i] : n * S + i;
+                    sigma = sigmas[row];
+                    c = c4[row];
+                }
+                const float zn = rn_norm_depth(z, near, far);
+                const float alpha = ok ? 1.0f - expf(-delta * (sigma * 1.0f)) : 0.0f;
+                const float tr = rn_excl_prod_scan(ok ? (1.0f - alpha + 1e-15f) : 1.0f, carry, lane);
+                const float w = alpha * tr;
+                if (ok) {
+                    acc[0] += w * c.x; acc[1] += w * c.y; acc[2] += w * c.z;
+                    acc[3] += w * zn; acc[4] += w; acc[5] += w * c.w;
+                }
+                z_[ch] = z; delta_[ch] = delta; sigma_[ch] = sigma; c_[ch] = c; row_[ch] = row; alpha_[ch] = alpha; tr_[ch] = tr;
+            }
+        }
+        float o[6];
+#pragma unroll
+        for (int k = 0; k < 6; k++) {
+            o[k] = rn_wave_sum(acc[k]);
+            if (lane == 0) out_ray[(size_t)n * 6 + k] = o[k];
+        }
+        if (lane < 6) {
+            out_ray[((size_t)N + n) * 6 + lane] = 0.0f;
+            out_ray[((size_t)2 * N + n) * 6 + lane] = 0.0f;
+        }
+        const float gsc = grad_scale ? grad_scale[0] : 1.0f;
+        float go[6] = {0, 0, 0, 0, 0, 0};
+        rn_f4 term = {0.0f, 0.0f, 0.0f, 0.0f};
+#pragma unroll
+        for (int c = 0; c < 3; c++) {
+            const float d = o[c] - rgb_gt[(size_t)n * 3 + c];
+            term[c] = d;
+            go[c] = (2.0f * k_rgb * d) * gsc;
+        }
+        if (mask_gt) {
+            const float d = o[5] - mask_gt[n];
+            term[3] = d;
+            go[5] = (2.0f * k_m * d) * gsc;
+        }
+        if (lane == 0) { terms[n] = term; __threadfence(); }
+        bool any = false;
+#pragma unroll
+        for (int k = 0; k < 6; k++) any = any || !(go[k] == 0.0f);
+        const bool use = __builtin_amdgcn_readfirstlane(any ? 1 : 0) != 0;
+        const float e_lo = __expf(-15.0f), e_hi = __expf(15.0f);
+        uint32_t live_bits = 0;
+        float tot = 0.0f;
+        if (use) {
+#pragma unroll
+            for (int ch = 0; ch < NCH; ch++) {
+                const bool ok = ch * 64 + lane < S;
+                const float4 c = c_[ch];
+                const float zn = rn_norm_depth(z_[ch], near, far);
+                const float G = go[0] * c.x + go[1] * c.y + go[2] * c.z + go[3] * zn + go[4] + (detach_mask ? 0.0f : go[5] * c.w);
+                if (ok) tot += G * alpha_[ch] * tr_[ch];
+            }
+            tot = rn_wave_sum(tot);
+        }
+        float pref = 0.0f;
+#pragma unroll
+        for (int ch = 0; ch < NCH; ch++) {
+            const uint32_t i = ch * 64 + lane;
+            const bool ok = i < S;
+            const float z = z_[ch], delta = delta_[ch], sigma = sigma_[ch];
+            const float4 c = c_[ch];
+            const uint32_t row = row_[ch];
+            const float zn = rn_norm_depth(z, near, far);
+            const float e = rn_edit(c.w, soft, thr);
+            float gs = 0.0f, ge = 0.0f;
+            float4 gc = make_float4(0, 0, 0, 0);
+            if (use) {
+                const float m = rn_variant_scale(0, e);
+                const float alpha = alpha_[ch];
+                const float q = 1.0f - alpha + 1e-15f;
+                const float tr = tr_[ch];
+                const float w = alpha * tr;
+                const float G = go[0] * c.x + go[1] * c.y + go[2] * c.z + go[3] * zn + go[4] + (detach_mask ? 0.0f : go[5] * c.w);
+                const float incl = rn_incl_sum_scan(ok ? G * w : 0.0f, pref, lane);
+                const float suffix = tot - incl;
+                const float dalpha = G * tr - suffix / q;
+                const float dsv = dalpha * delta * (1.0f - alpha);
+                const bool detached = detach_bg && !(c.w >= 0.5f);
+                if (!detached) {
+                    gs += dsv * m;
+                    gc.x += go[0] * w; gc.y += go[1] * w; gc.z += go[2] * w;
+                }
+                gc.w += go[5] * w;
+            }
+            if (soft) gc.w += ge * 100.0f * e * (1.0f - e);
+            if (flush_thr > 0.0f) {
+                const float sc = fminf(fmaxf(sigma, e_lo), e_hi);
+                const bool dead = fabsf(gs) * sc < flush_thr && fabsf(gc.x) * (c.x * (1.0f - c.x)) < flush_thr && fabsf(gc.y) * (c.y * (1.0f - c.y)) < flush_thr &&
+                                  fabsf(gc.z) * (c.z * (1.0f - c.z)) < flush_thr && fabsf(gc.w) * (c.w * (1.0f - c.w)) < flush_thr;
+                if (dead) { gs = 0.0f; gc = make_float4(0, 0, 0, 0); }
+                else if (ok && tile_live) {
+                    const uint32_t Pc = N * T_coarse, t_f = S - T_coarse;
+                    const uint32_t lt = row < Pc ? (row - n * T_coarse) >> 5 : (T_coarse >> 5) + ((row - Pc - n * t_f) >> 5);
+                    live_bits |= 1u << lt;
+                }
+            }
+            if (ok) {
+                g_sigma[row] = gs;
+                reinterpret_cast<float4 *>(g_rgbc)[row] = gc;
+            }
+        }
+        if (tile_live) {
+            const uint32_t Pc = N * T_coarse, t_f = S - T_coarse, ntc = T_coarse >> 5, ntf = t_f >> 5;
+            for (uint32_t k = 0; k < ntc + ntf; k++) {
+                const bool live = __ballot((live_bits >> k) & 1u) != 0;
+                if (lane == 0) tile_live[k < ntc ? (n * T_coarse >> 5) + k : ((Pc + n * t_f) >> 5) + (k - ntc)] = live ? 1 : 0;
+            }
+        }
+    }
+    __syncthreads();
+    if (threadIdx.x == 0) {
+        __threadfence();
+        s_last = atomicAdd(&g_recon_loss_ticket, 1u) == gridDim.x - 1 ? 1u : 0u;
+    }
+    __syncthreads();
+    if (!s_last) return;
+    __threadfence();
+    const uint32_t stride = vblocks * 256;
+    for (uint32_t b0 = 0; b0 < vblocks; b0 += 8) {
+        float s_rgb[8], s_m[8];
+#pragma unroll
+        for (int j = 0; j < 8; j++) {
+            s_rgb[j] = 0.0f; s_m[j] = 0.0f;
+            if (b0 + j < vblocks)
+                for (uint32_t r = (b0 + j) * 256 + threadIdx.x; r < N; r += stride) {
+                    const rn_f4 t = __builtin_nontemporal_load(terms + r);
+#pragma unroll
+                    for (int c = 0; c < 3; c++) {
+                        const float d = t[c];
+                        s_rgb[j] += d * d;
+                    }
+                    if (mask_gt) {
+                        const float d = t[3];
+                        s_m[j] += d * d;
+                    }
+                }
+        }
+#pragma unroll
+        for (int j = 0; j < 8; j++) {
+            const float a = rn_wave_sum(s_rgb[j]), b = mask_gt ? rn_wave_sum(s_m[j]) : 0.0f;
+            if (lane == 0 && b0 + j < vblocks) { red[0][b0 + j][wave] = a; red[1][b0 + j][wave] = b; }
+        }
+    }
+    __syncthreads();
+    if (threadIdx.x < 64) {
+        const uint32_t b = threadIdx.x;
+        float p = 0.0f;
+        if (b < vblocks) {
+            p = k_rgb * (red[0][b][0] + red[0][b][1] + red[0][b][2] + red[0][b][3]) + k_m * (red[1][b][0] + red[1][b][1] + red[1][b][2] + red[1][b][3]);
+            loss[1 + b] = p;
+        }
+        const float v = rn_wave_sum(p);
+        if (threadIdx.x == 0) { loss[0] = v; g_recon_loss_ticket = 0; }
+    }
+}
+
 
 extern "C" {
 
@@ -656,6 +854,32 @@
     return cnerf_recon_loss_scaled(out_ray, rgb_gt, mask_gt, N, w_rgb, w_conf, nullptr, loss, grad_out_ray, stream);
 }
 
+int cnerf_composite_run_loss_backward_indexed(const float *sigmas, const float *rgbc, const float *z_vals, const float *nears, const float *fars, uint32_t N,
+                                              uint32_t S, uint32_t num_steps, int soft_mask, float conf_thr, int detach_bg, int detach_mask_from_field,
+                                              const uint32_t *src_index, const float *rgb_gt, const float *mask_gt, float w_rgb, float w_conf,
+                                              const float *grad_scale, float *out_ray, float *loss, float *ray_terms, float *grad_sigmas,
+                                              float *grad_rgbc, int flush_half_zero, uint8_t *tile_live, void *stream) {
+    if (N == 0 || S == 0 || S > 64 * RN_MAXCH || num_steps == 0) return CNERF_EINVAL;
+    if (!sigmas || !rgbc || !z_vals || !nears || !fars || !rgb_gt || !out_ray || !loss || !ray_terms || !grad_sigmas || !grad_rgbc) return CNERF_ENULL;
+    if ((((uintptr_t)rgbc) | ((uintptr_t)grad_rgbc) | ((uintptr_t)ray_terms)) & 15) return CNERF_EINVAL;
+    if (tile_live && (!flush_half_zero || !src_index || num_steps >= S || (num_steps & 31u) || ((S - num_steps) & 31u) || S > 256)) return CNERF_EINVAL;
+    if ((uint64_t)N * S > 0xFFFFFFFFull) return CNERF_EINVAL;
+    const uint32_t vblocks = cn_div_up(N, 256) < RL_BLOCKS ? cn_div_up(N, 256) : RL_BLOCKS;
+#define RN_CLB(NCH)                                                                                                                                     \
+    hipLaunchKernelGGL(k_composite_run_loss_bwd<NCH>, dim3(cn_div_up(N, RN_WAVES)), dim3(RN_THREADS), 0, CN_STREAM(stream), sigmas, rgbc, z_vals, nears, \
+                       fars, N, S, num_steps, soft_mask, conf_thr, detach_bg, detach_mask_from_field, src_index, rgb_gt, mask_gt,                      \
+                       w_rgb / (3.0f * (float)N), mask_gt ? w_conf / (float)N : 0.0f, grad_scale, out_ray, grad_sigmas, grad_rgbc,                    \
+                       flush_half_zero ? 1.4901161193847656e-08f  : 0.0f, tile_live, reinterpret_cast<rn_f4 *>(ray_terms), loss, vblocks)
+    switch (cn_div_up(S, 64)) {
+        case 1: RN_CLB(1); break;
+        case 2: RN_CLB(2); break;
+        case 3: RN_CLB(3); break;
+        default: RN_CLB(4); break;
+    }
+#undef RN_CLB
+    return cn_launch_status();
+}
+
 int cnerf_sample_pdf(const float *bins, const float *weights, const float *u, uint32_t B, uint32_t n_bins, uint32_t n_samples, float *samples, void *stream) {
     if (n_bins < 2 || n_bins > RN_PDF_MAXB) return CNERF_EINVAL;
     if (B == 0 || n_samples == 0) return CNERF_OK;
diff --git a/customnerf_amd/gridencoder/grid.py b/customnerf_amd/gridencoder/grid.py
--- a/customnerf_amd/gridencoder/grid.py
+++ b/customnerf_amd/gridencoder/grid.py
@@ -261,6 +261,7 @@
         grad_embeddings = tgt if in_place else torch.zeros(eshape, device=grad.device, dtype=torch.float32)
         if in_place:
             grad_chain_wait(grad.device)
+            ctx.param._cnerf_grad_writes = getattr(ctx.param, '_cnerf_grad_writes', 0) + 1
         if ctx.plan is not None:
             ws, ev = ctx.plan.ws, ctx.plan.event
             torch.cuda.current_stream().wait_event(ev)
@@ -432,6 +433,7 @@
             raise ValueError('grad is None, should be called after loss.backward() and before optimizer.step()!')
         inputs = inputs.contiguous().float()
         require_cuda(inputs, self.embeddings)
+        self.embeddings._cnerf_grad_writes = getattr(self.embeddings, '_cnerf_grad_writes', 0) + 1
         check(lib.cnerf_grad_total_variation(ptr(inputs), ptr(self.embeddings), ptr(self.embeddings.grad), self._offsets_host.ctypes.data,
                                              float(weight), B, D, C, L, S, H, self.gridtype_id, int(self.align_corners), stream()),
               "grad_total_variation")
diff --git a/customnerf_amd/nerf/render_ops.py b/customnerf_amd/nerf/render_ops.py
--- a/customnerf_amd/nerf/render_ops.py
+++ b/customnerf_amd/nerf/render_ops.py
@@ -189,3 +189,75 @@
 
 def recon_loss(out_ray, rgb_gt, mask_gt, w_rgb, w_conf, grad_scale=None):
     return _ReconLoss.apply(out_ray, rgb_gt, mask_gt, w_rgb, w_conf, grad_scale)
+
+
+def _tile_flags(N, S, num_steps, g_sigma):
+    tiles = (num_steps % 32 == 0 and (S - num_steps) % 32 == 0 and 0 < num_steps < S and S <= 256 and g_sigma.numel() == N * S)
+    return torch.empty(N * S // 32, dtype=torch.uint8, device=g_sigma.device) if tiles else None
+
+
+class _CompositeRunLoss(Function):
+
+    @staticmethod
+    def forward(ctx, sigmas, rgbc, z_vals, src_index, nears, fars, num_steps, soft_mask, conf_thr, detach_bg, detach_mask, flush_half_zero, rgb_gt, mask_gt,
+                w_rgb, w_conf, grad_scale):
+        require_cuda(sigmas, rgbc, z_vals, src_index, nears, fars, rgb_gt, mask_gt, grad_scale)
+        sigmas = sigmas.contiguous().float()
+        rgbc = rgbc.contiguous().float()
+        N, S = z_vals.shape
+        dev = z_vals.device
+        rgb_gt = rgb_gt.reshape(N, 3).contiguous().float()
+        mask_gt = mask_gt.reshape(N).contiguous().float() if mask_gt is not None else None
+        out_ray = torch.empty(3, N, 6, dtype=torch.float32, device=dev)
+        loss = torch.empty(65, dtype=torch.float32, device=dev)
+        terms = torch.empty(N, 4, dtype=torch.float32, device=dev)
+        g_sigma = torch.empty_like(sigmas)
+        g_rgbc = torch.empty_like(rgbc)
+        flush = bool(flush_half_zero)
+        tile_live = _tile_flags(N, S, int(num_steps), g_sigma) if flush else None
+        ctx.cfg = (int(num_steps), int(soft_mask), float(conf_thr), int(detach_bg), int(detach_mask), flush, float(w_rgb), float(w_conf))
+        check(lib.cnerf_composite_run_loss_backward_indexed(ptr(sigmas), ptr(rgbc), ptr(z_vals), ptr(nears), ptr(fars), N, S, int(num_steps), int(soft_mask),
+                                                            float(conf_thr), int(detach_bg), int(detach_mask), ptr(src_index), ptr(rgb_gt), ptr(mask_gt),
+                                                            float(w_rgb), float(w_conf), ptr(grad_scale), ptr(out_ray), ptr(loss), ptr(terms), ptr(g_sigma),
+                                                            ptr(g_rgbc), int(flush), ptr(tile_live), stream()), "composite_run_loss_backward_indexed")
+        ctx.save_for_backward(sigmas, rgbc, z_vals, src_index, nears, fars, rgb_gt, mask_gt, out_ray, g_sigma, g_rgbc, tile_live)
+        ctx.scale = grad_scale
+        ctx.set_materialize_grads(False)
+        return out_ray, loss[0]
+
+    @staticmethod
+    def backward(ctx, g_out_ray, g_loss):
+        none = (None,) * 15
+        if g_out_ray is None and g_loss is None:
+            return (None, None) + none
+        sigmas, rgbc, z_vals, src_index, nears, fars, rgb_gt, mask_gt, out_ray, g_sigma, g_rgbc, tile_live = ctx.saved_tensors
+        sc = ctx.scale
+        num_steps, soft, thr, dbg, dmask, flush, w_rgb, w_conf = ctx.cfg
+        N, S = z_vals.shape
+        if g_out_ray is None and sc is not None and g_loss.data_ptr() == sc.data_ptr() and g_loss.dtype == sc.dtype:
+            if tile_live is not None:
+                g_sigma._cnerf_tile_live = (tile_live, g_sigma.data_ptr(), g_sigma._version, g_rgbc.data_ptr(), g_rgbc._version)
+            return (g_sigma, g_rgbc) + none
+        g_ray = g_out_ray.contiguous().float() if g_out_ray is not None else None
+        if g_loss is not None:
+            scratch = torch.empty(65, dtype=torch.float32, device=out_ray.device)
+            g = torch.empty_like(out_ray)
+            check(lib.cnerf_recon_loss_scaled(ptr(out_ray), ptr(rgb_gt), ptr(mask_gt), N, w_rgb, w_conf, None, ptr(scratch), ptr(g), stream()), "recon_loss")
+            g = g * g_loss
+            g_ray = g if g_ray is None else g_ray + g
+        g_sigma = torch.empty_like(sigmas)
+        g_rgbc = torch.empty_like(rgbc)
+        tile_live = _tile_flags(N, S, num_steps, g_sigma) if flush else None
+        check(lib.cnerf_composite_run_backward_indexed_flush(ptr(g_ray), ptr(sigmas), ptr(rgbc), ptr(z_vals), ptr(nears), ptr(fars), N, S, num_steps, soft, thr,
+                                                             dbg, dmask, ptr(src_index), ptr(g_sigma), ptr(g_rgbc), int(flush), ptr(tile_live), stream()),
+              "composite_run_backward_indexed_flush")
+        if tile_live is not None:
+            g_sigma._cnerf_tile_live = (tile_live, g_sigma.data_ptr(), g_sigma._version, g_rgbc.data_ptr(), g_rgbc._version)
+        return (g_sigma, g_rgbc) + none
+
+
+def composite_run_recon_loss(sigmas, rgbc, z_vals, src_index, nears, fars, num_steps, soft_mask, conf_thr, rgb_gt, mask_gt, w_rgb, w_conf, grad_scale,
+                             detach_bg=False, detach_mask=False, flush_half_zero=False):
+    assert grad_scale is not None
+    return _CompositeRunLoss.apply(sigmas, rgbc, z_vals, src_index, nears, fars, num_steps, soft_mask, conf_thr, detach_bg, detach_mask, flush_half_zero,
+                                   rgb_gt, mask_gt, w_rgb, w_conf, grad_scale)
diff --git a/customnerf_amd/nerf/renderer.py b/customnerf_amd/nerf/renderer.py
--- a/customnerf_amd/nerf/renderer.py
+++ b/customnerf_amd/nerf/renderer.py
@@ -119,7 +119,8 @@
         if not (3 <= num_steps <= 128 and 2 <= upsample_steps <= 128):
             raise ValueError(f"run(): the sampling kernels take 3..128 coarse and 2..128 importance samples per ray (got {num_steps} + {upsample_steps}; "
                              "the reference's recipe is 64 + 64)")
-        return self._run_fused(rays_o, rays_d, num_steps, upsample_steps, perturb, _draws, fg_bg=bool(kwargs.get('fg_bg', True)))
+        return self._run_fused(rays_o, rays_d, num_steps, upsample_steps, perturb, _draws, fg_bg=bool(kwargs.get('fg_bg', True)),
+                               recon_loss=kwargs.get('_recon_loss'))
 
     def _dirs_twice(self, rays_d):
         if torch.cuda.is_current_stream_capturing():
@@ -143,7 +144,7 @@
             raise ValueError("run() with opt.train_conf needs forward() to return rgb + 1 confidence channel (network_grid.py:126-129)")
         return sigmas.reshape(-1), rgbc.reshape(-1, 4)
 
-    def _run_fused(self, rays_o, rays_d, num_steps, upsample_steps, perturb, _draws=None, fg_bg=True):
+    def _run_fused(self, rays_o, rays_d, num_steps, upsample_steps, perturb, _draws=None, fg_bg=True, recon_loss=None):
         prefix = rays_o.shape[:-1]
         rays_o = rays_o.contiguous().view(-1, 3).float()
         rays_d = rays_d.contiguous().view(-1, 3).float()
@@ -202,6 +203,7 @@
                 z_all, xyz_all = render_ops.sample_fine_merge(rays_o, rays_d, nears, fars, aabb, z_vals, sig_c, upsample_steps, u_draw())
                 if getattr(self.opt, 'eval_fine_density', False):
                     self.density(xyz_all.view(-1, 3))
+        fused_loss = None
         if split:
             dirs2 = self._dirs_twice(rays_d)
             if blockwise:
@@ -209,8 +211,13 @@
             else:
                 sig_l, rgbc_l = self.split_forward(enc, unit, xyz_list, dirs2, num_steps, plan=plan)
             flush = bool(grad_on and getattr(self.opt, 'early_termination', True) and self._fused_cfg() and self._half())
-            out_ray = render_ops.composite_run_indexed(sig_l, rgbc_l, z_all, src, nears, fars, num_steps, soft, thr, dbg, dmask, flush_half_zero=flush,
-                                                       variants=7 if fg_bg else 1)
+            if recon_loss is not None and not fg_bg and grad_on and recon_loss.get('grad_scale') is not None:
+                out_ray, fused_loss = render_ops.composite_run_recon_loss(sig_l, rgbc_l, z_all, src, nears, fars, num_steps, soft, thr,
+                                                                          recon_loss['rgb_gt'], recon_loss.get('mask_gt'), recon_loss['w_rgb'],
+                                                                          recon_loss['w_conf'], recon_loss['grad_scale'], dbg, dmask, flush_half_zero=flush)
+            else:
+                out_ray = render_ops.composite_run_indexed(sig_l, rgbc_l, z_all, src, nears, fars, num_steps, soft, thr, dbg, dmask, flush_half_zero=flush,
+                                                           variants=7 if fg_bg else 1)
             aux = _Lazy(lambda: render_ops.composite_run_indexed_aux(sig_l, rgbc_l, z_all, src, nears, fars, num_steps, soft, thr))
             weights_of = lambda v: _Lazy(lambda: aux.get()[0][v])
             sigma_e = _Lazy(lambda: aux.get()[1].view(N, S, 1))
@@ -238,6 +245,8 @@
             results['edit_mask'] = _Lazy(lambda: conf_of().detach() > 0.5)
         results['z_vals'] = z_all
         results['_out_ray'] = out_ray
+        if fused_loss is not None:
+            results['_recon_loss'] = fused_loss
         if fg_bg or not split:
             results['fg'] = pack(1)
             results['bg'] = pack(2)
diff --git a/customnerf_amd/optim.py b/customnerf_amd/optim.py
--- a/customnerf_amd/optim.py
+++ b/customnerf_amd/optim.py
@@ -67,7 +67,7 @@
         self.skip_params = set()
         self.updates_scaler = False
 
-    def arm_in_backward(self, p):
+    def arm_in_backward(self, p, grad_is_zero=False):
         self.disarm_in_backward()
         if self.scaler is None or p.grad is None or not (p.is_cuda and p.is_contiguous() and p.grad.is_contiguous() and p.dtype == torch.float32
                                                            and p.grad.dtype == torch.float32 and p.numel() % 4 == 0):
@@ -90,6 +90,7 @@
         cfg.scaler_state = self.scaler.state.data_ptr()
         cfg.extra_inv = float(self.grad_scale_inv)
         cfg.zero_grad = int(self.zero_grad_in_step)
+        cfg.grad_is_zero = int(bool(grad_is_zero) and self.zero_grad_in_step)
         check(lib.cnerf_grid_backward_adam(ctypes.addressof(cfg)), "grid_backward_adam")
         self._armed = p
         return True
diff --git a/customnerf_amd/trainer.py b/customnerf_amd/trainer.py
--- a/customnerf_amd/trainer.py
+++ b/customnerf_amd/trainer.py
@@ -126,6 +126,20 @@
         from .gridencoder import grid as ge
         ge.set_pre_scatter_hook(dp.start_small)
     return dp
+
+
+def table_grad_token(p):
+    g = getattr(p, 'grad', None)
+    if g is None or not torch.is_tensor(g):
+        return None
+    return (g.data_ptr(), g._version, getattr(p, '_cnerf_grad_writes', 0))
+
+
+def note_table_grad_cleared(trainer):
+    emb = getattr(getattr(trainer.model, 'pos_en', None), 'embeddings', None)
+    ok = (trainer.fused_adam and getattr(trainer.optimizer, 'zero_grad_in_step', False) and emb is not None
+          and id(emb) not in getattr(trainer.optimizer, 'skip_params', ()))
+    trainer._table_clean = table_grad_token(emb) if ok else None
 
 
 def apply_optimizer_step(trainer):
@@ -246,6 +260,7 @@
         self._flat = flat_grad_buffer(self.model.parameters())
         if fused_adam:
             enable_grad_in_place(model)
+            note_table_grad_cleared(self)
         self._dp = setup_sharded_dp(self, model, fp16) if (self.dp_mode == 'sharded' and fused_adam) else None
 
     def lr_factor(self):
@@ -269,6 +284,13 @@
             loss = loss + self.opt.train_conf * F.mse_loss(outputs['render_mask'].reshape(-1).float(), mask.reshape(-1))
         return loss
 
+    def _recon_loss_request(self, rgbs, mask):
+        if not (self.scaler is not None and self.world_size == 1 and type(self).loss is ReconTrainer.loss and 'loss' not in self.__dict__ and getattr(self.opt, 'fused_loss', True)
+                and getattr(self.opt, 'fuse_ray_pass', True) and getattr(self.opt, 'train_conf', 0) and mask is not None and rgbs.is_cuda and mask.is_cuda
+                and not torch.cuda.is_current_stream_capturing()):
+            return None
+        return dict(rgb_gt=rgbs, mask_gt=mask, w_rgb=getattr(self.opt, 'train_rgb', 1.0), w_conf=self.opt.train_conf, grad_scale=self.scaler.state[0:1])
+
     def allreduce_grads(self):
         self._flat = allreduce_grads_flat(list(self.model.parameters()), self._flat, self.world_size)
 
@@ -306,15 +328,24 @@
         for g, base in zip(self.optimizer.param_groups, self.base_lrs):
             g['lr'] = base * f
         self.optimizer.grad_scale_inv = 1.0 / (self.loss_scale * self.world_size)
-        return self.optimizer.arm_in_backward(self.model.pos_en.embeddings)
+        p = self.model.pos_en.embeddings
+        clean = getattr(self, '_table_clean', None)
+        if clean is not None and getattr(self.opt, 'table_grad_known_zero', True) and clean == table_grad_token(p):
+            return self.optimizer.arm_in_backward(p, grad_is_zero=True)
+        return self.optimizer.arm_in_backward(p)
 
     def _train_step(self, rays_o, rays_d, rgbs, mask, select_inds=None, **render_kw):
         self.model.train()
         rays_o, rays_d, rgbs, mask = self.select_rays(rays_o, rays_d, rgbs, mask, select_inds)
         render_kw.setdefault('fg_bg', getattr(self, 'needs_fg_bg', False))
+        req = self._recon_loss_request(rgbs, mask) if not render_kw['fg_bg'] else None
+        if req is not None:
+            render_kw['_recon_loss'] = req
         with torch.autocast('cuda', dtype=torch.float16, enabled=self.fp16):
             outputs = self.model.render(rays_o, rays_d, staged=False, perturb=True, force_all_rays=True, **render_kw)
-            loss = self.loss(outputs, rgbs, mask)
+            loss = outputs.pop('_recon_loss', None) if req is not None else None
+            if loss is None:
+                loss = self.loss(outputs, rgbs, mask)
         if self.scaler is not None:
             self._arm_table_step()
             try:
@@ -326,6 +357,7 @@
             (loss * self.loss_scale).backward()
         if self.fused_adam:
             apply_optimizer_step(self)
+            note_table_grad_cleared(self)
         else:
             self.allreduce_grads()
             f = self.lr_factor()
@@ -379,6 +411,7 @@
         self._inf_folded = inf_check_is_folded(self)
         ent[0].replay()
         apply_optimizer_step(self)
+        note_table_grad_cleared(self)
         self.global_step += 1
         return ent[1], None
 
diff --git a/include/customnerf_hip.h b/include/customnerf_hip.h
--- a/include/customnerf_hip.h
+++ b/include/customnerf_hip.h
@@ -139,6 +139,7 @@
     const float *scaler_state;
     float extra_inv;
     int zero_grad;
+    int grad_is_zero;
 } CnerfGridAdam;
 int cnerf_grid_backward_adam(const CnerfGridAdam *cfg);
 int cnerf_grid_backward_adam_consumed(int *yes);
@@ -221,6 +222,11 @@
                      float *loss, float *grad_out_ray, void *stream);
 int cnerf_recon_loss_scaled(const float *out_ray, const float *rgb_gt, const float *mask_gt, uint32_t N, float w_rgb, float w_conf,
                             const float *grad_scale, float *loss, float *grad_out_ray, void *stream);
+int cnerf_composite_run_loss_backward_indexed(const float *sigmas, const float *rgbc, const float *z_vals, const float *nears, const float *fars,
+                                              uint32_t N, uint32_t S, uint32_t num_steps, int soft_mask, float conf_thr, int detach_bg,
+                                              int detach_mask_from_field, const uint32_t *src_index, const float *rgb_gt, const float *mask_gt,
+                                              float w_rgb, float w_conf, const float *grad_scale, float *out_ray, float *loss, float *ray_terms,
+                                              float *grad_sigmas, float *grad_rgbc, int flush_half_zero, uint8_t *tile_live, void *stream);
 
 int cnerf_adam_step(float *p, float *g, float *m, float *v, void *p_half, uint64_t n, float lr, float beta1, float beta2,
                     float eps, uint32_t step, float grad_scale_inv, int zero_grad, void *stream);
```

After: 6.390 million. 0.761x the previous value.
